# fakerlove1/HPFG

Measured on AMD Instinct MI355X. Metric: labeled+unlabeled images/sec/node, U-Net 224x224 ACDC-shaped (Mean-Teacher step), higher is better.
Workload: dtype bf16x3 (fp32 storage; products as split-bf16 MFMA hi*hi+hi*lo+lo*hi, fp32 accumulate); 1 GPU; mean_teacher_unet_224x224 (BASELINE configs[1]): U-Net 1ch->4cls, 8 labelled + 8 unlabelled per GPU, student fwd+bwd + train-mode teacher fwd + CE/Dice/MSE + SGD + EMA; size=224, hipgraph=True, sync_bn=False, parallelism=dp1, math=bf16x3

## Files before the change

### hpfg_amd/_lib.py

```python
from __future__ import annotations

import ctypes as C
import os
import threading

_HERE = os.path.dirname(os.path.abspath(__file__))
LIB_PATH = os.path.join(_HERE, "lib", "libhpfg_hip.so")

BN_MEAN, BN_RSTD, BN_SCALE, BN_SHIFT, BN_K1, BN_K2, BN_K3, BN_SPARE, BN_ROWS = range(9)
ACT_NONE, ACT_PLAIN, ACT_STRIDED, ACT_BNACT, ACT_BNACT_POOL, ACT_UP2X, ACT_DZ, ACT_SPLIT16, ACT_UPBWD = range(9)
OPT_CONV_THIN, OPT_FIRST_MFMA, OPT_FIRST_WGRAD, OPT_NARROW_DEEP, OPT_UPDATE_PACK = 0, 1, 2, 3, 4
LOSS_NSUM = 32
LOSS_MAX_CLASSES = 16
ACC_MAX_SHARDS = 8
VERSION = 142
RESIZE_TAPS = 36
SURFACE_SEGS = 32
MATH_F32, MATH_BF16X3 = 0, 1


class HipLibraryError(RuntimeError):
    pass


class Act(C.Structure):
    _fields_ = [("z", C.c_void_p), ("bn", C.c_void_p), ("aux", C.c_void_p), ("mode", C.c_int32), ("C", C.c_int32),
                ("Hs", C.c_int32), ("Ws", C.c_int32), ("pstride", C.c_int32), ("aux_pstride", C.c_int32),
                ("bn_stride", C.c_int32), ("bn_coff", C.c_int32), ("sn", C.c_int32), ("sc", C.c_int32), ("sy", C.c_int32),
                ("sx", C.c_int32), ("drop_p", C.c_float), ("drop_seed", C.c_uint32), ("drop_mask", C.c_void_p), ("seed_dev", C.c_void_p),
                ("bn_acc", C.c_void_p), ("bn_gamma", C.c_void_p), ("bn_beta", C.c_void_p), ("bn_count", C.c_float), ("bn_eps", C.c_float),
                ("bn_shards", C.c_int32), ("reserved1", C.c_int32)]


class ConvArgs(C.Structure):
    _fields_ = [("a0", Act), ("a1", Act), ("wpk", C.c_void_p), ("bias", C.c_void_p), ("out", C.c_void_p),
                ("stat_partials", C.c_void_p), ("out_pstride", C.c_int32), ("Cout", C.c_int32), ("CoutPad", C.c_int32),
                ("N", C.c_int32), ("H", C.c_int32), ("W", C.c_int32), ("taps", C.c_int32), ("math", C.c_int32),
                ("bwd_stats", C.c_int32), ("bwd_of", Act), ("out2", C.c_void_p), ("out_split", C.c_int32), ("out2_pstride", C.c_int32),
                ("stat_acc", C.c_void_p), ("stat_shards", C.c_int32), ("reserved2", C.c_int32), ("stage_out", C.c_void_p), ("side_sums", C.c_void_p)]


class WgradArgs(C.Structure):
    _fields_ = [("a0", Act), ("a1", Act), ("g", Act), ("slab", C.c_void_p), ("dw_oihw", C.c_void_p), ("Cin", C.c_int32),
                ("CinPad", C.c_int32), ("Cout", C.c_int32), ("CoutPad", C.c_int32), ("N", C.c_int32), ("H", C.c_int32),
                ("W", C.c_int32), ("taps", C.c_int32), ("S", C.c_int32), ("math", C.c_int32), ("defer_reduce", C.c_int32)]


class PeerX(C.Structure):
    _fields_ = [("mbox", C.c_void_p * 8), ("epoch", C.c_void_p), ("err", C.c_void_p), ("world", C.c_int32), ("rank", C.c_int32),
                ("slot", C.c_int32), ("cap", C.c_int32), ("slot_bytes", C.c_int64)]


class PeerBuf(C.Structure):
    _fields_ = [("win", C.c_void_p * 8), ("epoch", C.c_void_p), ("err", C.c_void_p), ("world", C.c_int32), ("rank", C.c_int32),
                ("slice", C.c_int64), ("n", C.c_int64), ("stride", C.c_int64)]


class FusedBwdArgs(C.Structure):
    _fields_ = [("d", ConvArgs), ("xa0", Act), ("xa1", Act), ("slab", C.c_void_p), ("Cin", C.c_int32), ("CinPad", C.c_int32),
                ("Cout", C.c_int32), ("CoutPad", C.c_int32)]


class AugSample(C.Structure):
    _fields_ = [("img_off", C.c_int64), ("lab_off", C.c_int64), ("h", C.c_int32), ("w", C.c_int32), ("mode", C.c_int32), ("k", C.c_int32),
                ("axis", C.c_int32), ("tab_off", C.c_int32), ("m00", C.c_double), ("m01", C.c_double), ("m10", C.c_double),
                ("m11", C.c_double), ("off_y", C.c_double), ("off_x", C.c_double)]


class BnAccDesc(C.Structure):
    _fields_ = [("acc", C.c_void_p), ("gamma", C.c_void_p), ("beta", C.c_void_p), ("running_mean", C.c_void_p), ("running_var", C.c_void_p),
                ("bn", C.c_void_p), ("C", C.c_int32), ("count", C.c_float), ("shards", C.c_int32), ("reserved", C.c_int32)]


class BnAccBwdDesc(C.Structure):
    _fields_ = [("acc", C.c_void_p), ("gamma", C.c_void_p), ("bn", C.c_void_p), ("dgamma", C.c_void_p), ("dbeta", C.c_void_p),
                ("C", C.c_int32), ("count", C.c_float), ("shards", C.c_int32), ("reserved", C.c_int32)]


class SlabDesc(C.Structure):
    _fields_ = [("slab", C.c_void_p), ("dw_oihw", C.c_void_p), ("S", C.c_int32), ("taps", C.c_int32), ("Cin", C.c_int32),
                ("CinPad", C.c_int32), ("Cout", C.c_int32), ("CoutPad", C.c_int32)]


class PackDesc(C.Structure):
    _fields_ = [("w_oihw", C.c_void_p), ("b", C.c_void_p), ("wpk_fwd", C.c_void_p), ("wpk_dgrad", C.c_void_p),
                ("bias_pad", C.c_void_p), ("wpk16_fwd", C.c_void_p), ("wpk16_dgrad", C.c_void_p), ("Cout", C.c_int32), ("Cin", C.c_int32),
                ("CoutPad", C.c_int32), ("CinPad", C.c_int32), ("taps", C.c_int32), ("kc", C.c_int32)]


class UpdatePackDesc(C.Structure):
    _fields_ = [("w_off", C.c_long), ("b_off", C.c_long), ("wpk16_fwd", C.c_void_p), ("wpk16_dgrad", C.c_void_p), ("bias_pad", C.c_void_p),
                ("t_wpk16_fwd", C.c_void_p), ("t_bias_pad", C.c_void_p), ("Cout", C.c_int32), ("Cin", C.c_int32), ("CoutPad", C.c_int32),
                ("CinPad", C.c_int32), ("taps", C.c_int32), ("kc", C.c_int32), ("kc_t", C.c_int32), ("reserved", C.c_int32)]
# ... 80 lines not shown
    "hpfg_ln_bwd_blocks": (_i, [_l]),
    "hpfg_ln_px_fwd": (_i, [_p, _p, _p, _p, _p, _p, _i, _i, _i, _i, _i, _f, _p]),
    "hpfg_ln_px_bwd": (_i, [_p, _p, _p, _p, _p, _p, _p, _p, _p, _i, _i, _i, _i, _i, _p]),
    "hpfg_ln_px_bwd_blocks": (_i, [_l]),
    "hpfg_attn_fwd": (_i, [_p, _p, _p, _i, _i, _i, _i, _f, _p]),
    "hpfg_attn_bwd": (_i, [_p, _p, _p, _p, _p, _p, _i, _i, _i, _i, _f, _p]),
    "hpfg_dwgelu_fwd": (_i, [_p, _p, _p, _p, _i, _i, _i, _i, _p]),
    "hpfg_dwgelu_bwd": (_i, [_p, _p, _p, _p, _p, _p, _p, _p, _p, _i, _i, _i, _i, _p]),
    "hpfg_dwgelu_bwd_blocks": (_i, [_i, _i, _i]),
    "hpfg_resize_bilinear_fwd": (_i, [_p, _p, _i, _i, _i, _i, _i, _i, _p]),
    "hpfg_resize_sum_fwd": (_i, [_p, C.POINTER(C.c_void_p), C.POINTER(C.c_int), C.POINTER(C.c_int), _i, _p, _i, _i, _i, _i, _p]),
    "hpfg_resize_bilinear_bwd": (_i, [_p, _p, _i, _i, _i, _i, _i, _i, _p]),
    "hpfg_residual_scale": (_i, [_p, _p, _p, _p, _i, _l, _p]),
    "hpfg_scale_rows": (_i, [_p, _p, _p, _i, _l, _p]),
    "hpfg_im2col_nhwc": (_i, [_p, _p, _i, _i, _i, _i, _i, _i, _p]),
    "hpfg_col2im_nhwc": (_i, [_p, _p, _i, _i, _i, _i, _i, _i, _p]),
    "hpfg_linear_wgrad": (_i, [_p, _p, _p, _p, _l, _i, _i, _p]),
    "hpfg_linear_wgrad_splits": (_i, [_l, _i, _i]),
    "hpfg_tok_col_stats": (_i, [_p, _l, _i, _p, _p, _p]),
    "hpfg_tok_stat_blocks": (_i, [_l]),
    "hpfg_bnrelu_apply": (_i, [_p, _p, _p, _p, _p, _p, _f, _l, _p, _l, _i, _p]),
    "hpfg_bnrelu_bwd": (_i, [_p, _p, _p, _p, _p, _p, _p, _f, _l, _p, _p, _p, _l, _i, _p]),
    "hpfg_noise_add": (_i, [_p, _p, _p, _l, _l, _f, _f, _f, _p]),
    "hpfg_uncertainty_mask": (_i, [C.POINTER(PredBlocks), _i, _i, _i, _i, _i, _p, _p, _p, _p]),
    "hpfg_mix_samples": (_i, [_p, _p, _p, _p, _i, _l, _p]),
    "hpfg_softmax_mix": (_i, [_p, _p, _p, _p, _i, _i, _i, _i, _p]),
    "hpfg_pool_scatter_add": (_i, [C.POINTER(Act), _p, _i, _p, _i, _i, _i, _i, _p]),
    "hpfg_upsample2x_bwd": (_i, [_p, _i, _p, _i, _i, _i, _i, _p]),
    "hpfg_upsample2x_bwd_sums": (_i, [_p, _i, _p, _i, _i, _i, _i, _p, _p]),
    "hpfg_upsample2x_bwd_blocks": (_i, [_i, _i, _i, _i]),
    "hpfg_loss_blocks": (_i, [_i, _i, _i]),
    "hpfg_loss_nsum": (_i, [_i]),
    "hpfg_seg_loss_partials": (_i, [C.POINTER(LossArgs), _p]),
    "hpfg_seg_loss_finalize": (_i, [C.POINTER(LossArgs), _p]),
    "hpfg_seg_loss_bwd": (_i, [C.POINTER(LossArgs), _p, _p]),
    "hpfg_argmax_labels": (_i, [_p, _i, _i, _i, _i, _p, _p, _p, _p]),
    "hpfg_cutmix_blend": (_i, [_p, _p, _p, _p, _l, _p]),
    "hpfg_sgd_step": (_i, [_p, _p, _p, _l, _p, _f, _f, _f, _p]),
    "hpfg_adamw_step": (_i, [_p, _p, _p, _p, _l, _p, _p, _d, _d, _f, _f, _f, _p]),
    "hpfg_ema_update": (_i, [_p, _p, _l, _p, _p]),
    "hpfg_sgd_ema_step": (_i, [_p, _p, _p, _l, _p, _f, _f, _f, _p, _l, _p, _p]),
    "hpfg_sgd_ema_pack_step": (_i, [_p, _p, _p, _l, _p, _f, _f, _f, _p, _l, _p, _p, C.POINTER(UpdatePackDesc), _i, _p, C.POINTER(C.c_long), _i, _p]),
    "hpfg_attn_mfma_fwd": (_i, [_p, _p, _p, _i, _i, _i, _i, _f, _p]),
    "hpfg_attn_mfma_bwd": (_i, [_p, _p, _p, _p, _p, _p, _i, _i, _i, _i, _f, _p]),
    "hpfg_attn_mfma_blocks": (_i, [_i]),
    "hpfg_attn_mfma_fwd_hd": (_i, [_p, _p, _p, _i, _i, _i, _i, _i, _f, _p]),
    "hpfg_attn_mfma_bwd_hd": (_i, [_p, _p, _p, _p, _p, _p, _i, _i, _i, _i, _i, _f, _p]),
    "hpfg_attn_mfma_scratch_floats": (_l, [_i, _i, _i, _i]),
    "hpfg_attn_keys_max": (_i, []),
    "hpfg_attn_keys_fwd": (_i, [_p, _p, _p, _p, _i, _i, _i, _i, _i, _f, _i, _p]),
    "hpfg_attn_keys_bwd": (_i, [_p, _p, _p, _p, _p, _p, _p, _p, _i, _i, _i, _i, _i, _f, _i, _p]),
    "hpfg_attn_keys_scratch_floats": (_l, [_i, _i, _i, _i, _i, _i]),
    "hpfg_attn_window_fwd": (_i, [_p, _p, _p, _i, _i, _i, _i, _i, _i, _i, _f, _i, _p]),
    "hpfg_attn_window_bwd": (_i, [_p, _p, _p, _p, _p, _p, _i, _i, _i, _i, _i, _i, _i, _f, _i, _p]),
    "hpfg_attn_window_scratch_floats": (_l, [_i, _i, _i, _i, _i, _i, _i]),
    "hpfg_attn_window_drop_fwd": (_i, [_p, _p, _p, _i, _i, _i, _i, _i, _i, _i, _f, _i, _f, _u32, _p, _p, _p]),
    "hpfg_attn_window_drop_bwd": (_i, [_p, _p, _p, _p, _p, _p, _i, _i, _i, _i, _i, _i, _i, _f, _i, _f, _u32, _p, _p, _p]),
    "hpfg_attn_window_drop_elems": (_l, [_i, _i, _i, _i, _i]),
    "hpfg_attn_window_drop_mask": (_i, [_p, _i, _i, _i, _i, _i, _f, _u32, _p, _p]),
    "hpfg_gelu_fwd": (_i, [_p, _p, _l, _p]),
    "hpfg_gelu_bwd": (_i, [_p, _p, _p, _l, _p]),
    "hpfg_token_dropout": (_i, [_p, _p, _l, _f, _u32, _p, _p, _p]),
    "hpfg_patch_merge_fwd": (_i, [_p, _p, _i, _i, _i, _i, _p]),
    "hpfg_patch_merge_bwd": (_i, [_p, _p, _i, _i, _i, _i, _p]),
    "hpfg_attn_fwd_hd": (_i, [_p, _p, _p, _i, _i, _i, _i, _i, _f, _p]),
    "hpfg_attn_bwd_hd": (_i, [_p, _p, _p, _p, _p, _p, _i, _i, _i, _i, _i, _f, _p]),
    "hpfg_gemm_f32": (_i, [_p, _l, _l, _p, _l, _l, _p, _l, _i, _i, _i, _p, _i, _i, _p]),
    "hpfg_gemm_f32_splitk": (_i, [_p, _l, _l, _p, _l, _l, _p, _l, _i, _i, _i, _p, _i, _i, _p, _p]),
    "hpfg_gemm_f32_splits": (_i, [_i, _i, _i]),
    "hpfg_gemm_bf16x3": (_i, [_p, _l, _l, _p, _l, _l, _p, _l, _i, _i, _i, _p, _i, _i, _p]),
    "hpfg_gemm_bf16x3_splits": (_i, [_i, _i, _i]),
    "hpfg_gemm_bf16x3_splitk": (_i, [_p, _l, _l, _p, _l, _l, _p, _l, _i, _i, _i, _p, _i, _i, _p, _p]),
    "hpfg_gemm_bf16x3_ok": (_i, [_p, _l, _l, _p, _l, _l, _i, _i, _i]),
    "hpfg_gemm_tn_bf16x3": (_i, [_p, _p, _p, _p, _l, _i, _i, _i, _p]),
    "hpfg_gemm_tn_splits": (_i, [_l, _i, _i]),
    "hpfg_col_sum2": (_i, [_p, _l, _i, _l, _p, _p, _p]),
    "hpfg_col_sum_splits": (_i, [_l]),
    "hpfg_col_sum": (_i, [_p, _l, _i, _l, _p, _p]),
    "hpfg_relu_bwd": (_i, [_p, _p, _l, _p]),
    "hpfg_neck_pool_fwd": (_i, [_p, _i, _i, _i, _i, _i, _i, _p, _p, _p]),
    "hpfg_neck_pool_bwd": (_i, [_p, _p, _i, _i, _i, _i, _i, _p, _p]),
    "hpfg_l2norm_fwd": (_i, [_p, _i, _i, _i, _i, _i, _p, _p, _p]),
    "hpfg_l2norm_bwd": (_i, [_p, _p, _p, _i, _i, _i, _i, _i, _p, _p, _p]),
    "hpfg_ntxent_rows": (_i, [_p, _i, _f, _p, _p, _p]),
}

_lock = threading.Lock()
_lib = None


def load() -> C.CDLL:
    global _lib
    if _lib is not None:
        return _lib
    with _lock:
        if _lib is not None:
            return _lib
        if not os.path.exists(LIB_PATH):
            raise HipLibraryError(
                f"{LIB_PATH} not found: build it with `python -c 'import __graft_entry__ as g; g.build()'` "
                f"or `make -C hpfg_amd/csrc`. There is no CPU fallback for the HIP path.")
        lib = C.CDLL(LIB_PATH)
        for name, (res, args) in PROTOTYPES.items():
            fn = getattr(lib, name)
            fn.restype = res
            fn.argtypes = args
        if lib.hpfg_version() != VERSION:
            raise HipLibraryError(f"libhpfg_hip.so version {lib.hpfg_version()} != binding version {VERSION}; rebuild")
        if os.environ.get("HPFG_FIRST_WGRAD", "1") == "0":
            lib.hpfg_set_option(OPT_FIRST_WGRAD, 0)
        if os.environ.get("HPFG_NARROW_DEEP") is not None:
            lib.hpfg_set_option(OPT_NARROW_DEEP, int(os.environ["HPFG_NARROW_DEEP"]))
        if os.environ.get("HPFG_UPDATE_PACK", "1") == "0":
            lib.hpfg_set_option(OPT_UPDATE_PACK, 0)
        _lib = lib
    return _lib


def check(rc: int, what: str):
    if rc != 0:
        msg = load().hpfg_last_error().decode("utf-8", "replace")
        raise HipLibraryError(f"{what} failed (rc={rc}): {msg}")


def ptr(t):
    return None if t is None else t.data_ptr()


def none_act() -> Act:
    return Act()
```

### hpfg_amd/csrc/common.h

```cpp
#pragma once
#include <hip/hip_runtime.h>
#include <stdint.h>
#include <stdio.h>
#include "../../include/hpfg_hip.h"

typedef float f32x4 __attribute__((ext_vector_type(4)));

#define HPFG_LEAKY 0.01f

extern "C" void hpfg_set_error(const char* fmt, ...);
int hpfg_opt(int which);
#define HPFG_ARG_CHECK(cond, ...)            \
  do {                                       \
    if (!(cond)) {                           \
      hpfg_set_error(__VA_ARGS__);           \
      return -1;                             \
    }                                        \
  } while (0)

static inline int hpfg_launch_status(const char* what) {
  hipError_t e = hipGetLastError();
  if (e != hipSuccess) {
    hpfg_set_error("%s: %s", what, hipGetErrorString(e));
    return (int)e;
// ... 266 lines not shown
      }
      break;
    }
    default:
      break;
  }
  return v;
}

__device__ static inline void dz_load_g_xhat(const HpfgAct& s, const ActCtx& cx, long pix, int c, f32x4& g_out, f32x4& xh_out) {
  f32x4 z = *reinterpret_cast<const f32x4*>(s.z + pix * s.pstride + c);
  f32x4 g = *reinterpret_cast<const f32x4*>(s.aux + pix * s.aux_pstride + c);
  const float* t = s.bn + s.bn_coff + c;
  f32x4 mu = *reinterpret_cast<const f32x4*>(t + HPFG_BN_MEAN * s.bn_stride);
  f32x4 rs = *reinterpret_cast<const f32x4*>(t + HPFG_BN_RSTD * s.bn_stride);
  f32x4 sc = *reinterpret_cast<const f32x4*>(t + HPFG_BN_SCALE * s.bn_stride);
  f32x4 sh = *reinterpret_cast<const f32x4*>(t + HPFG_BN_SHIFT * s.bn_stride);
  const uint32_t km = s.drop_p > 0.f ? keep4(s, cx, (uint32_t)(pix * s.C + c)) : 0xFu;
#pragma unroll
  for (int j = 0; j < 4; ++j) {
    float gg = (km >> j) & 1u ? g[j] * cx.inv_keep : 0.f;
    float yv = z[j] * sc[j] + sh[j];
    g_out[j] = yv > 0.f ? gg : HPFG_LEAKY * gg;
    xh_out[j] = (z[j] - mu[j]) * rs[j];
  }
}

__device__ static inline f32x4 cat_load4(const HpfgAct& a0, const ActCtx& c0, const HpfgAct& a1, const ActCtx& c1, int n, int y, int x, int c) {
  if (c < a0.C || a1.mode == HPFG_ACT_NONE) return act_load4(a0, c0, n, y, x, c);
  return act_load4(a1, c1, n, y, x, c - a0.C);
}


enum { HPFG_KIND_PLAIN = 0, HPFG_KIND_BNACT = 1, HPFG_KIND_POOL = 2, HPFG_KIND_CAT = 3, HPFG_KIND_DZ = 4, HPFG_KIND_SPLIT = 5, HPFG_KIND_UPB = 6 };

template <int MODE>
__device__ static inline f32x4 act_load4_mode(const HpfgAct& s, const ActCtx& cx, int n, int y, int x, int c) {
  HpfgAct t = s;
  t.mode = MODE;
  return act_load4(t, cx, n, y, x, c);
}

template <int KIND>
__device__ static inline f32x4 kind_load4(const HpfgAct& a0, const ActCtx& c0, const HpfgAct& a1, const ActCtx& c1, int n, int y, int x, int c) {
  if (KIND == HPFG_KIND_PLAIN) {
    if (a0.mode == HPFG_ACT_STRIDED) return act_load4_mode<HPFG_ACT_STRIDED>(a0, c0, n, y, x, c);
    return act_load4_mode<HPFG_ACT_PLAIN>(a0, c0, n, y, x, c);
  }
  if (KIND == HPFG_KIND_BNACT) return act_load4_mode<HPFG_ACT_BNACT>(a0, c0, n, y, x, c);
  if (KIND == HPFG_KIND_POOL) return act_load4_mode<HPFG_ACT_BNACT_POOL>(a0, c0, n, y, x, c);
  if (KIND == HPFG_KIND_DZ) return act_load4_mode<HPFG_ACT_DZ>(a0, c0, n, y, x, c);
  if (c < a0.C) return act_load4_mode<HPFG_ACT_BNACT>(a0, c0, n, y, x, c);
  return act_load4_mode<HPFG_ACT_UP2X>(a1, c1, n, y, x, c - a0.C);
}

__device__ inline void hpfg_up_taps(int lo, int L, int* idx, float* wgt, int& cnt) {
  const int O = 2 * L;
  const float r = O > 1 ? (float)(L - 1) / (float)(O - 1) : 0.f;
  cnt = 0;
  int b = 2 * lo - 2, e = 2 * lo + 4;
  if (b < 0) b = 0;
  if (e > O - 1) e = O - 1;
  for (int o = b; o <= e; ++o) {
    float f = r * (float)o;
    int i0 = (int)f;
    int i1 = i0 + (i0 < L - 1 ? 1 : 0);
    float w1 = f - (float)i0, w0 = 1.f - w1, w = 0.f;
    if (i0 == lo) w += w0;
    if (i1 == lo) w += w1;
    if ((i0 == lo || i1 == lo) && cnt < 8) {
      idx[cnt] = o;
      wgt[cnt] = w;
      ++cnt;
    }
  }
}
constexpr int HPFG_UPB_TAPS = 5;

__device__ __forceinline__ float hpfg_own_vgpr(float x) {
  asm volatile("" : "+v"(x));
  return x;
}
#if defined(HPFG_NO_PK_F32)
#elif defined(__HIP_DEVICE_COMPILE__)
#define HPFG_NO_PK_F32 __attribute__((target("no-packed-fp32-ops")))
#else
#define HPFG_NO_PK_F32
#endif

static inline int hpfg_kind_of(const HpfgAct& a0, const HpfgAct& a1) {
  if (a1.mode == HPFG_ACT_UP2X && a0.mode == HPFG_ACT_BNACT) return HPFG_KIND_CAT;
  if (a1.mode != HPFG_ACT_NONE) return -1;
  switch (a0.mode) {
    case HPFG_ACT_PLAIN: case HPFG_ACT_STRIDED: return HPFG_KIND_PLAIN;
    case HPFG_ACT_BNACT: return HPFG_KIND_BNACT;
    case HPFG_ACT_BNACT_POOL: return HPFG_KIND_POOL;
    case HPFG_ACT_DZ: return HPFG_KIND_DZ;
    case HPFG_ACT_SPLIT16: return HPFG_KIND_SPLIT;
    case HPFG_ACT_UPBWD: return HPFG_KIND_UPB;
    default: return -1;
  }
}
```

### hpfg_amd/csrc/conv.hip

```cpp
#include "conv_kernel.h"
#include "conv_bf16_kernel.h"

namespace {

struct HpfgFirstConvArgs {
  HpfgAct x;
  const float* w_oihw;
  const float* bias;
  float* out;
  float* stat_partials;
  long long* stat_acc;
  int stat_shards;
  long long* counters;
  int n_counters;
  int* seed_word;
  int seed_add;
};

__device__ __forceinline__ void first_bump(const HpfgFirstConvArgs& q) {
  if (blockIdx.x == 0) {
    for (int i = threadIdx.x; i < q.n_counters; i += 256) q.counters[i] += 1;
    if (threadIdx.x == 0 && q.seed_word && q.seed_add) *q.seed_word = (*q.seed_word + q.seed_add) & 0x7FFFFFFF;
  }
}
// ... 238 lines not shown
  for (const HpfgAct* s : {&a->a0, &a->a1}) {
    if (!s->bn_acc) continue;
    HPFG_ARG_CHECK((a->math & 0xff) == HPFG_MATH_BF16X3 && (s->mode == HPFG_ACT_BNACT || s->mode == HPFG_ACT_BNACT_POOL || s->mode == HPFG_ACT_DZ) &&
                       s->bn_gamma && (s->bn_beta || s->mode == HPFG_ACT_DZ) && s->bn_count >= 1.f && s->bn_count <= 16777216.f && s->C <= 256 && s->bn_shards >= 1 &&
                       s->bn_shards <= HPFG_ACC_MAX_SHARDS,
                   "conv_fwd: bn_acc needs a BNACT / BNACT_POOL / DZ source of the bf16x3 kernels with gamma (beta), a count of at most 2^24 (a float holds N*H*W exactly up to there) and at most 256 channels");
  }
  HPFG_ARG_CHECK((a->math & 0xff) != HPFG_MATH_BF16X3 || !(a->a0.mode == HPFG_ACT_BNACT || a->a0.mode == HPFG_ACT_BNACT_POOL || a->a0.mode == HPFG_ACT_DZ) ||
                     a->a0.C <= 256,
                 "conv_fwd(bf16x3): a BatchNorm'd source has at most 256 channels (got %d)", a->a0.C);
  const bool upb = a->a0.mode == HPFG_ACT_UPBWD;
  HPFG_ARG_CHECK(!upb || ((a->math & 0xff) == HPFG_MATH_BF16X3 && a->taps == 1 && a->a1.mode == HPFG_ACT_NONE && a->a0.C % 8 == 0 && a->a0.pstride % 4 == 0 &&
                          a->a0.Hs == a->H && a->a0.Ws == a->W && a->H <= 16383 && a->W <= 16383 && (long)a->N * 4 * a->H * a->W * a->a0.pstride < (1L << 31)),
                 "conv_fwd: an UPBWD source belongs to the 1x1 bf16x3 dgrad (channels a multiple of 8, pixel stride of 4, Hs x Ws == H x W)");
  HPFG_ARG_CHECK(!a->side_sums || upb, "conv_fwd: side_sums goes with an UPBWD source");
  HPFG_ARG_CHECK(!a->stage_out || upb || ((a->math & 0xff) == HPFG_MATH_BF16X3 && a->taps == 9 && hpfg_kind_of(a->a0, a->a1) > HPFG_KIND_PLAIN &&
                                    (a->a0.C + a->a1.C) % 8 == 0 && (a->H % 16 || a->W % 16)),
                 "conv_fwd: stage_out is a feature of the 3x3 bf16x3 kernels (non-PLAIN source, channels a multiple of 8, H or W not a multiple of 16)");
  hipStream_t st = (hipStream_t)stream;
  if (a->bwd_stats) {
    const int kind = hpfg_kind_of(a->a0, a->a1);
    HPFG_ARG_CHECK((a->math & 0xff) == HPFG_MATH_BF16X3 && (kind == HPFG_KIND_DZ || kind == HPFG_KIND_PLAIN || (kind == HPFG_KIND_UPB && a->bwd_stats == 1)),
                   "conv_fwd: bwd_stats is a dgrad feature of the bf16x3 kernels (DZ, PLAIN or UPBWD source)");
    HPFG_ARG_CHECK((a->stat_partials || a->stat_acc) && a->bwd_of.z && a->bwd_of.bn && !a->bias,
                   "conv_fwd: bwd_stats needs stat_partials or stat_acc, bwd_of.z / .bn and no bias");
    const int up = a->bwd_stats == 2 ? 2 : 1;
    HPFG_ARG_CHECK(a->bwd_stats == 1 || a->bwd_stats == 2, "conv_fwd: bwd_stats must be 0, 1 or 2");
    HPFG_ARG_CHECK(a->bwd_of.C == a->Cout && a->Cout == a->CoutPad && a->bwd_of.Hs == up * a->H && a->bwd_of.Ws == up * a->W && a->bwd_of.pstride % 4 == 0,
                   "conv_fwd: bwd_of must describe a layer with C == Cout == CoutPad (%d/%d/%d) at the output size (twice it for bwd_stats == 2)",
                   a->bwd_of.C, a->Cout, a->CoutPad);
    HPFG_ARG_CHECK(a->bwd_stats == 1 || (a->taps == 9 && (a->H % 16 || a->W % 16) && a->bwd_of.aux && a->bwd_of.aux_pstride % 4 == 0 && a->bwd_of.drop_p == 0.f && !a->out_split),
                   "conv_fwd: bwd_stats == 2 (max-pool backward in the epilogue) needs a 3x3 dgrad at a size that is not a multiple of 16, bwd_of.aux (the gradient so far) and no dropout behind bwd_of");
  }
  if ((a->math & 0xff) == HPFG_MATH_BF16X3) {
    {
      const int r = hpfg_conv_thin_try(*a, st, rows_only);
      if (r != HPFG_THIN_NONE) return r;
    }
    switch (hpfg_kind_of(a->a0, a->a1)) {
      case HPFG_KIND_PLAIN: return hpfg_conv16_launch_plain(*a, st, rows_only);
      case HPFG_KIND_BNACT: return hpfg_conv16_launch_bnact(*a, st, rows_only);
      case HPFG_KIND_POOL: return hpfg_conv16_launch_pool(*a, st, rows_only);
      case HPFG_KIND_CAT: return hpfg_conv16_launch_cat(*a, st, rows_only);
      case HPFG_KIND_DZ: return hpfg_conv16_launch_dz(*a, st, rows_only);
      case HPFG_KIND_UPB: return hpfg_conv16_launch_upb(*a, st, rows_only);
      default: break;
    }
    hpfg_set_error("conv_fwd(bf16x3): unsupported source combination (a0.mode=%d, a1.mode=%d)", a->a0.mode, a->a1.mode);
    return -1;
  }
  if (rows_only) {
    const int tl = tile_is_big(a->H, a->W) ? 16 : 8;
    *rows_only = a->N * ((a->H + tl - 1) / tl) * ((a->W + tl - 1) / tl);
    return 0;
  }
  switch (hpfg_kind_of(a->a0, a->a1)) {
    case HPFG_KIND_PLAIN: return hpfg_conv_launch_plain(*a, st);
    case HPFG_KIND_BNACT: return hpfg_conv_launch_bnact(*a, st);
    case HPFG_KIND_POOL: return hpfg_conv_launch_pool(*a, st);
    case HPFG_KIND_CAT: return hpfg_conv_launch_cat(*a, st);
    case HPFG_KIND_DZ: return hpfg_conv_launch_dz(*a, st);
    default: break;
  }
  hpfg_set_error("conv_fwd: unsupported source combination (a0.mode=%d, a1.mode=%d)", a->a0.mode, a->a1.mode);
  return -1;
}
// ... 45 lines not shown
```

### hpfg_amd/csrc/fused_bwd.hip

```cpp
#include "fused_bwd_kernel.h"

int hpfg_first_wgrad_grid(int N, int H, int W);
int hpfg_first_wgrad_launch(const HpfgAct& g, const HpfgAct& x, float* slab, int Cin, int N, int H, int W, hipStream_t st);

namespace {

using namespace hpfg_fused;

template <int CI, int CO, int AK, int GK, int NW, int WGS, int PFA, int PFPOS, int BMAX = 48, bool NODG = false>
int launch(const HpfgFusedBwdArgs& a, hipStream_t st, bool grid_only) {
  const int grid = fused_grid<CI, CO, AK, GK, NW, WGS, BMAX>(a);
  if (grid_only) return grid;
  const int tx = a.d.W / T, ty = a.d.H / T;
  if (a.d.stat_acc) HPFG_ACC_CHECK(grid, a.d.stat_shards, "fused_bwd");
  if constexpr (NODG) {
    hipLaunchKernelGGL((fused_bwd_kernel<CI, CO, AK, GK, false, NW, WGS, PFA, PFPOS, BMAX, true>), dim3(grid), dim3(64 * NW), 0, st, a, tx, ty);
  } else if (a.d.bwd_stats) {
    if constexpr (AK == HPFG_KIND_BNACT)
      hipLaunchKernelGGL((fused_bwd_kernel<CI, CO, AK, GK, true, NW, WGS, PFA, PFPOS, BMAX>), dim3(grid), dim3(64 * NW), 0, st, a, tx, ty);
    else
      return -3;
  } else {
    hipLaunchKernelGGL((fused_bwd_kernel<CI, CO, AK, GK, false, NW, WGS, PFA, PFPOS, BMAX>), dim3(grid), dim3(64 * NW), 0, st, a, tx, ty);
  }
  return hipGetLastError() == hipSuccess ? 0 : -1;
}

int dispatch(const HpfgFusedBwdArgs& a, hipStream_t st, bool grid_only) {
  const int ci = a.CinPad / 16, co = a.CoutPad / 16;
  const int ak = hpfg_kind_of(a.xa0, a.xa1), gk = hpfg_kind_of(a.d.a0, a.d.a1);
#define HPFG_FUSED_CASE(CI, CO, AK, GK, NW, WGS, PFA, PFPOS) \
  if (ci == CI && co == CO && ak == AK && gk == GK) return launch<CI, CO, AK, GK, NW, WGS, PFA, PFPOS>(a, st, grid_only);
  if (!a.d.out) {
    if (ci == 1 && co == 1 && ak == HPFG_KIND_PLAIN && gk == HPFG_KIND_DZ) {
      if (a.Cin == 1 && a.d.W >= 64 && a.d.W <= 512 && a.Cout == 16 && a.xa0.mode == HPFG_ACT_STRIDED && a.d.a0.pstride % 4 == 0 && a.d.a0.aux_pstride % 4 == 0 &&
          hpfg_opt(HPFG_OPT_FIRST_WGRAD) != 0) {
        if (grid_only) return hpfg_first_wgrad_grid(a.d.N, a.d.H, a.d.W);
        return hpfg_first_wgrad_launch(a.d.a0, a.xa0, a.slab, a.Cin, a.d.N, a.d.H, a.d.W, st);
      }
      return launch<1, 1, HPFG_KIND_PLAIN, HPFG_KIND_DZ, 4, 2, 1, 1, 48, true>(a, st, grid_only);
    }
    return grid_only ? 0 : -2;
  }
  HPFG_FUSED_CASE(1, 1, HPFG_KIND_BNACT, HPFG_KIND_DZ, 4, 2, 1, 1)
  HPFG_FUSED_CASE(1, 1, HPFG_KIND_BNACT, HPFG_KIND_PLAIN, 4, 2, 1, 1)
  HPFG_FUSED_CASE(1, 2, HPFG_KIND_POOL, HPFG_KIND_DZ, 8, 1, 1, 0)
  HPFG_FUSED_CASE(2, 2, HPFG_KIND_BNACT, HPFG_KIND_DZ, 8, 1, 2, 1)
  HPFG_FUSED_CASE(2, 1, HPFG_KIND_CAT, HPFG_KIND_DZ, 8, 1, 2, 1)
#undef HPFG_FUSED_CASE
  return grid_only ? 0 : -2;
}

int check(const HpfgFusedBwdArgs* a) {
  HPFG_ARG_CHECK(a, "fused_bwd: null args");
  const HpfgConvArgs& d = a->d;
  if (d.taps != 9 || d.H % T || d.W % T || (d.math & 0xff) != HPFG_MATH_BF16X3) return 1;
  if (a->CinPad % 16 || a->CoutPad % 16 || a->CinPad > 64 || a->CoutPad > 32) return 1;
  return 0;
}

}

extern "C" int hpfg_fused_bwd_grid(const HpfgFusedBwdArgs* a) {
  const int c = check(a);
  if (c) return c < 0 ? -1 : 0;
  return dispatch(*a, nullptr, true);
}

extern "C" int hpfg_fused_bwd(const HpfgFusedBwdArgs* a, void* stream) {
  const int c = check(a);
  if (c < 0) return -1;
  HPFG_ARG_CHECK(c == 0, "fused_bwd: 3x3 bf16x3 layers with H, W multiples of 16, CinPad <= 64 and CoutPad <= 32 only");
  const HpfgConvArgs& d = a->d;
  const bool wonly = !d.out;
  HPFG_ARG_CHECK(a->slab && d.a0.z && (wonly ? (!d.wpk && !d.bwd_stats && !d.out2) : d.wpk != nullptr), "fused_bwd: slab and the dZ source are required; wpk with out");
  HPFG_ARG_CHECK(d.Cout == a->Cin && d.CoutPad == a->CinPad && d.a0.C == a->Cout && a->xa0.C + a->xa1.C == a->Cin,
                 "fused_bwd: the dgrad side must describe the same layer (d.Cout == Cin, d.a0.C == Cout, input channels == Cin)");
  HPFG_ARG_CHECK((wonly || a->Cin % 8 == 0) && (a->Cout % 8 == 0 || d.a0.mode == HPFG_ACT_PLAIN || d.a0.mode == HPFG_ACT_STRIDED), "fused_bwd: Cin (and Cout behind a DZ source) must be multiples of 8");
#ifndef HPFG_TRACE
  HPFG_ARG_CHECK(!d.bias, "fused_bwd: the dgrad side takes no bias");
#endif
  HPFG_ARG_CHECK(d.a1.mode == 0 && !d.a1.z, "fused_bwd: the dgrad side takes no second source");
  HPFG_ARG_CHECK(wonly || (d.Cout == d.CoutPad && d.out_pstride % 4 == 0 && d.out2_pstride % 4 == 0), "fused_bwd: Cin must be a multiple of 16 and the dX pixel strides of 4");
  if (hpfg_kind_of(a->xa0, a->xa1) == HPFG_KIND_CAT)
    HPFG_ARG_CHECK(a->xa0.C == a->xa1.C && a->xa0.C % 16 == 0, "fused_bwd: a concatenated input must be two halves of a multiple of 16 channels");
  HPFG_ARG_CHECK(!d.out_split || (d.out2 && d.out_split % 16 == 0 && d.out_split < d.Cout && !d.bwd_stats),
                 "fused_bwd: out_split needs out2, a multiple of 16 below Cin, and no bwd_stats");
  if (d.bwd_stats) {
    HPFG_ARG_CHECK((d.stat_partials || d.stat_acc) && d.bwd_of.z && d.bwd_of.bn, "fused_bwd: bwd_stats needs stat_partials or stat_acc, and bwd_of.z / .bn");
    HPFG_ARG_CHECK(!d.stat_acc || (d.stat_shards >= 1 && d.stat_shards <= HPFG_ACC_MAX_SHARDS && (d.stat_shards & (d.stat_shards - 1)) == 0),
                   "fused_bwd: bad stat_shards %d", d.stat_shards);
    HPFG_ARG_CHECK(d.bwd_of.C == d.Cout && d.Cout == d.CoutPad && d.bwd_of.Hs == d.H && d.bwd_of.Ws == d.W && d.bwd_of.pstride % 4 == 0,
                   "fused_bwd: bwd_of must describe a layer with C == Cin == CinPad at the layer's size");
    HPFG_ARG_CHECK(a->xa0.mode == HPFG_ACT_BNACT && a->xa1.mode == 0 && d.bwd_of.z == a->xa0.z && d.bwd_of.bn == a->xa0.bn &&
                       d.bwd_of.bn_coff == a->xa0.bn_coff && d.bwd_of.pstride == a->xa0.pstride,
                   "fused_bwd: bwd_of must be the producer of this layer's (BNACT) input");
  } else {
    HPFG_ARG_CHECK(!d.stat_partials && !d.stat_acc, "fused_bwd: stat_partials / stat_acc without bwd_stats");
  }
  const int r = dispatch(*a, (hipStream_t)stream, false);
  HPFG_ARG_CHECK(r != -2, "fused_bwd: no instantiation for CinPad %d, CoutPad %d, input kind %d, dZ kind %d", a->CinPad, a->CoutPad,
                 hpfg_kind_of(a->xa0, a->xa1), hpfg_kind_of(a->d.a0, a->d.a1));
  HPFG_ARG_CHECK(r != -3, "fused_bwd: bwd_stats needs a BNACT input");
  HPFG_ARG_CHECK(r == 0, "fused_bwd: launch failed");
  return 0;
}
```

### hpfg_amd/csrc/fused_bwd_kernel.h

```cpp
#pragma once
#include <type_traits>
#include "tile16.h"

namespace hpfg_fused {

using namespace hpfg_tile16;
using hpfg_conv16::Cfg;

constexpr int DPL = PL, DCH = CH;
constexpr int APL = T * T * 32;
constexpr int ACH = 2 * APL;

template <int NW>
struct Split {
  static constexpr int NTH = 64 * NW;
  static constexpr int ND = halo_pieces<NTH>(), NA = T * T * 2 / NTH, MI = 16 / NW;
  static_assert(NW == 4 || NW == 8, "4 or 8 waves");
};

template <int CI, int CO, int AK, int GK, int NW, bool BWD, int BMAX = 48>
struct Geo : Halves<CI, AK> {
  using Halves<CI, AK>::NA0;
  using Halves<CI, AK>::NA1;
  static constexpr int TABD = GK == HPFG_KIND_DZ ? 5 * 16 * CO * 4 : 0;
  static constexpr int TABA = 2 * 16 * NA0 * 4;
  static constexpr int STAT = 2 * NW * 16 * CI * 4;
  static constexpr int KS = 5 * CO;
  static constexpr bool BREG = KS * CI * 8 <= BMAX;
  static constexpr int BFR = BREG ? 0 : KS * CI * 2 * 1024;
  static constexpr bool ZLDS = BWD && AK == HPFG_KIND_BNACT;
  static constexpr int ZPS = 64 * CI + 32;
  static constexpr int ZL = ZLDS ? T * T * ZPS : 0;
  static constexpr int OFF_STAT = CO * DCH + CI * ACH, OFF_TABD = OFF_STAT + STAT, OFF_TABA = OFF_TABD + TABD, OFF_B = OFF_TABA + TABA,
                       OFF_Z = OFF_B + BFR, OFF_U = OFF_Z + ZL;
  static constexpr int LDS = OFF_U + NA1 * UBYTES;
};

template <int CI, int CO, int AK, int GK, bool BWD, int NW, int WGS, int PFA, int PFPOS, int BMAX = 48, bool NODG = false>
__global__ __launch_bounds__(64 * NW, WGS) void fused_bwd_kernel(HpfgFusedBwdArgs p, int tiles_x, int tiles_y) {
  using C = Cfg<16, 16, 4, 1, CI, 9, 16>;
  using G = Geo<CI, CO, AK, GK, NW, BWD, BMAX>;
  static_assert(!BWD || AK == HPFG_KIND_BNACT, "the backward sums of the layer below need its raw output as this layer's input");
  using SP = Split<NW>;
  constexpr int AK0 = G::AK0, NA0 = G::NA0, NA1 = G::NA1, NTH = SP::NTH, ND = SP::ND, NA = SP::NA, MI = SP::MI;
  __shared__ __attribute__((aligned(16))) unsigned char lds[G::LDS];
  unsigned char* ldsD = lds;
  unsigned char* ldsA = lds + CO * DCH;
  float* ldsf = reinterpret_cast<float*>(lds + G::OFF_STAT);
  float* tabD = reinterpret_cast<float*>(lds + G::OFF_TABD);
  float* tabA = reinterpret_cast<float*>(lds + G::OFF_TABA);
  const bf16x8* ldsB = reinterpret_cast<const bf16x8*>(lds + G::OFF_B);
  unsigned char* ldsZ = lds + G::OFF_Z;
  float* ldsU = reinterpret_cast<float*>(lds + G::OFF_U);
  static_assert(NA1 == 0 || UP::SH * UP::SW * 2 <= NTH, "one source piece of the upsampled half per thread");
  const int tid = threadIdx.x, lane = tid & 63, wave = tid >> 6;
  const int H = p.d.H, W = p.d.W;
  const int ntiles = tiles_x * tiles_y, nwork = ntiles * p.d.N;
  const HpfgAct none = {};
  const HpfgAct& aD = p.d.a0;
  const HpfgAct aS = skip_source<G::CATK>(p.xa0);
  const ActCtx cxg = make_ctx(aD), cxa = make_ctx(aS);
#ifdef HPFG_TRACE
  const bool tr_on = (p.d.math & 0x2000) && tid == 0;
  unsigned long long* tr_buf = reinterpret_cast<unsigned long long*>(const_cast<float*>(p.d.bias)) + 256 * (long)blockIdx.x;
  int tr_i = 0;
#endif
  HPFG_TR_REAL(12)
  HPFG_TR(1)
  const int gsel = tid & 1;

  if (GK == HPFG_KIND_DZ) fill_tables_lds<GK, 16 * CO>(aD, tabD, 16 * CO, tid, NTH);
  fill_tables_lds<AK0, 16 * NA0, false>(aS, tabA, 16 * NA0, tid, NTH);

  constexpr int NIJ = CI * CO;
  constexpr int PPW = NIJ >= NW ? NIJ / NW : 1;
  constexpr int TSTR = NIJ >= NW ? 1 : NW / NIJ;
  constexpr int NT = (9 + TSTR - 1) / TSTR;
  static_assert(NIJ == 1 || NIJ == 2 || NIJ == 4 || NIJ == 8, "pairs must split evenly over the waves");
  f32x4 accw[PPW][NT];
#pragma unroll
  for (int a = 0; a < PPW; ++a)
#pragma unroll
    for (int t = 0; t < NT; ++t) accw[a][t] = f32x4{0.f, 0.f, 0.f, 0.f};
  const int wt0 = NIJ >= NW ? 0 : wave / NIJ;

  const int kg = lane >> 4;
  int aoff[MI], toff[5];
  frag_offsets<MI>(aoff, toff, wave, lane);
  const int q4 = (lane & 15) >> 2, pp = lane & 3;
  const int trA = (4 * kg + q4) * 32 + pp * 8, trD = trA;

  constexpr int KS = G::KS;
  constexpr int PB = G::BREG && !NODG ? KS : 0;
  const int ntn = p.d.CoutPad / 16;
  const bf16x8* wpk = reinterpret_cast<const bf16x8*>(p.d.wpk);
  bf16x8 pbh[PB > 0 ? PB : 1][CI], pbl[PB > 0 ? PB : 1][CI];
  resident_weights<C, PB, !G::BREG && !NODG>(pbh, pbl, wpk, ntn, reinterpret_cast<bf16x8*>(lds + G::OFF_B), KS * CI * 2 * 64, tid, NTH);

  f32x4 s1[CI], s2[CI];
#pragma unroll
  for (int j = 0; j < CI; ++j) {
    s1[j] = f32x4{0.f, 0.f, 0.f, 0.f};
    s2[j] = s1[j];
  }
  ActCtx bcx = {};
  if (BWD) bcx = make_ctx(p.d.bwd_of);

  const TileWalk tw = tile_walk(nwork, gridDim.x >= 8 ? 8 : 1);
  const int wend = tw.wend, GS = tw.step;

  RawPiece<GK> rawD[CO][ND];
  RawPiece<AK0> rawA0[NA0][NA];
  f32x4 rawU[NA1 > 0 ? NA1 : 1][2];

  auto issue = [&](auto early_tag, int n, int ty0, int tx0, bool live) {
    constexpr bool EARLY = decltype(early_tag)::value;
    if (EARLY) {
#pragma unroll
      for (int c = 0; c < CO; ++c) {
        const int c0 = c * 16 + gsel * 8;
        issue_halo<GK, NTH>(rawD[c], aD, cxg, n, ty0, tx0, H, W, tid, c0, c0 < aD.C, live);
      }
    }
#pragma unroll
    for (int c = 0; c < NA0; ++c) {
      if ((c < PFA) != EARLY) continue;
      const int c0 = c * 16 + gsel * 8;
      const bool chv = c0 < aS.C;
#pragma unroll
      for (int i = 0; i < NA; ++i) {
        const int pix = (tid + i * NTH) >> 1;
        issue_piece<AK0>(rawA0[c][i], aS, none, cxa, n, live ? ty0 + pix / T : 0, live ? tx0 + pix % T : 0, chv ? c0 : 0, live && chv);
      }
    }
    if (NA1 > 0) {
      const int sy_base = up_base(ty0, p.xa1.Hs), sx_base = up_base(tx0, p.xa1.Ws);
#pragma unroll
      for (int c = 0; c < NA1; ++c) {
        if ((NA0 + c < PFA) != EARLY) continue;
        const int cu = c * 16 + gsel * 8;
        up_patch_issue<UP::SW>(rawU[c], p.xa1, n, sy_base, sx_base, live ? tid >> 1 : 0, cu < p.xa1.C ? cu : 0);
      }
    }
  };

  int w = tw.w;
  if (w < wend) issue(std::true_type{}, w / ntiles, ((w % ntiles) / tiles_x) * T, ((w % ntiles) % tiles_x) * T, true);
  __syncthreads();
  HPFG_TR(2)

  for (; w < wend; w += GS) {
    const int n = w / ntiles, ty0 = ((w % ntiles) / tiles_x) * T, tx0 = ((w % ntiles) % tiles_x) * T;
    if (PFA < CI) issue(std::false_type{}, n, ty0, tx0, true);
    HPFG_TR(3)
#pragma unroll
    for (int c = 0; c < CO; ++c) {
      const int c0 = c * 16 + gsel * 8;
      Tab tg;
      load_tables_lds<GK, 16 * CO>(tg, tabD, aD, c0);
      stage_halo<GK, NTH>(ldsD + c * DCH, rawD[c], tg, aD, cxg, n, ty0, tx0, H, W, tid, c0, c0 < aD.C);
    }
#pragma unroll
    for (int c = 0; c < NA0; ++c) {
      const int c0 = c * 16 + gsel * 8;
      const bool chv = c0 < aS.C;
      Tab ta;
      load_tables_lds<AK0, 16 * NA0>(ta, tabA, aS, c0);
#pragma unroll
      for (int i = 0; i < NA; ++i) {
        const int pix = (tid + i * NTH) >> 1;
        f32x4 v0, v1;
        finish_piece<AK0>(v0, v1, rawA0[c][i], ta, aS, none, cxa, n, ty0 + pix / T, tx0 + pix % T, chv ? c0 : 0, chv);
        if (G::ZLDS) {
          *reinterpret_cast<f32x4*>(ldsZ + pix * G::ZPS + c0 * 4) = rawA0[c][i].v[0];
          *reinterpret_cast<f32x4*>(ldsZ + pix * G::ZPS + c0 * 4 + 16) = rawA0[c][i].v[1];
        }
        bf16x8 hi, lo;
        split8(v0, v1, hi, lo);
        unsigned char* o = ldsA + c * ACH + pix * 32 + gsel * 16;
        *reinterpret_cast<bf16x8*>(o) = hi;
        *reinterpret_cast<bf16x8*>(o + APL) = lo;
      }
    }
    if (NA1 > 0) {
      if (tid < UP::SH * UP::SW * 2) {
#pragma unroll
        for (int c = 0; c < NA1; ++c) up_patch_park<16>(ldsU + c * (UBYTES / 4), rawU[c], tid >> 1, gsel * 8);
      }
      __syncthreads();
      const int sy_base = up_base(ty0, p.xa1.Hs), sx_base = up_base(tx0, p.xa1.Ws);
#pragma unroll
      for (int i = 0; i < NA; ++i) {
        const int pix = (tid + i * NTH) >> 1;
// ... 210 lines not shown
```

### hpfg_amd/csrc/loss.hip

```cpp
#include <string.h>
#include "common.h"
#include "peer.h"

namespace {

constexpr int PIX_PER_BLOCK = 1024;
constexpr float SMOOTH = 1e-5f;
constexpr int OFF_I0 = 8;
constexpr int stride_of(int C) { return C <= 4 ? 4 : 16; }
constexpr int nsum_of(int C) { return OFF_I0 + 6 * stride_of(C); }
static_assert(nsum_of(4) == HPFG_LOSS_NSUM && nsum_of(5) == HPFG_LOSS_NSUM_WIDE && nsum_of(16) == HPFG_LOSS_NSUM_WIDE, "sums layout");

template <int C>
__device__ inline void load_px(const float* base, long pix, float* l) {
  if (C % 4 == 0) {
    const f32x4* b = reinterpret_cast<const f32x4*>(base + pix * C);
#pragma unroll
    for (int j = 0; j < C / 4; ++j) {
      f32x4 v = b[j];
      l[4 * j] = v[0]; l[4 * j + 1] = v[1]; l[4 * j + 2] = v[2]; l[4 * j + 3] = v[3];
    }
  } else {
#pragma unroll
    for (int c = 0; c < C; ++c) l[c] = base[pix * C + c];
  }
}

template <int C>
__device__ inline void store_px(float* base, long pix, const float* g) {
  if (C % 4 == 0) {
    f32x4* b = reinterpret_cast<f32x4*>(base + pix * C);
#pragma unroll
    for (int j = 0; j < C / 4; ++j) b[j] = f32x4{g[4 * j], g[4 * j + 1], g[4 * j + 2], g[4 * j + 3]};
  } else {
#pragma unroll
    for (int c = 0; c < C; ++c) base[pix * C + c] = g[c];
  }
}

template <int C>
__device__ inline void softmax_w(const float* l, float* p, float& m, float& se) {
  m = l[0];
#pragma unroll
  for (int c = 1; c < C; ++c) m = fmaxf(m, l[c]);
  se = 0.f;
#pragma unroll
  for (int c = 0; c < C; ++c) {
    p[c] = expf(l[c] - m);
    se += p[c];
  }
  const float inv = 1.f / se;
#pragma unroll
  for (int c = 0; c < C; ++c) p[c] *= inv;
}

__device__ inline float wave_sum(float v) {
#pragma unroll
  for (int o = 32; o >= 1; o >>= 1) v += __shfl_xor(v, o);
  return v;
}

template <int C>
__global__ __launch_bounds__(256) void loss_partials_kernel(HpfgLossArgs a, long npix_img) {
  constexpr int S = stride_of(C), NS = nsum_of(C);
  __shared__ float red[4][NS];
  const int tid = threadIdx.x, lane = tid & 63, wave = tid >> 6;
  for (int i = tid; i < 4 * NS; i += 256) (&red[0][0])[i] = 0.f;
  const long total = (long)a.N * npix_img;
  const long p0 = (long)blockIdx.x * PIX_PER_BLOCK;
  const long p1 = p0 + PIX_PER_BLOCK < total ? p0 + PIX_PER_BLOCK : total;
  const long pb = (long)a.n_lab * npix_img;
  __syncthreads();
#pragma nounroll
  for (int grp = 0; grp < 2; ++grp) {
    const long lo = grp == 0 ? p0 : (p0 > pb ? p0 : pb);
    const long hi = grp == 0 ? (p1 < pb ? p1 : pb) : p1;
    if (lo >= hi) continue;
    const uint8_t* lab = grp == 0 ? a.labels0 : a.labels1;
    const long lab_off = grp == 0 ? 0 : pb;
    const bool cons = grp == 1 && a.t_logits;
    float nll = 0.f, cnt = 0.f, mse = 0.f, msk = 0.f;
    float I[C], Z[C], Y[C];
#pragma unroll
    for (int c = 0; c < C; ++c) I[c] = Z[c] = Y[c] = 0.f;
    for (long pix = lo + tid; pix < hi; pix += 256) {
      float l[C], p[C], m, se;
      load_px<C>(a.logits, pix, l);
      softmax_w<C>(l, p, m, se);
// ... 40 lines not shown
    }
    float* r = red[wave];
    const int base = OFF_I0 + grp * 3 * S;
    nll = wave_sum(nll);
    cnt = wave_sum(cnt);
    if (lane == 0) {
      r[2 * grp] = nll;
      r[2 * grp + 1] = cnt;
    }
    if (cons) {
      mse = wave_sum(mse);
      msk = wave_sum(msk);
      if (lane == 0) {
        r[4] = mse;
        r[5] = msk;
      }
    }
    if (lab) {
#pragma unroll
      for (int c = 0; c < C; ++c) {
        const float vi = wave_sum(I[c]), vz = wave_sum(Z[c]), vy = wave_sum(Y[c]);
        if (lane == 0) {
          r[base + c] = vi;
          r[base + S + c] = vz;
          r[base + 2 * S + c] = vy;
        }
      }
    }
  }
  __syncthreads();
  for (int i = tid; i < NS; i += 256) a.partials[(long)blockIdx.x * NS + i] = red[0][i] + red[1][i] + red[2][i] + red[3][i];
}

__global__ __launch_bounds__(256) void loss_reduce_kernel(const float* __restrict__ partials, int nblk, int ns, float* __restrict__ sums, HpfgPeerX px) {
  __shared__ double sh[4];
  const int i = blockIdx.x;
  double v = 0.0;
  for (int b = threadIdx.x; b < nblk; b += 256) v += (double)partials[(long)b * ns + i];
#pragma unroll
  for (int o = 32; o >= 1; o >>= 1) v += __shfl_xor(v, o);
  if ((threadIdx.x & 63) == 0) sh[threadIdx.x >> 6] = v;
  __syncthreads();
  if (threadIdx.x == 0) {
    double t[1] = {sh[0] + sh[1] + sh[2] + sh[3]};
    if (px.world > 1) {
      const int idx[1] = {i};
      hpfg_peer_allreduce<1>(px, idx, t);
    }
    sums[i] = (float)t[0];
  }
}

__device__ inline float dice_of(const float* s, int base, int S, int C) {
  float d = 0.f;
  for (int c = 0; c < C; ++c) d += 1.f - (2.f * s[base + c] + SMOOTH) / (s[base + S + c] + s[base + 2 * S + c] + SMOOTH);
  return d / (float)C;
}

__global__ void loss_finalize_kernel(HpfgLossArgs a) {
  if (threadIdx.x != 0 || blockIdx.x != 0) return;
  const float* s = a.sums;
  const int C = a.C, S = stride_of(C);
  float ce0 = s[1] > 0.f ? s[0] / s[1] : 0.f;
  float ce1 = s[3] > 0.f ? s[2] / s[3] : 0.f;
  float d0 = a.labels0 && a.n_lab > 0 ? dice_of(s, OFF_I0, S, C) : 0.f;
  float d1 = a.labels1 && a.n_lab < a.N ? dice_of(s, OFF_I0 + 3 * S, S, C) : 0.f;
  float cnt = (float)((double)(a.N - a.n_lab) * a.H * a.W * C * a.world);
  float mse = (a.t_logits && cnt > 0.f) ? (a.cons_mask ? s[4] / (2.f * s[5] + 1e-16f) : s[4] / cnt) : 0.f;
  const float* k = a.coef;
  a.out[0] = k[0] * ce0 + k[1] * d0 + k[2] * ce1 + k[3] * d1 + k[4] * mse;
  a.out[1] = ce0;
  a.out[2] = d0;
  a.out[3] = ce1;
  a.out[4] = d1;
  a.out[5] = mse;
  a.out[6] = 0.f;
  a.out[7] = 0.f;
}

template <int C>
__global__ __launch_bounds__(256) void loss_bwd_kernel(HpfgLossArgs a, long npix_img, const float* __restrict__ gscale_dev) {
  constexpr int S = stride_of(C), CW = 16;
  __shared__ float cA[2][CW], cB[2][CW];
  const float gscale = gscale_dev ? *gscale_dev : 1.f;
  const float* s = a.sums;
  const float* k = a.coef;
  const long total = (long)a.N * npix_img;
  const long pb = (long)a.n_lab * npix_img;
  const float cnt_mse = (float)((double)(a.N - a.n_lab) * a.H * a.W * C * a.world);
  if (threadIdx.x < 2 * CW) {
    const int g = threadIdx.x / CW, c = threadIdx.x % CW;
    float ca = 0.f, cb = 0.f;
    if (c < C) {
      const int base = OFF_I0 + g * 3 * S;
      const float wd = k[2 * g + 1] / (float)C;
      const float den = s[base + S + c] + s[base + 2 * S + c] + SMOOTH;
      const float num = 2.f * s[base + c] + SMOOTH;
      ca = -2.f * wd / den;
      cb = 2.f * wd * num / (den * den);
    }
    cA[g][c] = ca;
    cB[g][c] = cb;
  }
  __syncthreads();
  const float wm = cnt_mse > 0.f ? k[4] * 2.f / (a.cons_mask ? 2.f * s[5] + 1e-16f : cnt_mse) : 0.f;
  for (long pix = blockIdx.x * 256L + threadIdx.x; pix < total; pix += (long)gridDim.x * 256) {
    const int grp = pix < pb ? 0 : 1;
    float l[C], p[C], dp[C], m, se;
    load_px<C>(a.logits, pix, l);
    if (a.input_is_prob) {
#pragma unroll
      for (int c = 0; c < C; ++c) p[c] = l[c];
    } else {
      softmax_w<C>(l, p, m, se);
    }
#pragma unroll
    for (int c = 0; c < C; ++c) dp[c] = 0.f;
    const uint8_t* lab = grp == 0 ? a.labels0 : a.labels1;
    int t = 255;
    if (lab) {
      t = grp == 0 ? lab[pix] : lab[pix - pb];
      const float* ga = cA[grp];
      const float* gb = cB[grp];
#pragma unroll
      for (int c = 0; c < C; ++c) {
        const float tc = (t == c) ? 1.f : 0.f;
        dp[c] += ga[c] * tc + gb[c] * p[c];
      }
    }
    if (grp == 1 && a.t_logits) {
      float q[C], tl[C], tm, ts;
      const long upix = pix - pb;
      load_px<C>(a.t_logits, a.t_unlab_only ? upix : pix, tl);
      if (a.teacher_is_prob) {
#pragma unroll
        for (int c = 0; c < C; ++c) q[c] = tl[c];
      } else {
        softmax_w<C>(tl, q, tm, ts);
      }
      const float w = a.cons_mask ? wm * a.cons_mask[upix] : wm;
#pragma unroll
      for (int c = 0; c < C; ++c) dp[c] += w * (p[c] - q[c]);
    }
    float dot = 0.f;
#pragma unroll
    for (int c = 0; c < C; ++c) dot += p[c] * dp[c];
    const float cn = s[2 * grp + 1];
    const float wc = k[2 * grp];
    const bool ce_on = lab && t != 255 && t < C && cn > 0.f;
    float g[C];
#pragma unroll
    for (int c = 0; c < C; ++c) {
      g[c] = a.input_is_prob ? dp[c] : p[c] * (dp[c] - dot);
      if (ce_on && !a.input_is_prob) g[c] += wc * (p[c] - (t == c ? 1.f : 0.f)) / cn;
      g[c] *= gscale;
    }
    store_px<C>(a.dlogits, pix, g);
  }
}

#define HPFG_LOSS_CASE(N_, ...) case N_: { constexpr int C = N_; __VA_ARGS__; } break;
#define HPFG_LOSS_DISPATCH(C_, ...) \
  switch (C_) {                      \
    HPFG_LOSS_CASE(2, __VA_ARGS__) HPFG_LOSS_CASE(3, __VA_ARGS__) HPFG_LOSS_CASE(4, __VA_ARGS__) HPFG_LOSS_CASE(5, __VA_ARGS__) HPFG_LOSS_CASE(6, __VA_ARGS__)      \
    HPFG_LOSS_CASE(7, __VA_ARGS__) HPFG_LOSS_CASE(8, __VA_ARGS__) HPFG_LOSS_CASE(9, __VA_ARGS__) HPFG_LOSS_CASE(10, __VA_ARGS__) HPFG_LOSS_CASE(11, __VA_ARGS__)    \
    HPFG_LOSS_CASE(12, __VA_ARGS__) HPFG_LOSS_CASE(13, __VA_ARGS__) HPFG_LOSS_CASE(14, __VA_ARGS__) HPFG_LOSS_CASE(15, __VA_ARGS__) HPFG_LOSS_CASE(16, __VA_ARGS__) \
    default: HPFG_ARG_CHECK(false, "seg_loss: C must be 2..16 (got %d)", C_); \
  }

}

extern "C" int hpfg_loss_blocks(int N, int H, int W) { return (int)(((long)N * H * W + PIX_PER_BLOCK - 1) / PIX_PER_BLOCK); }

extern "C" int hpfg_loss_nsum(int C) { return nsum_of(C); }

static int check_loss(const HpfgLossArgs* a) {
  HPFG_ARG_CHECK(a && a->logits && a->coef && a->sums, "seg_loss: null pointer");
  HPFG_ARG_CHECK(a->C >= 2 && a->C <= 16, "seg_loss: C must be 2..16 (got %d)", a->C);
  HPFG_ARG_CHECK(a->N > 0 && a->n_lab >= 0 && a->n_lab <= a->N && a->H > 0 && a->W > 0 && a->world >= 1, "seg_loss: bad sizes");
  HPFG_ARG_CHECK(a->n_lab == 0 || a->labels0, "seg_loss: labels0 missing");
  return 0;
}

static int loss_partials_impl(const HpfgLossArgs* a, const HpfgPeerX* px, void* stream) {
  if (int rc = check_loss(a)) return rc;
  HPFG_ARG_CHECK(a->partials, "seg_loss_partials: workspace missing");
  const int nblk = hpfg_loss_blocks(a->N, a->H, a->W), ns = nsum_of(a->C);
  const long npix = (long)a->H * a->W;
  HPFG_LOSS_DISPATCH(a->C, hipLaunchKernelGGL(loss_partials_kernel<C>, dim3(nblk), dim3(256), 0, (hipStream_t)stream, *a, npix));
  HpfgPeerX none;
  memset(&none, 0, sizeof(none));
  hipLaunchKernelGGL(loss_reduce_kernel, dim3(ns), dim3(256), 0, (hipStream_t)stream, a->partials, nblk, ns, a->sums, px ? *px : none);
  return hpfg_launch_status("loss_partials_kernel");
}

extern "C" int hpfg_seg_loss_partials(const HpfgLossArgs* a, void* stream) { return loss_partials_impl(a, nullptr, stream); }

extern "C" int hpfg_seg_loss_partials_x(const HpfgLossArgs* a, const HpfgPeerX* px, void* stream) {
  HPFG_ARG_CHECK(px, "seg_loss_partials_x: null exchange descriptor");
  if (int rc = check_loss(a)) return rc;
  if (px->world > 1) {
    HPFG_ARG_CHECK(px->world <= HPFG_PEER_MAX_RANKS && px->rank >= 0 && px->rank < px->world && px->epoch && px->slot >= 0 &&
                       hpfg_loss_nsum(a->C) <= px->cap && px->slot_bytes == hpfg_peer_slot_bytes(px->world, px->cap),
                   "seg_loss_partials_x: bad exchange descriptor");
    for (int r = 0; r < px->world; ++r) HPFG_ARG_CHECK(px->mbox[r], "seg_loss_partials_x: mailbox of rank %d not mapped", r);
  }
  return loss_partials_impl(a, px, stream);
}

extern "C" int hpfg_seg_loss_finalize(const HpfgLossArgs* a, void* stream) {
  if (int rc = check_loss(a)) return rc;
  HPFG_ARG_CHECK(a->out, "seg_loss_finalize: out missing");
  hipLaunchKernelGGL(loss_finalize_kernel, dim3(1), dim3(64), 0, (hipStream_t)stream, *a);
  return hpfg_launch_status("loss_finalize_kernel");
}

extern "C" int hpfg_seg_loss_bwd(const HpfgLossArgs* a, const float* grad_scale_dev, void* stream) {
  if (int rc = check_loss(a)) return rc;
  HPFG_ARG_CHECK(a->dlogits, "seg_loss_bwd: dlogits missing");
  const long npix = (long)a->H * a->W, total = a->N * npix;
  long b = (total + 255) / 256;
  if (b > 4096) b = 4096;
  HPFG_LOSS_DISPATCH(a->C, hipLaunchKernelGGL(loss_bwd_kernel<C>, dim3((int)b), dim3(256), 0, (hipStream_t)stream, *a, npix, grad_scale_dev));
  return hpfg_launch_status("loss_bwd_kernel");
}
```

### hpfg_amd/csrc/misc.hip

```cpp
#include <stdarg.h>
#include <string.h>
#include "stage.h"

static thread_local char g_err[512] = "";
extern "C" void hpfg_set_error(const char* fmt, ...) {
  va_list ap;
  va_start(ap, fmt);
  vsnprintf(g_err, sizeof(g_err), fmt, ap);
  va_end(ap);
}
extern "C" const char* hpfg_last_error(void) { return g_err; }
extern "C" int hpfg_version(void) { return HPFG_VERSION; }

static int g_opt[HPFG_OPT_COUNT] = {1, 1, 1, 128, 1};
int hpfg_opt(int which) { return which >= 0 && which < HPFG_OPT_COUNT ? g_opt[which] : 0; }
extern "C" int hpfg_get_option(int which) { return hpfg_opt(which); }
extern "C" int hpfg_set_option(int which, int value) {
  HPFG_ARG_CHECK(which >= 0 && which < HPFG_OPT_COUNT, "set_option: unknown option %d", which);
  const int old = g_opt[which];
  g_opt[which] = value;
  return old;
}

namespace {

__global__ __launch_bounds__(256) void pack_weights_kernel(const HpfgPackDesc* __restrict__ table, long long* __restrict__ counters, int n_counters,
                                                           int* __restrict__ seed_word, int seed_add, long long* __restrict__ zero, long n_zero) {
  if (blockIdx.x == 0 && blockIdx.y == 0) {
    for (int i = threadIdx.x; i < n_counters; i += 256) counters[i] += 1;
    if (threadIdx.x == 0 && seed_word && seed_add) *seed_word = (*seed_word + seed_add) & 0x7FFFFFFF;
  }
  for (long i = ((long)blockIdx.y * gridDim.x + blockIdx.x) * 256 + threadIdx.x; i < n_zero; i += (long)gridDim.x * gridDim.y * 256) zero[i] = 0;
  const HpfgPackDesc d = table[blockIdx.y];
  const long total = (long)d.taps * d.CinPad * d.CoutPad;
  const int nt_f = d.CoutPad / 16, nch_f = d.CinPad / 16;
  const int nt_d = d.CinPad / 16, nch_d = d.CoutPad / 16;
  for (long i = blockIdx.x * 256L + threadIdx.x; i < total; i += (long)gridDim.x * 256) {
    int ks = (int)(i & 3), lane = (int)((i >> 2) & 63);
    long r = i >> 8;
    if (d.wpk_fwd) {
      int nt = (int)(r % nt_f), ch = (int)((r / nt_f) % nch_f), tap = (int)(r / ((long)nt_f * nch_f));
      int co = nt * 16 + (lane & 15), ci = ch * 16 + ks * 4 + (lane >> 4);
      d.wpk_fwd[i] = (co < d.Cout && ci < d.Cin) ? d.w_oihw[((long)co * d.Cin + ci) * d.taps + tap] : 0.f;
    }
    if (d.wpk_dgrad) {
      int nt = (int)(r % nt_d), ch = (int)((r / nt_d) % nch_d), tap = (int)(r / ((long)nt_d * nch_d));
      int co = ch * 16 + ks * 4 + (lane >> 4), ci = nt * 16 + (lane & 15);
// ... 594 lines not shown
```

### hpfg_amd/csrc/stage.h

```cpp
#pragma once
#include "common.h"

namespace hpfg_stage {

typedef __bf16 bf16x8 __attribute__((ext_vector_type(8)));

typedef float f32x2 __attribute__((ext_vector_type(2)));
typedef __bf16 bf16x2 __attribute__((ext_vector_type(2)));

__device__ __forceinline__ void split8(const f32x4& a, const f32x4& b, bf16x8& hi, bf16x8& lo) {
  uint32_t hw[4], lw[4];
#pragma unroll
  for (int k = 0; k < 4; ++k) {
    const float x0 = k < 2 ? a[2 * k] : b[2 * k - 4], x1 = k < 2 ? a[2 * k + 1] : b[2 * k - 3];
    const bf16x2 h = __builtin_convertvector(f32x2{x0, x1}, bf16x2);
    const uint32_t w = __builtin_bit_cast(uint32_t, h);
    const f32x2 hf = {__builtin_bit_cast(float, w << 16), __builtin_bit_cast(float, w & 0xFFFF0000u)};
    const bf16x2 l = __builtin_convertvector(f32x2{x0, x1} - hf, bf16x2);
    hw[k] = w;
    lw[k] = __builtin_bit_cast(uint32_t, l);
  }
  typedef uint32_t u32x4 __attribute__((ext_vector_type(4)));
  hi = __builtin_bit_cast(bf16x8, (u32x4{hw[0], hw[1], hw[2], hw[3]}));
  lo = __builtin_bit_cast(bf16x8, (u32x4{lw[0], lw[1], lw[2], lw[3]}));
}

__device__ __forceinline__ f32x4 ld4(const float* base, int off) { return *reinterpret_cast<const f32x4*>(base + off); }
__device__ __forceinline__ int clampi(int v, int lo, int hi) { return min(max(v, lo), hi); }

typedef short s16x4 __attribute__((ext_vector_type(4)));
typedef short s16x8 __attribute__((ext_vector_type(8)));
__device__ __forceinline__ bf16x8 tr_read8(const unsigned char* row0, const unsigned char* row1) {
  const s16x4 a = __builtin_amdgcn_ds_read_tr16_b64_v4i16((s16x4 __attribute__((address_space(3)))*)(row0));
  const s16x4 b = __builtin_amdgcn_ds_read_tr16_b64_v4i16((s16x4 __attribute__((address_space(3)))*)(row1));
  return __builtin_bit_cast(bf16x8, (s16x8{a[0], a[1], a[2], a[3], b[0], b[1], b[2], b[3]}));
}

#ifdef HPFG_TRACE
#define HPFG_TR(ID)                                                                                        \
  if (tr_on && tr_i < 255) {                                                                               \
    tr_buf[tr_i++] = ((unsigned long long)(ID) << 56) | (__builtin_amdgcn_s_memtime() & 0xffffffffffffffull); \
  }
#define HPFG_TR_REAL(ID)                                                                                   \
  if (tr_on && tr_i < 255) {                                                                               \
    tr_buf[tr_i++] = ((unsigned long long)(ID) << 56) | (__builtin_amdgcn_s_memrealtime() & 0xffffffffffffffull); \
  }
#else
#define HPFG_TR(ID)
#define HPFG_TR_REAL(ID)
#endif

struct TileWalk {
  int w, wend, step;
};
__device__ __forceinline__ TileWalk tile_walk(int nwork, int nx) {
  const int xg = (int)blockIdx.x % nx, xj = (int)blockIdx.x / nx;
  const int per_x = (nwork + nx - 1) / nx;
  TileWalk t;
  t.wend = (xg + 1) * per_x < nwork ? (xg + 1) * per_x : nwork;
  t.step = ((int)gridDim.x - xg + nx - 1) / nx;
  t.w = xg * per_x + xj;
  return t;
}

template <int KIND>
struct RawCount { static constexpr int N = KIND == HPFG_KIND_POOL || KIND == HPFG_KIND_CAT ? 8 : (KIND == HPFG_KIND_DZ ? 4 : 2); };

template <int KIND>
struct RawPiece {
  f32x4 v[RawCount<KIND>::N];
  uint32_t dm[2];
};

struct Tab {
  f32x4 sc[2], sh[2], k1[2], k2[2], k3[2];
};

template <int KIND>
__device__ __forceinline__ void load_tables(Tab& t, const HpfgAct& a0, int c0, bool chvalid) {
  if (KIND == HPFG_KIND_PLAIN || KIND == HPFG_KIND_SPLIT || !chvalid) return;
  if (KIND == HPFG_KIND_CAT && c0 >= a0.C) return;
  const float* b = a0.bn + a0.bn_coff + c0;
  const int st = a0.bn_stride;
  t.sc[0] = ld4(b, HPFG_BN_SCALE * st);
  t.sc[1] = ld4(b, HPFG_BN_SCALE * st + 4);
  t.sh[0] = ld4(b, HPFG_BN_SHIFT * st);
  t.sh[1] = ld4(b, HPFG_BN_SHIFT * st + 4);
  if (KIND == HPFG_KIND_DZ) {
    t.k1[0] = ld4(b, HPFG_BN_K1 * st);
    t.k1[1] = ld4(b, HPFG_BN_K1 * st + 4);
    t.k2[0] = ld4(b, HPFG_BN_K2 * st);
    t.k2[1] = ld4(b, HPFG_BN_K2 * st + 4);
    t.k3[0] = ld4(b, HPFG_BN_K3 * st);
    t.k3[1] = ld4(b, HPFG_BN_K3 * st + 4);
  }
}

constexpr int HPFG_BN_CMAX = 256;
template <int KIND>
// ... 200 lines not shown
    up_coord(gx, u.Ws, i0, i1, wx1);
    const float wy0 = 1.f - wy1, wx0 = 1.f - wx1;
    v0 = bilerp(wy0, wy1, wx0, wx1, raw[0], raw[2], raw[4], raw[6]);
    v1 = bilerp(wy0, wy1, wx0, wx1, raw[1], raw[3], raw[5], raw[7]);
  } else {
    f32x4 ga = raw[2], gb = raw[3];
    if (a.drop_p > 0.f) {
      const uint32_t e = (uint32_t)(((n * a.Hs + gy) * a.Ws + gx) * a.C + c0);
      const uint32_t thr = drop_thresh(a, cx0);
      ga = ga * cx0.inv_keep;
      gb = gb * cx0.inv_keep;
      keep_select4(ga, a.drop_mask ? rp.dm[0] : hpfg_hash32(e >> 2, cx0.seed), thr);
      keep_select4(gb, a.drop_mask ? rp.dm[1] : hpfg_hash32((e + 4) >> 2, cx0.seed), thr);
    }
    const f32x4 ya = raw[0] * t.sc[0] + t.sh[0], yb = raw[1] * t.sc[1] + t.sh[1];
    const f32x4 la = ga * HPFG_LEAKY, lb = gb * HPFG_LEAKY;
#pragma unroll
    for (int j = 0; j < 4; ++j) {
      ga[j] = ya[j] > 0.f ? ga[j] : la[j];
      gb[j] = yb[j] > 0.f ? gb[j] : lb[j];
    }
    v0 = t.k1[0] * ga + (t.k2[0] * raw[0] + t.k3[0]);
    v1 = t.k1[1] * gb + (t.k2[1] * raw[1] + t.k3[1]);
  }
  if (need_ok) {
#pragma unroll
    for (int j = 0; j < 4; ++j) {
      v0[j] = ok ? v0[j] : 0.f;
      v1[j] = ok ? v1[j] : 0.f;
    }
  }
}

template <int KIND>
__device__ __forceinline__ void split_piece(const f32x4& v0, const f32x4& v1, bf16x8& hi, bf16x8& lo) {
  if (KIND == HPFG_KIND_SPLIT) {
    hi = __builtin_bit_cast(bf16x8, v0);
    lo = __builtin_bit_cast(bf16x8, v1);
  } else {
    split8(v0, v1, hi, lo);
  }
}

}
```

### hpfg_amd/csrc/tile16.h

```cpp
#pragma once
#include "conv_bf16_kernel.h"

namespace hpfg_tile16 {

using namespace hpfg_stage;

constexpr int T = 16, HP = 18, RS = 18;
constexpr int NSLOT = (HP * HP + 15) / 16 * 16;
constexpr int PL = NSLOT * 32;
constexpr int CH = 2 * PL;
using UP = UpPatch<T, T>;
constexpr int UBYTES = UP::SH * UP::SW * 16 * 4;

template <int CI, int AK>
struct Halves {
  static constexpr bool CATK = AK == HPFG_KIND_CAT;
  static constexpr int AK0 = CATK ? HPFG_KIND_BNACT : AK;
  static constexpr int NA0 = CATK ? CI / 2 : CI, NA1 = CATK ? CI / 2 : 0;
};
template <bool CATK>
__device__ __forceinline__ HpfgAct skip_source(const HpfgAct& a) {
  HpfgAct s = a;
  if (CATK) s.drop_p = 0.f;
  return s;
// ... 34 lines not shown
#pragma unroll
  for (int i = 0; i < halo_pieces<NTH>(); ++i) {
    const int idx = tid + i * NTH, pix = idx >> 1;
    const int gy = ty0 + pix / HP - 1, gx = tx0 + pix % HP - 1;
    const bool ok = live && idx < HP * HP * 2 && chv && gy >= 0 && gy < H && gx >= 0 && gx < W;
    issue_piece<KIND>(raw[i], a, none, cx, n, live ? clampi(gy, 0, H - 1) : 0, live ? clampi(gx, 0, W - 1) : 0, chv ? c0 : 0, ok);
  }
}
__device__ __forceinline__ void store_halo(unsigned char* chunk, int idx, const f32x4& v0, const f32x4& v1) {
  if (idx < HP * HP * 2) {
    const int pix = idx >> 1;
    bf16x8 hi, lo;
    split8(v0, v1, hi, lo);
    unsigned char* o = chunk + ((pix / HP) * RS + pix % HP) * 32 + (idx & 1) * 16;
    *reinterpret_cast<bf16x8*>(o) = hi;
    *reinterpret_cast<bf16x8*>(o + PL) = lo;
  }
}
template <int KIND, int NTH>
__device__ __forceinline__ void stage_halo(unsigned char* chunk, const RawPiece<KIND> (&raw)[halo_pieces<NTH>()], const Tab& t, const HpfgAct& a,
                                           const ActCtx& cx, int n, int ty0, int tx0, int H, int W, int tid, int c0, bool chv) {
  const HpfgAct none = {};
#pragma unroll
  for (int i = 0; i < halo_pieces<NTH>(); ++i) {
    const int idx = tid + i * NTH, pix = idx >> 1;
    const int gy = ty0 + pix / HP - 1, gx = tx0 + pix % HP - 1;
    const bool ok = idx < HP * HP * 2 && chv && gy >= 0 && gy < H && gx >= 0 && gx < W;
    f32x4 v0, v1;
    finish_piece<KIND>(v0, v1, raw[i], t, a, none, cx, n, clampi(gy, 0, H - 1), clampi(gx, 0, W - 1), chv ? c0 : 0, ok);
    store_halo(chunk, idx, v0, v1);
  }
}

}
```

### hpfg_amd/csrc/wgrad.hip

```cpp
#include <cstdlib>
#include "wgrad_kernel.h"
#include "wgrad_bf16_kernel.h"

namespace {

__global__ __launch_bounds__(256) void slab_reduce_kernel(const float* __restrict__ slab, float* __restrict__ dw, int S, int taps, int Cin,
                                                          int CinPad, int Cout, int CoutPad) {
  __shared__ float red[16][17];
  const long per = (long)taps * CinPad * CoutPad;
  const int il = threadIdx.x & 15, sl = threadIdx.x >> 4;
  const long i = (long)blockIdx.x * 16 + il;
  float t0 = 0.f, t1 = 0.f;
  if (i < per) {
    int s = sl;
    for (; s + 16 < S; s += 32) {
      t0 += slab[s * per + i];
      t1 += slab[(s + 16) * per + i];
    }
    if (s < S) t0 += slab[s * per + i];
  }
  red[sl][il] = t0 + t1;
  __syncthreads();
  if (sl == 0 && i < per) {
    float t = 0.f;
// ... 98 lines not shown
  for (int o = 32; o >= 1; o >>= 1) a += __shfl_xor(a, o);
  if (threadIdx.x == 0) out[c] = (float)a;
}

}

extern "C" int hpfg_wgrad_splits(int N, int H, int W, int CinPad, int CoutPad, int taps) {
  (void)taps;
  using namespace hpfg_wg;
  int ni, nj;
  hpfg_wg16::pick_shape(CinPad, CoutPad, &ni, &nj);
  long pairs = (long)(CinPad / (16 * ni)) * (CoutPad / (16 * nj));
  long nwork = (long)N * ((H + TH - 1) / TH) * ((W + TW - 1) / TW);
  const long resident = 512;
  long target = resident / pairs;
  if (target < 1) target = 1;
  if (target > nwork) target = nwork;
  long per_block = (nwork + target - 1) / target;
  return (int)((nwork + per_block - 1) / per_block);
}

extern "C" long hpfg_wgrad_slab_floats(int N, int H, int W, int CinPad, int CoutPad, int taps) {
  return (long)hpfg_wgrad_splits(N, H, W, CinPad, CoutPad, taps) * taps * CinPad * CoutPad;
}

extern "C" int hpfg_wgrad(const HpfgWgradArgs* a, void* stream) {
  HPFG_ARG_CHECK(a && a->slab && a->dw_oihw, "wgrad: null pointer");
  HPFG_ARG_CHECK(a->taps == 9 || a->taps == 1, "wgrad: taps must be 1 or 9");
  HPFG_ARG_CHECK(a->CinPad % 16 == 0 && a->CoutPad % 16 == 0 && a->Cin <= a->CinPad && a->Cout <= a->CoutPad, "wgrad: bad channel padding");
  HPFG_ARG_CHECK(a->S >= 1, "wgrad: S < 1");
  HPFG_ARG_CHECK(a->a1.mode == HPFG_ACT_NONE || a->a0.C % 16 == 0, "wgrad: concat needs a0.C %% 16 == 0");
  hipStream_t st = (hipStream_t)stream;
  const int akind = hpfg_kind_of(a->a0, a->a1);
  HPFG_ARG_CHECK(akind >= 0 && akind != HPFG_KIND_DZ, "wgrad: unsupported input source (a0.mode=%d, a1.mode=%d)", a->a0.mode, a->a1.mode);
  int rc = 1;
  const bool b16 = (a->math & 0xff) == HPFG_MATH_BF16X3 && a->taps == 9;
  if ((a->math & 0xff) == HPFG_MATH_BF16X3 && a->taps == 1 && (a->g.mode == HPFG_ACT_PLAIN || a->g.mode == HPFG_ACT_STRIDED) && a->g.C % 4 == 0)
    rc = hpfg_wgrad16_launch_1x1(*a, akind, st);
  if (a->g.mode == HPFG_ACT_SPLIT16 || akind == HPFG_KIND_SPLIT) {
    HPFG_ARG_CHECK(b16, "wgrad: SPLIT16 sources are a feature of the 3x3 bf16x3 kernel");
    rc = hpfg_wgrad16_launch_split(*a, akind, st);
  } else if (rc != 1) {
  } else if (b16 && a->g.mode == HPFG_ACT_DZ) rc = hpfg_wgrad16_launch_dz(*a, akind, st);
  else if (b16 && (a->g.mode == HPFG_ACT_PLAIN || a->g.mode == HPFG_ACT_STRIDED)) rc = hpfg_wgrad16_launch_plain(*a, akind, st);
  else if (a->g.mode == HPFG_ACT_DZ) rc = hpfg_wgrad_launch_dz(*a, akind, st);
  else if (a->g.mode == HPFG_ACT_PLAIN || a->g.mode == HPFG_ACT_STRIDED) rc = hpfg_wgrad_launch_plain(*a, akind, st);
  else {
    hpfg_set_error("wgrad: unsupported gradient source mode %d", a->g.mode);
    return -1;
  }
  if (rc || a->defer_reduce) return rc;
  long per = (long)a->taps * a->CinPad * a->CoutPad;
  hipLaunchKernelGGL(slab_reduce_kernel, dim3((unsigned)((per + 15) / 16)), dim3(256), 0, st, a->slab, a->dw_oihw, a->S, a->taps, a->Cin, a->CinPad,
                     a->Cout, a->CoutPad);
  return hpfg_launch_status("slab_reduce_kernel");
}

extern "C" int hpfg_slab_reduce_multi(const HpfgSlabDesc* table_dev, const HpfgSlabDesc* table_host, int nlayers, void* stream) {
  HPFG_ARG_CHECK(table_dev && table_host && nlayers > 0 && nlayers < 65536, "slab_reduce_multi: bad args");
  long mx = 0;
  for (int i = 0; i < nlayers; ++i) {
    long per = (long)table_host[i].taps * table_host[i].CinPad * table_host[i].CoutPad;
    if (per > mx) mx = per;
  }
  long gx = (mx + 63) / 64;
  if (gx > 2048) gx = 2048;
  hipLaunchKernelGGL(slab_reduce_multi_kernel, dim3((unsigned)gx, nlayers), dim3(256), 0, (hipStream_t)stream, table_dev);
// ... 26 lines not shown
```

### hpfg_amd/engine.py

```python
from __future__ import annotations

import ctypes as C
import itertools
import os
from dataclasses import dataclass
from typing import Dict, List, Optional

import torch

from . import _lib as L

SEED_BUMP = -1

WIDTHS = (16, 32, 64, 128, 256)
ENC_DROPOUT = (0.05, 0.1, 0.2, 0.3, 0.5)
BN_EPS, BN_MOMENTUM = 1e-5, 0.1


ACC, LOCAL, ALLREDUCE, PEER, EVAL = "acc", "local", "allreduce", "peer", "eval"


def bn_route(train: bool, math: int, bn_acc_on: bool, peer: bool, world: int, force_sync: bool) -> str:
    if not train:
        return EVAL
# ... 153 lines not shown
        self._accb_table: Optional[DescTable] = None
        self.seed_dev = torch.zeros(1, dtype=torch.int32, device=device)
        self.bump_counters: Optional[torch.Tensor] = None
        self.base_seed = 0x1234567
        self.dropout_on = False
        self._stage_inputs = False
        self.bwd_ready = False
        self.x: Optional[torch.Tensor] = None
        self.world = 1
        self.gtmp, self.direct = None, False
        self._bwd_alloc_key: Optional[tuple] = None
        self.dA, self.dA_ps = {}, {}
        self.dcat, self.dup, self.dU, self.dP = {}, {}, {}, {}
        self.slab_of, self.csum_part, self.csum_rows = {}, {}, {}
        self.slabs: Optional[DescTable] = None
        self.bias_layers = [s for s in self.order if not s.bn]
        self._n_enc_desc = sum(1 for s in self.order if s.name.startswith("encoder."))
        self._n_thin_enc_desc = sum(1 for s in self.order if s.name.startswith("encoder.in_conv") or s.name.startswith("encoder.down1"))
        self.fuse_bwd_stats = 1
        self._fused_rows: Dict[str, int] = {}
        self.fused_bwd = os.environ.get("HPFG_FUSED_BWD", "1") == "1"
        self.pool_fuse = True
        self._pool_done: set = set()
        self.dz_side = True
        self.act_side = True
        self.upb_fuse = os.environ.get("HPFG_UPB_FUSE", "1") == "1"
        self.upb_max_c1 = int(os.environ.get("HPFG_UPB_MAX_C1", "128"))
        self.dzbuf: Dict[str, torch.Tensor] = {}
        self.actbuf: Dict[str, torch.Tensor] = {}
        self._act_live: set = set()
        self.defer_wgrad = False
        self._deferred: Optional[list] = None
        self._csum_pending: Optional[torch.Tensor] = None
        self.fused_grid: Dict[str, int] = {}
        self._side, self._side_used = None, False
        self.force_sync = False
        self.math = L.MATH_F32
        self.ext_masks: Dict[str, torch.Tensor] = {}
        self.allreduce = None
        self.peer, self.peer_base, self.xepoch = None, 0, None
        self.marks: Optional[MarkLog] = None

    def _stream(self):
        return torch.cuda.current_stream(self.dev).cuda_stream

    def _call(self, fn, *args, tag: Optional[str] = None, stream: Optional[int] = None):
        st = self._stream() if stream is None else stream

        def launch():
            L.check(fn(*args, st), f"{fn.__name__}[{tag}]" if tag else fn.__name__)
        if tag is None or self.marks is None:
            return launch()
        self.marks.bracket(tag, st, launch)

    @property
    def _b16(self) -> bool:
        return self.math == L.MATH_BF16X3

    def _fork_side(self) -> torch.cuda.Stream:
        if self._side is None:
            self._side = torch.cuda.Stream(device=self.dev)
        self._side.wait_stream(torch.cuda.current_stream(self.dev))
        return self._side

    def _join_side(self):
        if self._side_used:
            torch.cuda.current_stream(self.dev).wait_stream(self._side)
            self._side_used = False

    def layer_seed(self, s: ConvSpec) -> int:
        return (self.base_seed * 0x9E3779B1 + 0x85EBCA6B * (s.idx + 1)) & 0xFFFFFFFF

    def _act_bn(self, name: str, mode=L.ACT_BNACT) -> L.Act:
        s = self.specs[name]
        a = L.Act()
        a.z, a.bn, a.mode, a.C = L.ptr(self.z[name]), L.ptr(self.bn[name]), mode, s.cout
        a.Hs, a.Ws, a.pstride, a.bn_stride, a.bn_coff = s.h, s.w, s.cout, s.cout, 0
        if self.fwd_route == ACC and mode in (L.ACT_BNACT, L.ACT_BNACT_POOL):
            a.bn_acc, a.bn_gamma, a.bn_beta = L.ptr(self.acc_of[name]), L.ptr(self.params[f"{s.bn}.weight"]), L.ptr(self.params[f"{s.bn}.bias"])
            a.bn_count, a.bn_eps, a.bn_shards = float(self.N * s.h * s.w), BN_EPS, self.acc_shards[name]
        if mode == L.ACT_BNACT:
            self._act_dropout(a, s)
        return a

    def _act_dropout(self, a: L.Act, s: ConvSpec):
        if s.drop_p > 0 and self.dropout_on:
            a.drop_p, a.drop_seed, a.seed_dev = s.drop_p, self.layer_seed(s), L.ptr(self.seed_dev)
            a.drop_mask = L.ptr(self.ext_masks.get(s.name)) if self.ext_masks else None

    def _act_plain(self, t: torch.Tensor, C_: int, h: int, w: int, pstride: Optional[int] = None, mode=L.ACT_PLAIN) -> L.Act:
# ... 85 lines not shown
        self._call(self.lib.hpfg_bn_acc_bwd_finalize, dev, host, n, tag="bn_bfin_all")

    def _finalize_all(self, track: bool):
        if track not in self._acc_tables:
            descs = (L.BnAccDesc * len(self.bn_layers))()
            for d, s in zip(descs, self.bn_layers):
                d.acc, d.gamma, d.beta = L.ptr(self.acc_of[s.name]), L.ptr(self.params[f"{s.bn}.weight"]), L.ptr(self.params[f"{s.bn}.bias"])
                d.running_mean = L.ptr(self.buffers[f"{s.bn}.running_mean"]) if track else None
                d.running_var = L.ptr(self.buffers[f"{s.bn}.running_var"]) if track else None
                d.bn, d.C, d.count, d.shards = L.ptr(self.bn[s.name]), s.cout, float(self.N * s.h * s.w), self.acc_shards[s.name]
            self._acc_tables[track] = DescTable(descs, self.dev)
        dev, host, n = self._acc_tables[track].sub(0, len(self.bn_layers))
        self._call(self.lib.hpfg_bn_acc_finalize, dev, host, n, BN_MOMENTUM, BN_EPS, tag="bn_fin_all")

    def _finalize_bn(self, s: ConvSpec, nblk: int, track: bool):
        rm, rv = (L.ptr(self.buffers[f"{s.bn}.running_{k}"]) if track else None for k in ("mean", "var"))
        tail = (float(self.N * s.h * s.w * self.world), L.ptr(self.params[f"{s.bn}.weight"]), L.ptr(self.params[f"{s.bn}.bias"]), rm, rv,
                BN_MOMENTUM, BN_EPS, L.ptr(self.bn[s.name]), s.cout)
        if self.fwd_route == PEER:
            px = self.peer.peer_desc(self.peer_base + 2 * self._bn_idx[s.name], self.xepoch)
            self._call(self.lib.hpfg_bn_fwd_finalize_x, L.ptr(self.partials), nblk, C.byref(px), *tail, tag="bn_fin:" + s.name)
        elif self.fwd_route == ALLREDUCE:
            sums = self.sums[: 2 * s.cout_pad]
            self._call(self.lib.hpfg_reduce_partials, L.ptr(self.partials), nblk, s.cout_pad, L.ptr(sums))
            self.allreduce(sums)
            self._call(self.lib.hpfg_bn_fwd_finalize, None, 0, L.ptr(sums), *tail)
        else:
            self._call(self.lib.hpfg_bn_fwd_finalize, L.ptr(self.partials), nblk, None, *tail, tag="bn_fin:" + s.name)

    def forward(self, x: torch.Tensor, train: bool = True, dropout: Optional[bool] = None, track_running: bool = True,
                seed_step: Optional[int] = None, needs_grad: bool = True) -> torch.Tensor:
        pack_args = self._fwd_begin(x, train, dropout, seed_step, needs_grad)
        logits = torch.empty(self.N, self.H, self.W, self.ncls, dtype=torch.float32, device=self.dev)
        for i, s in enumerate(self.order):
            if i == 0 and pack_args is not None:
                main = torch.cuda.current_stream(self.dev)
                with torch.cuda.stream(self._fork_side()):
                    self.pack(**pack_args)
                self._fwd_layer(s, logits, track_running)
                main.wait_stream(self._side)
                continue
            self._fwd_layer(s, logits, track_running)
            if self.after_layer is not None and i == self.after_layer[0]:
                self.after_layer[1]()
        if self.fwd_route == ACC:
            self._finalize_all(track_running)
            self._acc_dirty = False
        self.bwd_ready = bool(train and needs_grad)
        return logits

    def _fwd_begin(self, x: torch.Tensor, train: bool, dropout: Optional[bool], seed_step: Optional[int], needs_grad: bool) -> Optional[dict]:
        assert x.is_cuda and x.dtype == torch.float32 and tuple(x.shape) == (self.N, self.in_ch, self.H, self.W), (x.shape, x.dtype, x.device)
        self.x = x
        self._act_live = set()
        self._stage_inputs = bool(train and needs_grad and self.act_side and self._b16)
        self.dropout_on = train if dropout is None else dropout
        if seed_step is not None and seed_step != SEED_BUMP:
            self.seed_dev.fill_(int(seed_step) & 0x7FFFFFFF)
        counters, self.bump_counters = self.bump_counters, None
        self.fwd_route = bn_route(train, self.math, self.bn_acc_on, self.peer is not None, self.world, self.force_sync)
        if self.fwd_route == ACC:
            if self._acc_dirty:
                self.acc_all.zero_()
            self._acc_dirty = True
        pack_args = dict(with_dgrad=bool(train and needs_grad), counters=counters, seed_add=1 if seed_step == SEED_BUMP else 0)
        self._first_bump = None
        self.last_fwd_packed = not (self._b16 and self.frag_ok and self.frag_token is not None and (self.frag_dgrad or not pack_args["with_dgrad"]))
        self.frag_ok = False
        if not self.last_fwd_packed:
            if counters is not None or pack_args["seed_add"]:
                self._first_bump = (counters, pack_args["seed_add"])
            pack_args = None
        elif not (self.pack_overlap and train):
            self.pack(**pack_args)
            pack_args = None
        if self.marks is not None:
            self.marks.calib(self._stream())
        if self.fwd_route == PEER:
            self.peer.bump(self.xepoch, self._stream())
        return pack_args

    def _fwd_layer(self, s: ConvSpec, logits: torch.Tensor, track_running: bool):
        out = logits if s.name == "decoder.out_conv" else self.z[s.name]
        want_stats = bool(s.bn) and self.fwd_route != EVAL
        acc = want_stats and self.fwd_route == ACC
        if s.idx == 0:
# ... 163 lines not shown
        return self.N * ((su.h + t - 1) // t) * ((su.w + t - 1) // t)

    def _side_buf(self, pool: Dict[str, torch.Tensor], s: ConvSpec, c: int) -> torch.Tensor:
        if s.name not in pool:
            pool[s.name] = torch.empty(self.N, s.h, s.w, c, dtype=torch.float32, device=self.dev)
        return pool[s.name]

    @staticmethod
    def _side_layer(s: ConvSpec) -> bool:
        return s.taps == 9 and bool(s.h % 16 or s.w % 16)

    def _sums_from_epilogue(self, ca: L.ConvArgs, s: ConvSpec, kind: int, layer: str, dA: torch.Tensor, dA_ps: int, rows: Optional[int] = None):
        ca.bwd_stats, ca.bwd_of, ca.stat_partials = kind, self._act_dz(layer, dA, dA_ps), L.ptr(self.partials)
        if rows is None:
            rows = self.lib.hpfg_conv_stat_rows(C.byref(ca))
        if rows <= 0 or rows * 2 * s.cin > self.partials.numel():
            raise RuntimeError(f"backward of {s.name}: {rows} rows of backward sums of {layer} do not fit the partials workspace")
        if self.bwd_route == ACC:
            ca.stat_partials, ca.stat_acc, ca.stat_shards = None, L.ptr(self.accb_of[layer]), self.acc_shards[layer]
        self._fused_rows[layer] = rows
        if kind == 2:
            self._pool_done.add(layer)

    def _dx_args(self, ca: L.ConvArgs, s: ConvSpec, g: L.Act, out: Optional[torch.Tensor], out2: Optional[torch.Tensor]) -> L.ConvArgs:
        ca.a0, ca.math, ca.out = g, self.math, L.ptr(out)
        if out is not None:
            ca.wpk = L.ptr(self.wpk16_d[s.name]) if self._b16 else L.ptr(self.wpk_d[s.name])
        ca.out_pstride, ca.Cout, ca.CoutPad = s.cin, s.cin, s.cin_pad
        if out2 is not None:
            ca.out2, ca.out_split, ca.out_pstride, ca.out2_pstride = L.ptr(out2), s.cin // 2, s.cin // 2, s.cin // 2
        ca.N, ca.H, ca.W, ca.taps = self.N, s.h, s.w, s.taps
        return ca

    def _fused_bwd(self, s: ConvSpec, g: L.Act, out: torch.Tensor, stats_for: Optional[str], out2: Optional[torch.Tensor]):
        fa = L.FusedBwdArgs()
        fa.xa0, fa.xa1 = self.input_acts(s.name)
        fa.slab = L.ptr(self.slab_of[s.name])
        fa.Cin, fa.CinPad, fa.Cout, fa.CoutPad = s.cin, s.cin_pad, s.cout, s.cout_pad
        ca = self._dx_args(fa.d, s, g, out, out2)
        rows, grid = self.fused_grid[s.name], self.lib.hpfg_fused_bwd_grid(C.byref(fa))
        if grid != rows:
            raise RuntimeError(f"fused_bwd[{s.name}]: {grid} workgroups, {rows} weight-gradient slabs allocated")
        if stats_for is not None and self.fuse_bwd_stats and s.cin == s.cin_pad and out2 is None:
            self._sums_from_epilogue(ca, s, 1, stats_for, out, s.cin, rows)
        self._call(self.lib.hpfg_fused_bwd, C.byref(fa), tag="fused_bwd:" + s.name)

    def _wgrad(self, s: ConvSpec, g: L.Act, stream: Optional[int] = None):
        wa = L.WgradArgs()
        if s.name in self._act_live:
            wa.a0, wa.a1 = self._act_split(self.actbuf[s.name], s.cin, s.h, s.w), L.Act()
        else:
            wa.a0, wa.a1 = self.input_acts(s.name)
        wa.g = g
        wa.slab, wa.dw_oihw, wa.defer_reduce = L.ptr(self.slab_of[s.name]), L.ptr(self.grads[f"{s.name}.weight"]), 1
        wa.Cin, wa.CinPad, wa.Cout, wa.CoutPad = s.cin, s.cin_pad, s.cout, s.cout_pad
        wa.N, wa.H, wa.W, wa.taps = self.N, s.h, s.w, s.taps
        wa.S = self.lib.hpfg_wgrad_splits(self.N, s.h, s.w, s.cin_pad, s.cout_pad, s.taps)
        wa.math = self.math
        self._call(self.lib.hpfg_wgrad, C.byref(wa), tag="wgrad:" + s.name, stream=stream)

    def _dgrad(self, s: ConvSpec, g: L.Act, out: torch.Tensor, stats_for: Optional[str] = None, out2: Optional[torch.Tensor] = None,
               stage_out: Optional[torch.Tensor] = None, pool_of: Optional[str] = None, side_sums: Optional[torch.Tensor] = None):
        ca = self._dx_args(L.ConvArgs(), s, g, out, out2)
        if stage_out is not None:
            ca.stage_out = L.ptr(stage_out)
        if side_sums is not None:
            ca.side_sums = L.ptr(side_sums)
            rows = self.lib.hpfg_conv_stat_rows(C.byref(ca))
            if rows != self.csum_rows[s.name]:
                raise RuntimeError(f"dgrad[{s.name}]: {rows} workgroups, {self.csum_rows[s.name]} rows of bias-gradient sums allocated")
        spills = s.taps == 9 and s.cin_pad % 32 == 0 and s.h % 16 == 0 and s.w % 16 == 0
        fusable = self._b16 and self.fuse_bwd_stats and s.cin == s.cin_pad
        if stats_for is not None and fusable and (not spills or self.fuse_bwd_stats == 2):
            self._sums_from_epilogue(ca, s, 1, stats_for, out, s.cin)
        elif pool_of is not None and fusable and self._side_layer(s) and out2 is None:
            self._sums_from_epilogue(ca, s, 2, pool_of, self.dA[pool_of], self.dA_ps[pool_of])
        self._call(self.lib.hpfg_conv_fwd, C.byref(ca), tag="dgrad:" + s.name)

    def _slab_reduce(self, lo: int, hi: int, stream=None):
        if hi <= lo:
            return
        self._call(self.lib.hpfg_slab_reduce_multi, *self.slabs.sub(lo, hi), tag="slab_reduce", stream=stream)

    def _csum(self, dlogits: torch.Tensor, stream: Optional[int] = None):
        s = self.specs["decoder.out_conv"]
        self._call(self.lib.hpfg_channel_sum_partials, L.ptr(dlogits), self.ncls, self.N * s.h * s.w, self.ncls, L.ptr(self.csum_part[s.name]), tag="csum:" + s.name, stream=stream)

    def _flush_deferred(self, lo: int, hi: int):
        if self._deferred is None:
            return
        side = self._fork_side().cuda_stream
        if self._csum_pending is not None:
            self._csum(self._csum_pending, side)
            self._csum_pending = None
        batches = [(self._deferred, lo, hi)]
        if hi == self._n_enc_desc and lo + 2 < hi and len(self._deferred) == hi - lo:
            batches = [(self._deferred[:-2], lo + 2, hi), (self._deferred[-2:], lo, lo + 2)]
        for layers, a, b in batches:
            for s_, g_ in layers:
                self._wgrad(s_, g_, side)
            self._slab_reduce(a, b, side)
        self._side_used = True

    def _bwd_head(self, dlogits: torch.Tensor):
        s = self.specs["decoder.out_conv"]
        g = self._act_plain(dlogits, self.ncls, s.h, s.w)
        if self.marks is not None:
            self.marks.calib(self._stream())
        if self._deferred is None:
            self._csum(dlogits)
        else:
            self._csum_pending = dlogits
        self._wgrad_dgrad(s, g, self.dA["decoder.up4.conv.conv_conv.4"], "decoder.up4.conv.conv_conv.4")

    def _bwd_decoder_block(self, k: int, sole_consumer: bool):
        sp = self.specs
        p = f"decoder.up{k}.conv.conv_conv"
        s2, s1, su = sp[f"{p}.4"], sp[f"{p}.0"], sp[f"decoder.up{k}.conv1x1"]
        g2 = self._bn_backward(s2)
        self._wgrad_dgrad(s2, g2, self.dA[s1.name], s1.name)
        g1 = self._bn_backward(s1)
        c2 = su.cout
        self._wgrad_dgrad(s1, g1, self.dcat[k], out2=self.dup.get(k))
        if k in self.dup:
            dup, dup_ps = self.dup[k], c2
        else:
            dup, dup_ps = self.dcat[k].view(-1)[c2:], 2 * c2
        prev = enc_prefix(4) + ".4" if k == 1 else f"decoder.up{k - 1}.conv.conv_conv.4"
        stats_prev = prev if sole_consumer else None
        gu = self._act_plain(self.dU[k], c2, su.h, su.w)
        if self._upb_on(su):
            gsrc = L.Act()
            gsrc.z, gsrc.mode, gsrc.C, gsrc.Hs, gsrc.Ws, gsrc.pstride = L.ptr(dup), L.ACT_UPBWD, c2, su.h, su.w, dup_ps
            self._dgrad(su, gsrc, self.dA[prev], stats_prev, stage_out=self.dU[k], side_sums=self.csum_part[su.name])
            if self._deferred is not None:
                self._deferred.append((su, gu))
            else:
                self._wgrad(su, gu)
        else:
            self._call(self.lib.hpfg_upsample2x_bwd_sums, L.ptr(dup), dup_ps, L.ptr(self.dU[k]), self.N, su.h, su.w, c2, L.ptr(self.csum_part[su.name]), tag="upbwd:" + su.name)
            self._wgrad_dgrad(su, gu, self.dA[prev], stats_prev)

    def _bwd_encoder_level(self, lvl: int):
        p = enc_prefix(lvl)
        s2, s1 = self.specs[f"{p}.4"], self.specs[f"{p}.0"]
        g2 = self._bn_backward(s2, self.dP[lvl + 1] if (lvl < 4 and s2.name not in self._pool_done) else None)
        self._wgrad_dgrad(s2, g2, self.dA[s1.name], s1.name)
        g1 = self._bn_backward(s1)
        if lvl > 0:
            self._wgrad_dgrad(s1, g1, self.dP[lvl], pool_of=(enc_prefix(lvl - 1) + ".4") if self.pool_fuse else None)
        elif s1.name in self.fused_grid:
            self._fused_bwd(s1, g1, None, None, None)
        else:
            self._wgrad(s1, g1)

    def backward(self, dlogits: torch.Tensor, dfeat4: Optional[torch.Tensor] = None, bucket_cb=None):
        assert self.bwd_ready, "backward() needs a preceding train-mode forward()"
        assert dlogits.is_contiguous() and tuple(dlogits.shape) == (self.N, self.H, self.W, self.ncls)
        self._alloc_bwd()
        self.bwd_route = bn_route(True, self.math, self.bn_acc_on, self.peer is not None, self.world, self.force_sync)
        if self.bwd_route == ACC:
            if self._accb_dirty:
                self.accb_all.zero_()
            self._accb_dirty = True
        defer = bool(self.defer_wgrad and bucket_cb is None)
        self._deferred = [] if defer else None
        self._pool_done, self._csum_pending = set(), None
        self._bwd_head(dlogits)
        for k in range(4, 0, -1):
            self._bwd_decoder_block(k, sole_consumer=k > 1 or dfeat4 is None)
        if dfeat4 is not None:
            self.dA[enc_prefix(4) + ".4"].add_(dfeat4)
        self._flush_deferred(self._n_enc_desc, len(self.slabs.host))
        self._deferred = [] if defer else None
        if bucket_cb is not None:
            self._join_side()
            self._slab_reduce(self._n_enc_desc, len(self.slabs.host))
            self._finalize_bwd_all(self._n_enc_bn, len(self.bn_layers))
            bucket_cb(0)
        for lvl in range(4, -1, -1):
            self._bwd_encoder_level(lvl)
            if lvl == 2:
                self._flush_deferred(self._n_thin_enc_desc, self._n_enc_desc)
                self._deferred = None
        if defer:
            self._slab_reduce(0, self._n_thin_enc_desc)
        self._join_side()
        self._finalize_bwd_all(0, self._n_enc_bn if bucket_cb is not None else len(self.bn_layers))
        self._accb_dirty = False
        if bucket_cb is not None:
            self._slab_reduce(0, self._n_enc_desc)
            bucket_cb(1)
        elif not defer:
            self._slab_reduce(0, len(self.slabs.host))
        self.bwd_ready = False
```

### hpfg_amd/model/unet.py

```python
from __future__ import annotations

from collections import OrderedDict
from typing import Dict, List, Optional, Tuple

import torch
import torch.nn as nn

import os
import weakref

from .. import _lib as L
from .. import engine as E
from .. import heads

WIDTHS = E.WIDTHS

_INSTANCES = [0]


def reset_dropout_streams(count: int = 0) -> None:
    _INSTANCES[0] = int(count)


def _fresh_dropout_seed() -> int:
# ... 149 lines not shown
            ls = [(n, b) for n, b in self.named_buffers() if b.dtype == torch.long]
            fl = torch.stack([b.detach().reshape(()) for _, b in ls]).to(dev) if ls else torch.zeros(0, dtype=torch.long, device=dev)
            for i, (n, b) in enumerate(ls):
                b.data = fl[i]
        self._flat, self._flat_grad, self._flat_buf, self._flat_long = flat, flat_grad, fb, fl
        self._engines, self._last_engine = {}, None
        self._anchor = torch.zeros(1, device=dev, requires_grad=True)
        self._backbone_numel = sum(p.numel() for n, p in ps if n.startswith("encoder.") or n.startswith("decoder."))
        self._encoder_numel = sum(p.numel() for n, p in ps if n.startswith("encoder."))

    def _is_flat(self) -> bool:
        ps = list(self.parameters())
        if self._flat is None or not ps:
            return False
        first, last = ps[0], ps[-1]
        return (first.data_ptr() == self._flat.data_ptr() and
                last.data_ptr() == self._flat.data_ptr() + (self._flat.numel() - last.numel()) * 4)

    def _ensure_flat(self):
        if not self._is_flat():
            self._flatten()

    def _apply(self, fn, *a, **k):
        out = super()._apply(fn, *a, **k)
        self._flatten()
        return out

    def __deepcopy__(self, memo):
        cls = self.__class__
        new = cls.__new__(cls)
        nn.Module.__init__(new)
        import copy
        for k, v in self.__dict__.items():
            if k in ("_flat", "_flat_grad", "_flat_buf", "_flat_long", "_engines", "_last_engine", "_anchor", "dp"):
                continue
            new.__dict__[k] = copy.deepcopy(v, memo)
        new.dp = self.dp
        new.dropout_seed = _fresh_dropout_seed()
        new._flat = new._flat_grad = new._flat_buf = new._flat_long = None
        new._engines, new._anchor = {}, None
        new._flatten()
        return new

    def load_state_dict(self, *a, **k):
        out = super().load_state_dict(*a, **k)
        self._ensure_flat()
        self.mark_fragments_stale()
        return out

    def _weights_token(self) -> tuple:
        return (self.math, self._flat.data_ptr(), self._flat._version, sum(p._version for p in self.parameters()))

    def mark_fragments_stale(self):
        for pool in self.__dict__.get("_engines", {}).values():
            for e in pool:
                e.frag_token = None

    @property
    def flat_params(self) -> torch.Tensor:
        self._ensure_flat()
        return self._flat

    @property
    def flat_grads(self) -> torch.Tensor:
        self._ensure_flat()
        return self._flat_grad

    def grad_bucket(self, i: int) -> torch.Tensor:
        return self._flat_grad[self._encoder_numel:] if i == 0 else self._flat_grad[:self._encoder_numel]

    def backbone_numel(self) -> int:
        return self._backbone_numel

    def attach_grad_views(self):
        for n, p in self.named_parameters():
            if p.requires_grad:
                off, k = self._offsets[n]
                g = self._flat_grad[off:off + k].view(p.shape)
                if p.grad is None or p.grad.data_ptr() != g.data_ptr():
                    p.grad = g

    def zero_flat_grad(self):
        if getattr(self, "direct_grads", False):
            return
        self._flat_grad.zero_()

    def _next_seed(self):
        if getattr(self, "_graph_seed_mode", False):
            self._graph_fwds = getattr(self, "_graph_fwds", 0) + 1
            return E.SEED_BUMP
        self._seed_counter += 1
        return self._seed_counter

    def bump_graph_seed(self):
        self._seed_counter += getattr(self, "_fwds_per_replay", 0)

    def _acquire_engine(self, x: torch.Tensor) -> E.UNetEngine:
        if not x.is_cuda:
            raise RuntimeError("hpfg_amd.UNet runs on the HIP library only: move the input to the GPU (no CPU fallback)")
        self._ensure_flat()
        if x.device != self._flat.device:
            raise RuntimeError(f"input on {x.device} but parameters on {self._flat.device}")
        key = (tuple(x.shape), x.device.index)
        pool = self._engines.setdefault(key, [])
        direct = bool(getattr(self, "direct_grads", False))
        eng = next((e for e in pool if not e.bwd_ready and e.direct == direct), None)
        if eng is None and len(pool) >= 4:
            eng = next((e for e in pool if e.direct == direct), None)
        if eng is None:
            named = dict(self.named_parameters())
            params = {n: p.data for n, p in named.items()}
            bufs = {n: b.data for n, b in self.named_buffers()}
            gtmp = self._flat_grad if direct else torch.zeros_like(self._flat)
            grads = {n: gtmp[o:o + k].view(named[n].shape) for n, (o, k) in self._offsets.items()}
            eng = E.UNetEngine(params, bufs, grads, self.in_channels, self.num_classes, x.shape[0], x.shape[2], x.shape[3], x.device)
            eng.gtmp = gtmp
            eng.direct = direct
            pool.append(eng)
# ... 84 lines not shown
```

### hpfg_amd/train.py

```python
from __future__ import annotations

import contextlib
import ctypes as C
import math
import os
from typing import Dict, Optional

import numpy as np
import torch

from . import _lib as L
from .utils import (BoxMaskGenerator, build_lr_scheduler, build_optimizer, ema_alpha, linear_rampup, seg_loss, sigmoid_rampup,
                    update_ema_variables, update_ema_variables_backbone)
from .utils.loss import _nhwc
from .utils.optim import FusedSGD

S_LR1, S_LR2, S_ALPHA, S_THRESH, S_COEF_A, S_COEF_B = 0, 1, 2, 3, 8, 16


class StepScalars:

    SLOTS = 8

    def __init__(self, dev):
        self.host = torch.zeros(32, dtype=torch.float32)
        self.ring = torch.zeros(self.SLOTS, 32, dtype=torch.float32).pin_memory()
        self.events = [None] * self.SLOTS
        self.slot = 0
        self.dev = torch.zeros(32, dtype=torch.float32, device=dev)
        self.on_push = None

    def push(self):
        if self.on_push is not None:
            self.on_push()
        k = self.slot
        self.slot = (k + 1) % self.SLOTS
        if self.events[k] is not None:
            self.events[k].synchronize()
        self.ring[k].copy_(self.host)
        self.dev.copy_(self.ring[k], non_blocking=True)
        ev = self.events[k] or torch.cuda.Event()
        ev.record(torch.cuda.current_stream(self.dev.device))
        self.events[k] = ev

    def view(self, off, n=1):
# ... 111 lines not shown
        with torch.cuda.stream(stream):
            yield

    def _join(self, stream, *outs):
        cur = torch.cuda.current_stream(self.dev)
        cur.wait_stream(stream)
        for o in outs:
            for t_ in (o if isinstance(o, (tuple, list)) else (o,)):
                for u in (t_ if isinstance(t_, (tuple, list)) else (t_,)):
                    if torch.is_tensor(u):
                        u.record_stream(cur)

    def _teacher_forward(self, x, forked: bool = False):
        with (torch.cuda.stream(self.side) if forked else self._fork(self.side)), torch.no_grad():
            self._mark(2)
            out = self.ema_model(x)
            self._mark(3)
        return out

    def _backward(self, loss, stream):
        for o in self.optimizers:
            o.zero_grad()
        loss.backward()
        self._join(stream)

    def _attach(self, model, alone: bool = False):
        model.dp = self.dp
        model._alone = bool(alone)
        if alone:
            model.defer_wgrad = True
        if any(p.requires_grad for p in model.parameters()):
            model.direct_grads = True

    def _loss_backward(self, res):
        if getattr(self, "_g1", None) is None or self._g1.device != res.device:
            self._g1 = torch.zeros(res.numel(), dtype=res.dtype, device=res.device)
            self._g1[0] = 1.0
        res.backward(self._g1)

    def _reduce_grads(self, *models):
        if self.dp is not None and (self.dp.world_size > 1 or self.dp.force_sync):
            p2p = getattr(self.dp, "p2p_grads", False)
            red = self.dp.peer_allreduce_sum if p2p else self.dp.allreduce_sum
            for m in models:
                if getattr(m, "_buckets_launched", False):
                    m._buckets_launched = False
                    self.dp.join_buckets()
                elif hasattr(m, "flat_grads") and not hasattr(m, "_hpfg_generic_flat"):
                    red(m.flat_grads)
                elif getattr(m, "_hpfg_flat_optimizer", None) is not None:
                    opt = m._hpfg_flat_optimizer
                    assert opt.external_gather, "a flat-buffer optimizer under data parallel must be registered with _StepBase._own_gather"
                    red(opt.gather_flat_grads())
                else:
                    gs = [p.grad for p in m.parameters() if p.grad is not None]
                    flat = torch.cat([g.reshape(-1) for g in gs])
                    red(flat)
                    o = 0
                    for g in gs:
                        g.copy_(flat[o:o + g.numel()].view_as(g))
                        o += g.numel()

    def _own_gather(self, *optimizers):
        active = self.dp is not None and (self.dp.world_size > 1 or self.dp.force_sync)
        for o in optimizers:
            if hasattr(o, "external_gather"):
                o.external_gather = bool(active)

    def _set_grad_scale(self, *optimizers):
        if self.dp is not None and not getattr(self.dp, "sync_bn", True):
            for o in optimizers:
                o.grad_scale = 1.0 / self.dp.world_size

    @staticmethod
    def _lr(opt):
        lr = opt.param_groups[0]["lr"]
        return 0.0 if torch.is_tensor(lr) else float(lr)


class SupervisedStep(_StepBase):
    def __init__(self, model, args, dp=None):
        super().__init__(args, dp, [model])
        self.sc.host[S_COEF_A:S_COEF_A + 2] = torch.tensor([0.5, 0.5])

    def host_scalars(self, cur_itrs):
        self.sc.host[S_LR1] = self._lr(self.optimizer)

    def device_fwd_bwd(self, img, label):
        out = self.model(img)
        res = seg_loss(out, label, coef=self.sc.view(S_COEF_A, 8), dp=self.dp)
        self.optimizer.zero_grad()
        self._loss_backward(res)
        return {"loss": res[0].detach(), "logits": out.detach(), "parts": res.detach()}

    def step(self, img, label, cur_itrs):
        return self.eager_step((img, label), cur_itrs)


class _TeacherStudentStep(_StepBase):

    def __init__(self, model, ema_model, args, dp=None):
        super().__init__(args, dp, [model], ema_model)

    def host_scalars(self, cur_itrs, cons_w=None):
        w = self._cons_w(cur_itrs, cons_w)
        h = self.sc.host
        h[S_LR1] = self._lr(self.optimizer)
        h[S_ALPHA] = ema_alpha(cur_itrs, self.args.ema_decay)
        h[S_COEF_A:S_COEF_A + 5] = torch.tensor([0.5, 0.5, 0.0, 0.0, w])
        return w

    def device_update(self):
        fs, ft = getattr(self.model, "flat_params", None), getattr(self.ema_model, "flat_params", None)
        if isinstance(self.optimizer, FusedSGD) and fs is not None and ft is not None and fs.numel() == ft.numel() and fs.is_cuda:
            self.optimizer.step(push_lr=False, ema=(ft, fs.numel(), self.sc.view(S_ALPHA), self.ema_model))
        else:
            self.optimizer.step(push_lr=False)
            update_ema_variables(self.model, self.ema_model, self.args.ema_decay, 0, alpha_dev=self.sc.view(S_ALPHA))


class MeanTeacherStep(_TeacherStudentStep):
    def __init__(self, model, ema_model, args, dp=None):
        super().__init__(model, ema_model, args, dp)
        self.teacher_after = 7

    def device_fwd_bwd(self, label_img, target_label, unlabel_img):
        nl = label_img.shape[0]
        x = cat_batch(label_img, unlabel_img)
        self._mark(0)
        ev = torch.cuda.Event()
        ev.record(torch.cuda.current_stream(self.dev))
        self._mark(1)
        box = []

        def teacher():
            with torch.cuda.stream(self.side), torch.no_grad():
                self.side.wait_event(ev)
                self._mark(2)
                box.append(self.ema_model(x))
                self._mark(3)

        self.model._after_layer = (self.teacher_after, teacher)
        try:
            out = self.model(x)
        finally:
            self.model._after_layer = None
        if not box:
            teacher()
        t_out = box[0]
        self._mark(4)
        self._join(self.side, t_out)
        self._mark(5)
        res = seg_loss(out, target_label, nl, coef=self.sc.view(S_COEF_A, 8), teacher_logits=t_out, dp=self.dp)
        self.optimizer.zero_grad()
        self._loss_backward(res)
        self._mark(6)
        return {"loss": res[0].detach(), "parts": res.detach(), "logits": out.detach(), "t_logits": t_out}

    def device_update(self):
        super().device_update()
        self._mark(7)

    def step(self, label_img, target_label, unlabel_img, cur_itrs, cons_w=None):
        return self.eager_step((label_img, target_label, unlabel_img), cur_itrs, cons_w=cons_w)


def mix_samples(a: torch.Tensor, b: torch.Tensor, f: torch.Tensor) -> torch.Tensor:
    a, b, f = a.contiguous(), b.contiguous(), f.reshape(-1).float().contiguous()
    out = torch.empty_like(a)
    L.check(L.load().hpfg_mix_samples(L.ptr(a), L.ptr(b), L.ptr(f), L.ptr(out), a.shape[0], a[0].numel(),
                                      torch.cuda.current_stream(a.device).cuda_stream), "mix_samples")
    return out


def softmax_mix(t0: torch.Tensor, t1: torch.Tensor, f: torch.Tensor) -> torch.Tensor:
    x0, x1 = _nhwc(t0.detach()), _nhwc(t1.detach())
    n, H, W, Cc = x0.shape
    out = torch.empty(n, H, W, Cc, dtype=torch.float32, device=x0.device)
    L.check(L.load().hpfg_softmax_mix(L.ptr(x0), L.ptr(x1), L.ptr(f.reshape(-1).float().contiguous()), L.ptr(out), n, H, W, Cc,
                                      torch.cuda.current_stream(x0.device).cuda_stream), "softmax_mix")
    return out.permute(0, 3, 1, 2)


class ICTStep(_TeacherStudentStep):

    def draw_mix_factors(self, unlabel_bs: int, rng=None) -> torch.Tensor:
        rng = np.random if rng is None else rng
        a = float(getattr(self.args, "ict_alpha", 0.2))
# ... 709 lines not shown
```

### hpfg_amd/utils/__init__.py

```python
from .loss import DiceLoss, Med_Sup_Loss, Dense_Loss, seg_loss
from .optim import FusedAdamW, FusedSGD, build_lr_scheduler, build_optimizer, flatten_parameters
from .scheduler import CosineWarmupLR_Scheduler, Medical_LR, PolyLR
from .utils import (AttrDict, BoxMaskGenerator, ema_alpha, get_current_consistency_weight, linear_rampup, loadyaml, mk_path,
                    sigmoid_rampup, update_ema_variables, update_ema_variables_backbone)
from .logger import _get_logger
```

### hpfg_amd/utils/loss.py

```python
from __future__ import annotations

import ctypes as C
from typing import Optional, Sequence

import torch
import torch.nn as nn

from .. import _lib as L


def _nhwc(t: torch.Tensor) -> torch.Tensor:
    v = t.permute(0, 2, 3, 1)
    return v if v.is_contiguous() else v.contiguous()


def _labels_u8(t: Optional[torch.Tensor]) -> Optional[torch.Tensor]:
    if t is None:
        return None
    if t.dim() == 4:
        t = t[:, 0]
    if t.dtype != torch.uint8:
        t = t.to(torch.uint8)
    return t.contiguous()


class _SegLossFn(torch.autograd.Function):
    @staticmethod
    def forward(ctx, logits, coef, labels0, labels1, t_logits, n_lab, is_prob, dp, t_is_prob=False, cons_mask=None):
        lib = L.load()
        if not logits.is_cuda:
            raise RuntimeError("hpfg_amd losses run on the HIP library only (no CPU fallback)")
        if logits.shape[1] > L.LOSS_MAX_CLASSES:
            raise ValueError(f"seg_loss supports at most {L.LOSS_MAX_CLASSES} classes (got {logits.shape[1]})")
        x = _nhwc(logits.float())
        N, H, W, Cc = x.shape
        dev = x.device
        a = L.LossArgs()
        nblk = lib.hpfg_loss_blocks(N, H, W)
        nsum = lib.hpfg_loss_nsum(Cc)
        partials = torch.empty(nblk * nsum, dtype=torch.float32, device=dev)
        sums = torch.empty(nsum, dtype=torch.float32, device=dev)
        out = torch.empty(8, dtype=torch.float32, device=dev)
        t = _nhwc(t_logits.float()) if t_logits is not None else None
        a.logits, a.t_logits, a.labels0, a.labels1 = L.ptr(x), L.ptr(t), L.ptr(labels0), L.ptr(labels1)
        a.coef, a.partials, a.sums, a.out, a.dlogits = L.ptr(coef), L.ptr(partials), L.ptr(sums), L.ptr(out), None
        a.N, a.n_lab, a.H, a.W, a.C = N, n_lab, H, W, Cc
        if dp is not None and not getattr(dp, "sync_bn", True):
            dp = None
        a.world = dp.world_size if dp is not None else 1
        a.input_is_prob = 1 if is_prob else 0
        a.teacher_is_prob = 1 if t_is_prob else 0
        if t is not None:
            if t.shape[0] == N - n_lab and n_lab > 0:
                a.t_unlab_only = 1
            elif t.shape[0] != N:
                raise ValueError(f"consistency target has {t.shape[0]} images; expected {N} (whole batch) or {N - n_lab} (unlabelled part)")
        cm = None
        if cons_mask is not None:
            cm = cons_mask.float().reshape(-1).contiguous()
            if t is None or cm.numel() != (N - n_lab) * H * W:
                raise ValueError("cons_mask needs a consistency target and one weight per unlabelled pixel")
            a.cons_mask = L.ptr(cm)
        st = torch.cuda.current_stream(dev).cuda_stream
        if dp is not None and getattr(dp, "p2p", False) and (dp.world_size > 1 or dp.force_sync):
            slot, epoch = dp.next_loss_slot()
            dp.bump(epoch, st)
            px = dp.peer_desc(slot, epoch)
            L.check(lib.hpfg_seg_loss_partials_x(C.byref(a), C.byref(px), st), "seg_loss_partials_x")
        else:
            L.check(lib.hpfg_seg_loss_partials(C.byref(a), st), "seg_loss_partials")
            if dp is not None and (dp.world_size > 1 or dp.force_sync):
                dp.allreduce_sum(sums)
        L.check(lib.hpfg_seg_loss_finalize(C.byref(a), st), "seg_loss_finalize")
        ctx.args, ctx.keep = a, (x, t, labels0, labels1, coef, sums, cm)
        ctx.shape = (N, H, W, Cc)
        return out

    @staticmethod
    def backward(ctx, gout):
        lib = L.load()
        a = ctx.args
        N, H, W, Cc = ctx.shape
        x = ctx.keep[0]
        dl = torch.empty(N, H, W, Cc, dtype=torch.float32, device=x.device)
        a.dlogits = L.ptr(dl)
        gs = gout[0:1].contiguous()
        L.check(lib.hpfg_seg_loss_bwd(C.byref(a), L.ptr(gs), torch.cuda.current_stream(x.device).cuda_stream), "seg_loss_bwd")
        return dl.permute(0, 3, 1, 2), None, None, None, None, None, None, None, None, None


def seg_loss(logits: torch.Tensor, labels: Optional[torch.Tensor], n_lab: Optional[int] = None, *,
             coef: torch.Tensor, pseudo: Optional[torch.Tensor] = None, teacher_logits: Optional[torch.Tensor] = None,
             is_prob: bool = False, dp=None, teacher_prob: Optional[torch.Tensor] = None,
             cons_mask: Optional[torch.Tensor] = None) -> torch.Tensor:
    N = logits.shape[0]
    n_lab = N if n_lab is None else int(n_lab)
    if teacher_prob is not None:
        assert teacher_logits is None
        return _SegLossFn.apply(logits, coef, _labels_u8(labels), _labels_u8(pseudo), teacher_prob, n_lab, is_prob, dp, True, cons_mask)
    return _SegLossFn.apply(logits, coef, _labels_u8(labels), _labels_u8(pseudo), teacher_logits, n_lab, is_prob, dp, False, cons_mask)


def _coef(dev, vals: Sequence[float]) -> torch.Tensor:
    v = list(vals) + [0.0] * (8 - len(vals))
    return torch.tensor(v, dtype=torch.float32, device=dev)


class DiceLoss(nn.Module):

    def __init__(self, n_classes: int):
        super().__init__()
        self.n_classes = n_classes
        self._coef = {}

    def forward(self, inputs, target, weight=None, softmax=False):
        if weight is not None and any(w != 1 for w in weight):
            raise NotImplementedError("class weights are not used on the hot path")
        assert inputs.shape[1] == self.n_classes, "predict & target shape do not match"
        k = inputs.device
        if k not in self._coef:
            self._coef[k] = _coef(k, [0.0, 1.0])
        return seg_loss(inputs, target, coef=self._coef[k], is_prob=not softmax)[0]


class Med_Sup_Loss(nn.Module):
    def __init__(self, num_classes: int, ce: float = 0.5, dice: float = 0.5):
        super().__init__()
        self.num_classes, self.ce, self.dice = num_classes, ce, dice
        self._coef = {}

    def forward(self, outputs, target_label):
        k = outputs.device
        if k not in self._coef:
# ... 18 lines not shown
```

### include/hpfg_hip.h

```cpp
#ifndef HPFG_HIP_H
#define HPFG_HIP_H

#include <stdint.h>

#ifdef __cplusplus
extern "C" {
#endif

#define HPFG_VERSION 142
enum { HPFG_MATH_F32 = 0, HPFG_MATH_BF16X3 = 1 };

enum { HPFG_BN_MEAN = 0, HPFG_BN_RSTD = 1, HPFG_BN_SCALE = 2, HPFG_BN_SHIFT = 3,
       HPFG_BN_K1 = 4, HPFG_BN_K2 = 5, HPFG_BN_K3 = 6, HPFG_BN_SPARE = 7, HPFG_BN_ROWS = 8 };

enum {
  HPFG_ACT_NONE = 0,
  HPFG_ACT_PLAIN = 1,
  HPFG_ACT_STRIDED = 2,
  HPFG_ACT_BNACT = 3,
  HPFG_ACT_BNACT_POOL = 4,
  HPFG_ACT_UP2X = 5,
  HPFG_ACT_DZ = 6,
  HPFG_ACT_SPLIT16 = 7,
  HPFG_ACT_UPBWD = 8
};

typedef struct HpfgAct {
  const float* z;
  const float* bn;
  const float* aux;
  int32_t mode;
  int32_t C;
  int32_t Hs, Ws;
  int32_t pstride;
  int32_t aux_pstride;
  int32_t bn_stride;
  int32_t bn_coff;
  int32_t sn, sc, sy, sx;
  float drop_p;
  uint32_t drop_seed;
  const uint8_t* drop_mask;
  const uint32_t* seed_dev;
  const long long* bn_acc;
  const float* bn_gamma;
  const float* bn_beta;
  float bn_count;
  float bn_eps;
  int32_t bn_shards;
  int32_t reserved1;
} HpfgAct;

typedef struct HpfgConvArgs {
  HpfgAct a0, a1;
  const float* wpk;
  const float* bias;
  float* out;
  float* stat_partials;
  int32_t out_pstride, Cout, CoutPad;
  int32_t N, H, W;
  int32_t taps;
  int32_t math;
  int32_t bwd_stats;
  HpfgAct bwd_of;
  float* out2;
  int32_t out_split;
  int32_t out2_pstride;
  long long* stat_acc;
  int32_t stat_shards;
  int32_t reserved2;
  float* stage_out;
  float* side_sums;
} HpfgConvArgs;
#define HPFG_ACC_MAX_SHARDS 8
#define HPFG_ACC_WORDS(C, shards) ((shards) * 2 * 2 * (C))

typedef struct HpfgWgradArgs {
  HpfgAct a0, a1;
  HpfgAct g;
  float* slab;
  float* dw_oihw;
  int32_t Cin, CinPad, Cout, CoutPad;
  int32_t N, H, W, taps;
  int32_t S;
  int32_t math;
  int32_t defer_reduce;
} HpfgWgradArgs;

typedef struct HpfgFusedBwdArgs {
  HpfgConvArgs d;
  HpfgAct xa0, xa1;
  float* slab;
  int32_t Cin, CinPad, Cout, CoutPad;
} HpfgFusedBwdArgs;

typedef struct HpfgSlabDesc {
  const float* slab;
  float* dw_oihw;
  int32_t S, taps, Cin, CinPad, Cout, CoutPad;
} HpfgSlabDesc;

typedef struct HpfgPackDesc {
  const float* w_oihw;
  const float* b;
  float* wpk_fwd;
  float* wpk_dgrad;
  float* bias_pad;
  void* wpk16_fwd;
  void* wpk16_dgrad;
  int32_t Cout, Cin, CoutPad, CinPad, taps;
  int32_t kc;
} HpfgPackDesc;

int hpfg_version(void);
const char* hpfg_last_error(void);
enum { HPFG_OPT_CONV_THIN = 0, HPFG_OPT_FIRST_MFMA = 1, HPFG_OPT_FIRST_WGRAD = 2, HPFG_OPT_NARROW_DEEP = 3, HPFG_OPT_UPDATE_PACK = 4, HPFG_OPT_COUNT = 5 };
int hpfg_get_option(int which);
int hpfg_set_option(int which, int value);

int hpfg_conv3x3_first_fwd(const HpfgAct* x, const float* w_oihw, const float* bias, float* out, float* stat_partials,
                           int N, int H, int W, int Cin, int Cout, void* stream);
int hpfg_conv_first_rows(int N, int H, int W);
int hpfg_conv3x3_first_fwd_acc(const HpfgAct* x, const float* w_oihw, const float* bias, float* out, float* stat_partials, long long* stat_acc,
                               int stat_shards, int N, int H, int W, int Cin, int Cout, void* stream);
int hpfg_conv_fwd(const HpfgConvArgs* args, void* stream);
int hpfg_conv_stat_blocks(int N, int H, int W);
int hpfg_conv_stat_rows(const HpfgConvArgs* args);
int hpfg_bn_fwd_finalize(const float* partials, int nblk, const double* sums, double count, const float* gamma, const float* beta,
                         float* running_mean, float* running_var, float momentum, float eps, float* bn, int C, void* stream);
typedef struct HpfgBnAccDesc {
  const long long* acc;
  const float* gamma;
  const float* beta;
  float* running_mean;
  float* running_var;
  float* bn;
  int32_t C;
  float count;
  int32_t shards;
  int32_t reserved;
} HpfgBnAccDesc;
int hpfg_bn_acc_finalize(const HpfgBnAccDesc* table_dev, const HpfgBnAccDesc* table_host, int nlayers, float momentum, float eps, void* stream);
typedef struct HpfgBnAccBwdDesc {
  long long* acc;
  const float* gamma;
  float* bn;
  float* dgamma;
  float* dbeta;
  int32_t C;
// ... 70 lines not shown
  int32_t world, rank;
  int64_t slice;
  int64_t n;
  int64_t stride;
} HpfgPeerBuf;
long hpfg_peer_buf_slice(int world, long n);
long hpfg_peer_buf_bytes(int world, long n);
int hpfg_peer_allreduce_f32(const HpfgPeerBuf* pb, float* buf, void* stream);

typedef struct HpfgLossArgs {
  const float* logits;
  const float* t_logits;
  const uint8_t* labels0;
  const uint8_t* labels1;
  const float* coef;
  float* partials;
  float* sums;
  float* out;
  float* dlogits;
  int32_t N, n_lab, H, W, C;
  int32_t world;
  int32_t input_is_prob;
  int32_t teacher_is_prob;
  int32_t t_unlab_only;
  int32_t reserved0;
  const float* cons_mask;
} HpfgLossArgs;
#define HPFG_LOSS_NSUM 32
#define HPFG_LOSS_NSUM_WIDE 104
int hpfg_loss_blocks(int N, int H, int W);
int hpfg_loss_nsum(int C);
int hpfg_seg_loss_partials(const HpfgLossArgs* a, void* stream);
int hpfg_seg_loss_partials_x(const HpfgLossArgs* a, const HpfgPeerX* px, void* stream);
int hpfg_seg_loss_finalize(const HpfgLossArgs* a, void* stream);
int hpfg_seg_loss_bwd(const HpfgLossArgs* a, const float* grad_scale_dev , void* stream);
int hpfg_argmax_labels(const float* logits, int N, int H, int W, int C, const uint8_t* mix_labels, const float* mix_mask,
                       uint8_t* out, void* stream);
int hpfg_confusion_counts(const uint8_t* pred, const uint8_t* gt, long n, int C, unsigned long long* counts, void* stream);
#define HPFG_RESIZE_TAPS 36
int hpfg_resize_cubic(const float* src, int S, int h, int w, float* dst, int H, int W, const float* taps_y, const float* taps_x, void* scratch,
                      long scratch_bytes, void* stream);
long hpfg_resize_cubic_scratch_bytes(int S, int h, int w, int H, int W);
#define HPFG_SURFACE_SEGS 32
int hpfg_surface_counts(const uint8_t* pred, const uint8_t* gt, int S, int h, int w, int C, int ndim, unsigned int* counts, void* stream);
int hpfg_surface_distances(const uint8_t* pred, const uint8_t* gt, int S, int h, int w, int C, int ndim, const unsigned int* counts_host,
                           void* workspace, long workspace_bytes, void* stream);
long hpfg_surface_workspace_bytes(int C, long n_points);
int hpfg_surface_sums(const void* workspace, long workspace_bytes, int C, const unsigned int* counts_host, long long* sums, void* stream);
typedef struct HpfgAugSample {
  int64_t img_off, lab_off;
  int32_t h, w;
  int32_t mode;
  int32_t k, axis;
  int32_t tab_off;
  double m00, m01, m10, m11, off_y, off_x;
} HpfgAugSample;
int hpfg_augment_batch(const float* img_pool, const uint8_t* lab_pool, const HpfgAugSample* samples_dev, const int* tabs_dev, int B, int H, int W,
                       float* out_img, uint8_t* out_lab, void* stream);
int hpfg_box_masks(const int* rects, int n, int n_boxes, int H, int W, int invert, float* out, void* stream);
int hpfg_mix_samples(const float* a, const float* b, const float* f, float* out, int n, long per_sample, void* stream);
int hpfg_softmax_mix(const float* t0, const float* t1, const float* f, float* out_prob, int n, int H, int W, int C, void* stream);
int hpfg_timestamp(unsigned long long* slot, void* stream);
int hpfg_noise_add(const float* x, const float* noise, float* out, long n_src, long n_out, float scale, float lo, float hi, void* stream);
typedef struct HpfgPredBlocks {
  const float* p[8];
  int32_t n_blocks, per_block;
// ... 130 lines not shown
```

Before: 8002 images/s.

## Fuse seg-loss gradient into final-layer fused backward halo load

Adds an ACT_LOSSG source mode so the final conv's fused backward kernel computes the CE/Dice/MSE logit gradient on the fly while staging its halo, instead of running a separate loss_bwd pass. The loss partials are split into student and consistency parts so the teacher-dependent part and the finalize can run later, in the backward tail. The aim is to remove a full-resolution kernel launch and a round trip of dlogits through memory. The cost is extra per-pixel softmax work inside the conv kernel, per-class template instantiations, more complex Python autograd plumbing, and a risk of ordering bugs around when the sums are finalized.

```diff
diff --git a/hpfg_amd/_lib.py b/hpfg_amd/_lib.py
--- a/hpfg_amd/_lib.py
+++ b/hpfg_amd/_lib.py
@@ -8,12 +8,13 @@
 LIB_PATH = os.path.join(_HERE, "lib", "libhpfg_hip.so")
 
 BN_MEAN, BN_RSTD, BN_SCALE, BN_SHIFT, BN_K1, BN_K2, BN_K3, BN_SPARE, BN_ROWS = range(9)
-ACT_NONE, ACT_PLAIN, ACT_STRIDED, ACT_BNACT, ACT_BNACT_POOL, ACT_UP2X, ACT_DZ, ACT_SPLIT16, ACT_UPBWD = range(9)
-OPT_CONV_THIN, OPT_FIRST_MFMA, OPT_FIRST_WGRAD, OPT_NARROW_DEEP, OPT_UPDATE_PACK = 0, 1, 2, 3, 4
+ACT_NONE, ACT_PLAIN, ACT_STRIDED, ACT_BNACT, ACT_BNACT_POOL, ACT_UP2X, ACT_DZ, ACT_SPLIT16, ACT_UPBWD, ACT_LOSSG = range(10)
+OPT_CONV_THIN, OPT_FIRST_MFMA, OPT_FIRST_WGRAD, OPT_NARROW_DEEP, OPT_UPDATE_PACK, OPT_LOSS_ON_LOAD = 0, 1, 2, 3, 4, 5
 LOSS_NSUM = 32
 LOSS_MAX_CLASSES = 16
+LOSSG_MAX_CLASSES = 8
 ACC_MAX_SHARDS = 8
-VERSION = 142
+VERSION = 143
 RESIZE_TAPS = 36
 SURFACE_SEGS = 32
 MATH_F32, MATH_BF16X3 = 0, 1
@@ -56,9 +57,15 @@
                 ("slice", C.c_int64), ("n", C.c_int64), ("stride", C.c_int64)]
 
 
+class LossGrad(C.Structure):
+    _fields_ = [("t_logits", C.c_void_p), ("labels0", C.c_void_p), ("labels1", C.c_void_p), ("sums", C.c_void_p), ("coef", C.c_void_p),
+                ("grad_scale", C.c_void_p), ("dlogits", C.c_void_p), ("n_lab", C.c_int32), ("t_unlab_only", C.c_int32), ("world", C.c_int32),
+                ("reserved3", C.c_int32)]
+
+
 class FusedBwdArgs(C.Structure):
     _fields_ = [("d", ConvArgs), ("xa0", Act), ("xa1", Act), ("slab", C.c_void_p), ("Cin", C.c_int32), ("CinPad", C.c_int32),
-                ("Cout", C.c_int32), ("CoutPad", C.c_int32)]
+                ("Cout", C.c_int32), ("CoutPad", C.c_int32), ("lg", LossGrad)]
 
 
 class AugSample(C.Structure):
@@ -205,6 +212,7 @@
     "hpfg_loss_blocks": (_i, [_i, _i, _i]),
     "hpfg_loss_nsum": (_i, [_i]),
     "hpfg_seg_loss_partials": (_i, [C.POINTER(LossArgs), _p]),
+    "hpfg_seg_loss_partials_part": (_i, [C.POINTER(LossArgs), _i, _p]),
     "hpfg_seg_loss_finalize": (_i, [C.POINTER(LossArgs), _p]),
     "hpfg_seg_loss_bwd": (_i, [C.POINTER(LossArgs), _p, _p]),
     "hpfg_argmax_labels": (_i, [_p, _i, _i, _i, _i, _p, _p, _p, _p]),
@@ -260,6 +268,12 @@
 
 _lock = threading.Lock()
 _lib = None
+LAUNCH_LOG = None
+
+
+def log_launch(tag: str, stream):
+    if LAUNCH_LOG is not None:
+        LAUNCH_LOG.append((tag, int(stream)))
 
 
 def load() -> C.CDLL:
@@ -286,6 +300,8 @@
             lib.hpfg_set_option(OPT_NARROW_DEEP, int(os.environ["HPFG_NARROW_DEEP"]))
         if os.environ.get("HPFG_UPDATE_PACK", "1") == "0":
             lib.hpfg_set_option(OPT_UPDATE_PACK, 0)
+        if os.environ.get("HPFG_LOSS_ON_LOAD", "1") == "0":
+            lib.hpfg_set_option(OPT_LOSS_ON_LOAD, 0)
         _lib = lib
     return _lib
 
diff --git a/hpfg_amd/csrc/common.h b/hpfg_amd/csrc/common.h
--- a/hpfg_amd/csrc/common.h
+++ b/hpfg_amd/csrc/common.h
@@ -322,7 +322,7 @@
 }
 
 
-enum { HPFG_KIND_PLAIN = 0, HPFG_KIND_BNACT = 1, HPFG_KIND_POOL = 2, HPFG_KIND_CAT = 3, HPFG_KIND_DZ = 4, HPFG_KIND_SPLIT = 5, HPFG_KIND_UPB = 6 };
+enum { HPFG_KIND_PLAIN = 0, HPFG_KIND_BNACT = 1, HPFG_KIND_POOL = 2, HPFG_KIND_CAT = 3, HPFG_KIND_DZ = 4, HPFG_KIND_SPLIT = 5, HPFG_KIND_UPB = 6, HPFG_KIND_LOSSG = 7 };
 
 template <int MODE>
 __device__ static inline f32x4 act_load4_mode(const HpfgAct& s, const ActCtx& cx, int n, int y, int x, int c) {
@@ -388,6 +388,7 @@
     case HPFG_ACT_DZ: return HPFG_KIND_DZ;
     case HPFG_ACT_SPLIT16: return HPFG_KIND_SPLIT;
     case HPFG_ACT_UPBWD: return HPFG_KIND_UPB;
+    case HPFG_ACT_LOSSG: return HPFG_KIND_LOSSG;
     default: return -1;
   }
 }
diff --git a/hpfg_amd/csrc/conv.hip b/hpfg_amd/csrc/conv.hip
--- a/hpfg_amd/csrc/conv.hip
+++ b/hpfg_amd/csrc/conv.hip
@@ -294,6 +294,7 @@
     HPFG_ARG_CHECK(a->bwd_stats == 1 || (a->taps == 9 && (a->H % 16 || a->W % 16) && a->bwd_of.aux && a->bwd_of.aux_pstride % 4 == 0 && a->bwd_of.drop_p == 0.f && !a->out_split),
                    "conv_fwd: bwd_stats == 2 (max-pool backward in the epilogue) needs a 3x3 dgrad at a size that is not a multiple of 16, bwd_of.aux (the gradient so far) and no dropout behind bwd_of");
   }
+  HPFG_ARG_CHECK(a->a0.mode != HPFG_ACT_LOSSG && a->a1.mode != HPFG_ACT_LOSSG, "conv_fwd: an HPFG_ACT_LOSSG source is read by hpfg_fused_bwd only");
   if ((a->math & 0xff) == HPFG_MATH_BF16X3) {
     {
       const int r = hpfg_conv_thin_try(*a, st, rows_only);
diff --git a/hpfg_amd/csrc/fused_bwd.hip b/hpfg_amd/csrc/fused_bwd.hip
--- a/hpfg_amd/csrc/fused_bwd.hip
+++ b/hpfg_amd/csrc/fused_bwd.hip
@@ -2,6 +2,7 @@
 
 int hpfg_first_wgrad_grid(int N, int H, int W);
 int hpfg_first_wgrad_launch(const HpfgAct& g, const HpfgAct& x, float* slab, int Cin, int N, int H, int W, hipStream_t st);
+int hpfg_fused_bwd_lossg(const HpfgFusedBwdArgs& a, hipStream_t st, bool grid_only);
 
 namespace {
 
@@ -44,6 +45,7 @@
   }
   HPFG_FUSED_CASE(1, 1, HPFG_KIND_BNACT, HPFG_KIND_DZ, 4, 2, 1, 1)
   HPFG_FUSED_CASE(1, 1, HPFG_KIND_BNACT, HPFG_KIND_PLAIN, 4, 2, 1, 1)
+  if (ci == 1 && co == 1 && ak == HPFG_KIND_BNACT && gk == HPFG_KIND_LOSSG) return hpfg_fused_bwd_lossg(a, st, grid_only);
   HPFG_FUSED_CASE(1, 2, HPFG_KIND_POOL, HPFG_KIND_DZ, 8, 1, 1, 0)
   HPFG_FUSED_CASE(2, 2, HPFG_KIND_BNACT, HPFG_KIND_DZ, 8, 1, 2, 1)
   HPFG_FUSED_CASE(2, 1, HPFG_KIND_CAT, HPFG_KIND_DZ, 8, 1, 2, 1)
@@ -76,7 +78,15 @@
   HPFG_ARG_CHECK(a->slab && d.a0.z && (wonly ? (!d.wpk && !d.bwd_stats && !d.out2) : d.wpk != nullptr), "fused_bwd: slab and the dZ source are required; wpk with out");
   HPFG_ARG_CHECK(d.Cout == a->Cin && d.CoutPad == a->CinPad && d.a0.C == a->Cout && a->xa0.C + a->xa1.C == a->Cin,
                  "fused_bwd: the dgrad side must describe the same layer (d.Cout == Cin, d.a0.C == Cout, input channels == Cin)");
-  HPFG_ARG_CHECK((wonly || a->Cin % 8 == 0) && (a->Cout % 8 == 0 || d.a0.mode == HPFG_ACT_PLAIN || d.a0.mode == HPFG_ACT_STRIDED), "fused_bwd: Cin (and Cout behind a DZ source) must be multiples of 8");
+  HPFG_ARG_CHECK((wonly || a->Cin % 8 == 0) && (a->Cout % 8 == 0 || d.a0.mode == HPFG_ACT_PLAIN || d.a0.mode == HPFG_ACT_STRIDED || d.a0.mode == HPFG_ACT_LOSSG),
+                 "fused_bwd: Cin (and Cout behind a DZ source) must be multiples of 8");
+  if (d.a0.mode == HPFG_ACT_LOSSG) {
+    const HpfgLossGrad& g = a->lg;
+    HPFG_ARG_CHECK(!wonly && d.a0.C >= 2 && d.a0.C <= 8 && d.a0.pstride == d.a0.C && d.a0.Hs == d.H && d.a0.Ws == d.W,
+                   "fused_bwd: a LOSSG source is the logits [N][H][W][C] of 2 .. 8 classes (got C %d, pstride %d)", d.a0.C, d.a0.pstride);
+    HPFG_ARG_CHECK(g.sums && g.coef && g.dlogits && g.world >= 1 && g.n_lab >= 0 && g.n_lab <= d.N && (g.n_lab == 0 || g.labels0),
+                   "fused_bwd: a LOSSG source needs lg.sums, lg.coef, lg.dlogits, 0 <= n_lab <= N and labels0 with n_lab > 0");
+  }
 #ifndef HPFG_TRACE
   HPFG_ARG_CHECK(!d.bias, "fused_bwd: the dgrad side takes no bias");
 #endif
diff --git a/hpfg_amd/csrc/fused_bwd_kernel.h b/hpfg_amd/csrc/fused_bwd_kernel.h
--- a/hpfg_amd/csrc/fused_bwd_kernel.h
+++ b/hpfg_amd/csrc/fused_bwd_kernel.h
@@ -22,7 +22,7 @@
 struct Geo : Halves<CI, AK> {
   using Halves<CI, AK>::NA0;
   using Halves<CI, AK>::NA1;
-  static constexpr int TABD = GK == HPFG_KIND_DZ ? 5 * 16 * CO * 4 : 0;
+  static constexpr int TABD = GK == HPFG_KIND_DZ ? 5 * 16 * CO * 4 : (GK == HPFG_KIND_LOSSG ? LOSSG_TAB * 4 : 0);
   static constexpr int TABA = 2 * 16 * NA0 * 4;
   static constexpr int STAT = 2 * NW * 16 * CI * 4;
   static constexpr int KS = 5 * CO;
@@ -36,11 +36,12 @@
   static constexpr int LDS = OFF_U + NA1 * UBYTES;
 };
 
-template <int CI, int CO, int AK, int GK, bool BWD, int NW, int WGS, int PFA, int PFPOS, int BMAX = 48, bool NODG = false>
+template <int CI, int CO, int AK, int GK, bool BWD, int NW, int WGS, int PFA, int PFPOS, int BMAX = 48, bool NODG = false, int NCLS = 0>
 __global__ __launch_bounds__(64 * NW, WGS) void fused_bwd_kernel(HpfgFusedBwdArgs p, int tiles_x, int tiles_y) {
   using C = Cfg<16, 16, 4, 1, CI, 9, 16>;
   using G = Geo<CI, CO, AK, GK, NW, BWD, BMAX>;
   static_assert(!BWD || AK == HPFG_KIND_BNACT, "the backward sums of the layer below need its raw output as this layer's input");
+  static_assert((GK == HPFG_KIND_LOSSG) == (NCLS > 0) && (NCLS == 0 || (CO == 1 && NW == 4)), "a LOSSG source: one chunk of NCLS <= 8 classes");
   using SP = Split<NW>;
   constexpr int AK0 = G::AK0, NA0 = G::NA0, NA1 = G::NA1, NTH = SP::NTH, ND = SP::ND, NA = SP::NA, MI = SP::MI;
   __shared__ __attribute__((aligned(16))) unsigned char lds[G::LDS];
@@ -60,6 +61,7 @@
   const HpfgAct& aD = p.d.a0;
   const HpfgAct aS = skip_source<G::CATK>(p.xa0);
   const ActCtx cxg = make_ctx(aD), cxa = make_ctx(aS);
+  const LossgSrc lq = lossg_src(aD, p.lg);
 #ifdef HPFG_TRACE
   const bool tr_on = (p.d.math & 0x2000) && tid == 0;
   unsigned long long* tr_buf = reinterpret_cast<unsigned long long*>(const_cast<float*>(p.d.bias)) + 256 * (long)blockIdx.x;
@@ -70,6 +72,7 @@
   const int gsel = tid & 1;
 
   if (GK == HPFG_KIND_DZ) fill_tables_lds<GK, 16 * CO>(aD, tabD, 16 * CO, tid, NTH);
+  if constexpr (GK == HPFG_KIND_LOSSG) fill_lossg_table<NCLS>(tabD, p.lg, p.d.N, H, W, tid);
   fill_tables_lds<AK0, 16 * NA0, false>(aS, tabA, 16 * NA0, tid, NTH);
 
   constexpr int NIJ = CI * CO;
@@ -115,7 +118,9 @@
 
   auto issue = [&](auto early_tag, int n, int ty0, int tx0, bool live) {
     constexpr bool EARLY = decltype(early_tag)::value;
-    if (EARLY) {
+    if constexpr (GK == HPFG_KIND_LOSSG) {
+      if (EARLY) issue_halo_lossg<NCLS, NTH>(rawD[0], lq, n, ty0, tx0, H, W, tid, live);
+    } else if (EARLY) {
 #pragma unroll
       for (int c = 0; c < CO; ++c) {
         const int c0 = c * 16 + gsel * 8;
@@ -153,12 +158,16 @@
     const int n = w / ntiles, ty0 = ((w % ntiles) / tiles_x) * T, tx0 = ((w % ntiles) % tiles_x) * T;
     if (PFA < CI) issue(std::false_type{}, n, ty0, tx0, true);
     HPFG_TR(3)
-#pragma unroll
-    for (int c = 0; c < CO; ++c) {
-      const int c0 = c * 16 + gsel * 8;
-      Tab tg;
-      load_tables_lds<GK, 16 * CO>(tg, tabD, aD, c0);
-      stage_halo<GK, NTH>(ldsD + c * DCH, rawD[c], tg, aD, cxg, n, ty0, tx0, H, W, tid, c0, c0 < aD.C);
+    if constexpr (GK == HPFG_KIND_LOSSG) {
+      stage_halo_lossg<NCLS, NTH>(ldsD, rawD[0], tabD, lq, n, ty0, tx0, H, W, tid);
+    } else {
+#pragma unroll
+      for (int c = 0; c < CO; ++c) {
+        const int c0 = c * 16 + gsel * 8;
+        Tab tg;
+        load_tables_lds<GK, 16 * CO>(tg, tabD, aD, c0);
+        stage_halo<GK, NTH>(ldsD + c * DCH, rawD[c], tg, aD, cxg, n, ty0, tx0, H, W, tid, c0, c0 < aD.C);
+      }
     }
 #pragma unroll
     for (int c = 0; c < NA0; ++c) {
diff --git a/hpfg_amd/csrc/fused_bwd_lossg.hip b/hpfg_amd/csrc/fused_bwd_lossg.hip
--- /dev/null
+++ b/hpfg_amd/csrc/fused_bwd_lossg.hip
@@ -0,0 +1,34 @@
+#include "fused_bwd_kernel.h"
+
+namespace {
+
+using namespace hpfg_fused;
+
+template <int NC>
+int launch(const HpfgFusedBwdArgs& a, hipStream_t st, bool grid_only) {
+  constexpr int AK = HPFG_KIND_BNACT, GK = HPFG_KIND_LOSSG, NW = 4, WGS = 2, PFA = 1, PFPOS = 1, BMAX = 32;
+  const int grid = fused_grid<1, 1, AK, GK, NW, WGS, BMAX>(a);
+  if (grid_only) return grid;
+  const int tx = a.d.W / T, ty = a.d.H / T;
+  if (a.d.stat_acc) HPFG_ACC_CHECK(grid, a.d.stat_shards, "fused_bwd");
+  if (a.d.bwd_stats)
+    hipLaunchKernelGGL((fused_bwd_kernel<1, 1, AK, GK, true, NW, WGS, PFA, PFPOS, BMAX, false, NC>), dim3(grid), dim3(64 * NW), 0, st, a, tx, ty);
+  else
+    hipLaunchKernelGGL((fused_bwd_kernel<1, 1, AK, GK, false, NW, WGS, PFA, PFPOS, BMAX, false, NC>), dim3(grid), dim3(64 * NW), 0, st, a, tx, ty);
+  return hipGetLastError() == hipSuccess ? 0 : -1;
+}
+
+}
+
+int hpfg_fused_bwd_lossg(const HpfgFusedBwdArgs& a, hipStream_t st, bool grid_only) {
+  switch (a.d.a0.C) {
+    case 2: return launch<2>(a, st, grid_only);
+    case 3: return launch<3>(a, st, grid_only);
+    case 4: return launch<4>(a, st, grid_only);
+    case 5: return launch<5>(a, st, grid_only);
+    case 6: return launch<6>(a, st, grid_only);
+    case 7: return launch<7>(a, st, grid_only);
+    case 8: return launch<8>(a, st, grid_only);
+    default: return grid_only ? 0 : -2;
+  }
+}
diff --git a/hpfg_amd/csrc/loss.hip b/hpfg_amd/csrc/loss.hip
--- a/hpfg_amd/csrc/loss.hip
+++ b/hpfg_amd/csrc/loss.hip
@@ -1,59 +1,13 @@
 #include <string.h>
 #include "common.h"
+#include "loss_px.h"
 #include "peer.h"
 
 namespace {
 
+using namespace hpfg_loss;
+
 constexpr int PIX_PER_BLOCK = 1024;
-constexpr float SMOOTH = 1e-5f;
-constexpr int OFF_I0 = 8;
-constexpr int stride_of(int C) { return C <= 4 ? 4 : 16; }
-constexpr int nsum_of(int C) { return OFF_I0 + 6 * stride_of(C); }
-static_assert(nsum_of(4) == HPFG_LOSS_NSUM && nsum_of(5) == HPFG_LOSS_NSUM_WIDE && nsum_of(16) == HPFG_LOSS_NSUM_WIDE, "sums layout");
-
-template <int C>
-__device__ inline void load_px(const float* base, long pix, float* l) {
-  if (C % 4 == 0) {
-    const f32x4* b = reinterpret_cast<const f32x4*>(base + pix * C);
-#pragma unroll
-    for (int j = 0; j < C / 4; ++j) {
-      f32x4 v = b[j];
-      l[4 * j] = v[0]; l[4 * j + 1] = v[1]; l[4 * j + 2] = v[2]; l[4 * j + 3] = v[3];
-    }
-  } else {
-#pragma unroll
-    for (int c = 0; c < C; ++c) l[c] = base[pix * C + c];
-  }
-}
-
-template <int C>
-__device__ inline void store_px(float* base, long pix, const float* g) {
-  if (C % 4 == 0) {
-    f32x4* b = reinterpret_cast<f32x4*>(base + pix * C);
-#pragma unroll
-    for (int j = 0; j < C / 4; ++j) b[j] = f32x4{g[4 * j], g[4 * j + 1], g[4 * j + 2], g[4 * j + 3]};
-  } else {
-#pragma unroll
-    for (int c = 0; c < C; ++c) base[pix * C + c] = g[c];
-  }
-}
-
-template <int C>
-__device__ inline void softmax_w(const float* l, float* p, float& m, float& se) {
-  m = l[0];
-#pragma unroll
-  for (int c = 1; c < C; ++c) m = fmaxf(m, l[c]);
-  se = 0.f;
-#pragma unroll
-  for (int c = 0; c < C; ++c) {
-    p[c] = expf(l[c] - m);
-    se += p[c];
-  }
-  const float inv = 1.f / se;
-#pragma unroll
-  for (int c = 0; c < C; ++c) p[c] *= inv;
-}
-
 __device__ inline float wave_sum(float v) {
 #pragma unroll
   for (int o = 32; o >= 1; o >>= 1) v += __shfl_xor(v, o);
@@ -160,9 +114,9 @@
   for (int i = tid; i < NS; i += 256) a.partials[(long)blockIdx.x * NS + i] = red[0][i] + red[1][i] + red[2][i] + red[3][i];
 }
 
-__global__ __launch_bounds__(256) void loss_reduce_kernel(const float* __restrict__ partials, int nblk, int ns, float* __restrict__ sums, HpfgPeerX px) {
+__global__ __launch_bounds__(256) void loss_reduce_kernel(const float* __restrict__ partials, int nblk, int ns, int first, float* __restrict__ sums, HpfgPeerX px) {
   __shared__ double sh[4];
-  const int i = blockIdx.x;
+  const int i = first + blockIdx.x;
   double v = 0.0;
   for (int b = threadIdx.x; b < nblk; b += 256) v += (double)partials[(long)b * ns + i];
 #pragma unroll
@@ -208,81 +162,36 @@
 
 template <int C>
 __global__ __launch_bounds__(256) void loss_bwd_kernel(HpfgLossArgs a, long npix_img, const float* __restrict__ gscale_dev) {
-  constexpr int S = stride_of(C), CW = 16;
   __shared__ float cA[2][CW], cB[2][CW];
   const float gscale = gscale_dev ? *gscale_dev : 1.f;
   const float* s = a.sums;
   const float* k = a.coef;
   const long total = (long)a.N * npix_img;
   const long pb = (long)a.n_lab * npix_img;
-  const float cnt_mse = (float)((double)(a.N - a.n_lab) * a.H * a.W * C * a.world);
+  const float cnt_mse = mse_count(a.N, a.n_lab, a.H, a.W, C, a.world);
   if (threadIdx.x < 2 * CW) {
     const int g = threadIdx.x / CW, c = threadIdx.x % CW;
-    float ca = 0.f, cb = 0.f;
-    if (c < C) {
-      const int base = OFF_I0 + g * 3 * S;
-      const float wd = k[2 * g + 1] / (float)C;
-      const float den = s[base + S + c] + s[base + 2 * S + c] + SMOOTH;
-      const float num = 2.f * s[base + c] + SMOOTH;
-      ca = -2.f * wd / den;
-      cb = 2.f * wd * num / (den * den);
-    }
-    cA[g][c] = ca;
-    cB[g][c] = cb;
-  }
-  __syncthreads();
-  const float wm = cnt_mse > 0.f ? k[4] * 2.f / (a.cons_mask ? 2.f * s[5] + 1e-16f : cnt_mse) : 0.f;
+    grad_coef<C>(s, k, g, c, cA[g][c], cB[g][c]);
+  }
+  __syncthreads();
+  const float wm = grad_wm(s, k, cnt_mse, a.cons_mask != nullptr);
   for (long pix = blockIdx.x * 256L + threadIdx.x; pix < total; pix += (long)gridDim.x * 256) {
     const int grp = pix < pb ? 0 : 1;
-    float l[C], p[C], dp[C], m, se;
+    float l[C], tl[C], g[C];
     load_px<C>(a.logits, pix, l);
-    if (a.input_is_prob) {
-#pragma unroll
-      for (int c = 0; c < C; ++c) p[c] = l[c];
-    } else {
-      softmax_w<C>(l, p, m, se);
-    }
-#pragma unroll
-    for (int c = 0; c < C; ++c) dp[c] = 0.f;
     const uint8_t* lab = grp == 0 ? a.labels0 : a.labels1;
     int t = 255;
-    if (lab) {
-      t = grp == 0 ? lab[pix] : lab[pix - pb];
-      const float* ga = cA[grp];
-      const float* gb = cB[grp];
-#pragma unroll
-      for (int c = 0; c < C; ++c) {
-        const float tc = (t == c) ? 1.f : 0.f;
-        dp[c] += ga[c] * tc + gb[c] * p[c];
-      }
-    }
-    if (grp == 1 && a.t_logits) {
-      float q[C], tl[C], tm, ts;
+    if (lab) t = grp == 0 ? lab[pix] : lab[pix - pb];
+    const bool cons = grp == 1 && a.t_logits;
+    float w = wm;
+#pragma unroll
+    for (int c = 0; c < C; ++c) tl[c] = 0.f;
+    if (cons) {
       const long upix = pix - pb;
       load_px<C>(a.t_logits, a.t_unlab_only ? upix : pix, tl);
-      if (a.teacher_is_prob) {
-#pragma unroll
-        for (int c = 0; c < C; ++c) q[c] = tl[c];
-      } else {
-        softmax_w<C>(tl, q, tm, ts);
-      }
-      const float w = a.cons_mask ? wm * a.cons_mask[upix] : wm;
-#pragma unroll
-      for (int c = 0; c < C; ++c) dp[c] += w * (p[c] - q[c]);
-    }
-    float dot = 0.f;
-#pragma unroll
-    for (int c = 0; c < C; ++c) dot += p[c] * dp[c];
-    const float cn = s[2 * grp + 1];
-    const float wc = k[2 * grp];
-    const bool ce_on = lab && t != 255 && t < C && cn > 0.f;
-    float g[C];
-#pragma unroll
-    for (int c = 0; c < C; ++c) {
-      g[c] = a.input_is_prob ? dp[c] : p[c] * (dp[c] - dot);
-      if (ce_on && !a.input_is_prob) g[c] += wc * (p[c] - (t == c ? 1.f : 0.f)) / cn;
-      g[c] *= gscale;
-    }
+      if (a.cons_mask) w = wm * a.cons_mask[upix];
+    }
+    grad_px<C>(g, l, tl, t, lab != nullptr, cons, cA[grp], cB[grp], w, s[2 * grp + 1], k[2 * grp], gscale, a.input_is_prob != 0, a.teacher_is_prob != 0);
     store_px<C>(a.dlogits, pix, g);
   }
 }
@@ -310,19 +219,35 @@
   return 0;
 }
 
-static int loss_partials_impl(const HpfgLossArgs* a, const HpfgPeerX* px, void* stream) {
-  if (int rc = check_loss(a)) return rc;
+static int loss_partials_impl(const HpfgLossArgs* a, const HpfgPeerX* px, int first, int count, void* stream) {
   HPFG_ARG_CHECK(a->partials, "seg_loss_partials: workspace missing");
   const int nblk = hpfg_loss_blocks(a->N, a->H, a->W), ns = nsum_of(a->C);
   const long npix = (long)a->H * a->W;
   HPFG_LOSS_DISPATCH(a->C, hipLaunchKernelGGL(loss_partials_kernel<C>, dim3(nblk), dim3(256), 0, (hipStream_t)stream, *a, npix));
   HpfgPeerX none;
   memset(&none, 0, sizeof(none));
-  hipLaunchKernelGGL(loss_reduce_kernel, dim3(ns), dim3(256), 0, (hipStream_t)stream, a->partials, nblk, ns, a->sums, px ? *px : none);
+  hipLaunchKernelGGL(loss_reduce_kernel, dim3(count < 0 ? ns : count), dim3(256), 0, (hipStream_t)stream, a->partials, nblk, ns, first, a->sums, px ? *px : none);
   return hpfg_launch_status("loss_partials_kernel");
 }
 
-extern "C" int hpfg_seg_loss_partials(const HpfgLossArgs* a, void* stream) { return loss_partials_impl(a, nullptr, stream); }
+extern "C" int hpfg_seg_loss_partials(const HpfgLossArgs* a, void* stream) {
+  if (int rc = check_loss(a)) return rc;
+  return loss_partials_impl(a, nullptr, 0, -1, stream);
+}
+
+extern "C" int hpfg_seg_loss_partials_part(const HpfgLossArgs* a, int part, void* stream) {
+  HPFG_ARG_CHECK(a && a->logits && a->coef && a->sums, "seg_loss_partials_part: null pointer");
+  HPFG_ARG_CHECK(part == 0 || part == 1, "seg_loss_partials_part: part must be 0 (student sums) or 1 (consistency sums)");
+  if (part == 0) {
+    if (int rc = check_loss(a)) return rc;
+    HPFG_ARG_CHECK(!a->t_logits && !a->cons_mask, "seg_loss_partials_part: the student part takes no consistency target");
+    return loss_partials_impl(a, nullptr, 0, -1, stream);
+  }
+  HPFG_ARG_CHECK(a->C >= 2 && a->C <= 16, "seg_loss: C must be 2..16 (got %d)", a->C);
+  HPFG_ARG_CHECK(a->N > 0 && a->n_lab >= 0 && a->n_lab <= a->N && a->H > 0 && a->W > 0 && a->world >= 1, "seg_loss: bad sizes");
+  HPFG_ARG_CHECK(a->t_logits && !a->labels0 && !a->labels1, "seg_loss_partials_part: the consistency part takes t_logits and no labels");
+  return loss_partials_impl(a, nullptr, 4, 2, stream);
+}
 
 extern "C" int hpfg_seg_loss_partials_x(const HpfgLossArgs* a, const HpfgPeerX* px, void* stream) {
   HPFG_ARG_CHECK(px, "seg_loss_partials_x: null exchange descriptor");
@@ -333,7 +258,7 @@
                    "seg_loss_partials_x: bad exchange descriptor");
     for (int r = 0; r < px->world; ++r) HPFG_ARG_CHECK(px->mbox[r], "seg_loss_partials_x: mailbox of rank %d not mapped", r);
   }
-  return loss_partials_impl(a, px, stream);
+  return loss_partials_impl(a, px, 0, -1, stream);
 }
 
 extern "C" int hpfg_seg_loss_finalize(const HpfgLossArgs* a, void* stream) {
diff --git a/hpfg_amd/csrc/loss_px.h b/hpfg_amd/csrc/loss_px.h
--- /dev/null
+++ b/hpfg_amd/csrc/loss_px.h
@@ -0,0 +1,126 @@
+#pragma once
+#include "common.h"
+
+namespace hpfg_loss {
+
+constexpr float SMOOTH = 1e-5f;
+constexpr int OFF_I0 = 8;
+constexpr int CW = 16;
+constexpr int stride_of(int C) { return C <= 4 ? 4 : 16; }
+constexpr int nsum_of(int C) { return OFF_I0 + 6 * stride_of(C); }
+static_assert(nsum_of(4) == HPFG_LOSS_NSUM && nsum_of(5) == HPFG_LOSS_NSUM_WIDE && nsum_of(16) == HPFG_LOSS_NSUM_WIDE, "sums layout");
+
+template <int C>
+__device__ inline void load_px(const float* base, long pix, float* l) {
+  if (C % 4 == 0) {
+    const f32x4* b = reinterpret_cast<const f32x4*>(base + pix * C);
+#pragma unroll
+    for (int j = 0; j < C / 4; ++j) {
+      f32x4 v = b[j];
+      l[4 * j] = v[0]; l[4 * j + 1] = v[1]; l[4 * j + 2] = v[2]; l[4 * j + 3] = v[3];
+    }
+  } else {
+#pragma unroll
+    for (int c = 0; c < C; ++c) l[c] = base[pix * C + c];
+  }
+}
+
+template <int C>
+__device__ inline void store_px(float* base, long pix, const float* g) {
+  if (C % 4 == 0) {
+    f32x4* b = reinterpret_cast<f32x4*>(base + pix * C);
+#pragma unroll
+    for (int j = 0; j < C / 4; ++j) b[j] = f32x4{g[4 * j], g[4 * j + 1], g[4 * j + 2], g[4 * j + 3]};
+  } else {
+#pragma unroll
+    for (int c = 0; c < C; ++c) base[pix * C + c] = g[c];
+  }
+}
+
+template <int C>
+__device__ inline void softmax_w(const float* l, float* p, float& m, float& se) {
+  m = l[0];
+#pragma unroll
+  for (int c = 1; c < C; ++c) m = fmaxf(m, l[c]);
+  se = 0.f;
+#pragma unroll
+  for (int c = 0; c < C; ++c) {
+    p[c] = expf(l[c] - m);
+    se += p[c];
+  }
+  const float inv = 1.f / se;
+#pragma unroll
+  for (int c = 0; c < C; ++c) p[c] *= inv;
+}
+
+template <int C>
+__device__ __forceinline__ void grad_coef(const float* s, const float* k, int g, int c, float& ca, float& cb) {
+#pragma clang fp contract(off)
+  constexpr int S = stride_of(C);
+  ca = 0.f;
+  cb = 0.f;
+  if (c < C) {
+    const int base = OFF_I0 + g * 3 * S;
+    const float wd = k[2 * g + 1] / (float)C;
+    const float den = s[base + S + c] + s[base + 2 * S + c] + SMOOTH;
+    const float num = fmaf(2.f, s[base + c], SMOOTH);
+    ca = -2.f * wd / den;
+    cb = 2.f * wd * num / (den * den);
+  }
+}
+
+__device__ __forceinline__ float mse_count(int N, int n_lab, int H, int W, int C, int world) {
+  return (float)((double)(N - n_lab) * H * W * C * world);
+}
+__device__ __forceinline__ float grad_wm(const float* s, const float* k, float cnt_mse, bool masked) {
+#pragma clang fp contract(off)
+  return cnt_mse > 0.f ? k[4] * 2.f / (masked ? fmaf(2.f, s[5], 1e-16f) : cnt_mse) : 0.f;
+}
+
+template <int C>
+__device__ __forceinline__ void grad_px(float* g, const float* l, const float* tl, int t, bool has_lab, bool cons, const float* ga, const float* gb,
+                                        float w, float cn, float wc, float gscale, bool input_is_prob, bool teacher_is_prob) {
+#pragma clang fp contract(off)
+  constexpr int KF = C > 8 ? C - 8 : 0;
+  float p[C], dp[C], m, se;
+  if (input_is_prob) {
+#pragma unroll
+    for (int c = 0; c < C; ++c) p[c] = l[c];
+  } else {
+    softmax_w<C>(l, p, m, se);
+  }
+#pragma unroll
+  for (int c = 0; c < C; ++c) dp[c] = 0.f;
+  if (has_lab) {
+#pragma unroll
+    for (int c = 0; c < C; ++c) {
+      const float tc = (t == c) ? 1.f : 0.f;
+      dp[c] += ga[c] * tc + gb[c] * p[c];
+    }
+  } else {
+    t = 255;
+  }
+  if (cons) {
+    float q[C], tm, ts;
+    if (teacher_is_prob) {
+#pragma unroll
+      for (int c = 0; c < C; ++c) q[c] = tl[c];
+    } else {
+      softmax_w<C>(tl, q, tm, ts);
+    }
+#pragma unroll
+    for (int c = 0; c < C; ++c) dp[c] = fmaf(w, p[c] - q[c], dp[c]);
+  }
+  float dot = 0.f;
+#pragma unroll
+  for (int c = 0; c < C; ++c) dot = c < KF ? fmaf(p[c], dp[c], dot) : dot + p[c] * dp[c];
+  const bool ce_on = has_lab && t != 255 && t < C && cn > 0.f;
+#pragma unroll
+  for (int c = 0; c < C; ++c) {
+    g[c] = input_is_prob ? dp[c] : p[c] * (dp[c] - dot);
+    if (ce_on && !input_is_prob) g[c] += wc * (p[c] - (t == c ? 1.f : 0.f)) / cn;
+    g[c] *= gscale;
+  }
+}
+
+}
diff --git a/hpfg_amd/csrc/misc.hip b/hpfg_amd/csrc/misc.hip
--- a/hpfg_amd/csrc/misc.hip
+++ b/hpfg_amd/csrc/misc.hip
@@ -12,7 +12,7 @@
 extern "C" const char* hpfg_last_error(void) { return g_err; }
 extern "C" int hpfg_version(void) { return HPFG_VERSION; }
 
-static int g_opt[HPFG_OPT_COUNT] = {1, 1, 1, 128, 1};
+static int g_opt[HPFG_OPT_COUNT] = {1, 1, 1, 128, 1, 1};
 int hpfg_opt(int which) { return which >= 0 && which < HPFG_OPT_COUNT ? g_opt[which] : 0; }
 extern "C" int hpfg_get_option(int which) { return hpfg_opt(which); }
 extern "C" int hpfg_set_option(int which, int value) {
diff --git a/hpfg_amd/csrc/stage.h b/hpfg_amd/csrc/stage.h
--- a/hpfg_amd/csrc/stage.h
+++ b/hpfg_amd/csrc/stage.h
@@ -1,5 +1,6 @@
 #pragma once
 #include "common.h"
+#include "loss_px.h"
 
 namespace hpfg_stage {
 
@@ -64,7 +65,7 @@
 }
 
 template <int KIND>
-struct RawCount { static constexpr int N = KIND == HPFG_KIND_POOL || KIND == HPFG_KIND_CAT ? 8 : (KIND == HPFG_KIND_DZ ? 4 : 2); };
+struct RawCount { static constexpr int N = KIND == HPFG_KIND_POOL || KIND == HPFG_KIND_CAT ? 8 : (KIND == HPFG_KIND_DZ || KIND == HPFG_KIND_LOSSG ? 4 : 2); };
 
 template <int KIND>
 struct RawPiece {
@@ -331,6 +332,87 @@
   }
 }
 
+struct LossgSrc {
+  const float* logits;
+  const float* t_logits;
+  const uint8_t* labels0;
+  const uint8_t* labels1;
+  float* dlogits;
+  int n_lab, t_unlab_only, H, W;
+};
+__device__ __forceinline__ LossgSrc lossg_src(const HpfgAct& a, const HpfgLossGrad& g) {
+  return LossgSrc{a.z, g.t_logits, g.labels0, g.labels1, g.dlogits, g.n_lab, g.t_unlab_only, a.Hs, a.Ws};
+}
+constexpr int LOSSG_CB = 2 * hpfg_loss::CW, LOSSG_SC = 4 * hpfg_loss::CW, LOSSG_TAB = LOSSG_SC + 8;
+template <int NC>
+__device__ __forceinline__ void fill_lossg_table(float* t, const HpfgLossGrad& g, int N, int H, int W, int tid) {
+  using namespace hpfg_loss;
+  if (tid < 2 * CW) {
+    const int grp = tid / CW, c = tid % CW;
+    grad_coef<NC>(g.sums, g.coef, grp, c, t[grp * CW + c], t[LOSSG_CB + grp * CW + c]);
+  } else if (tid == 2 * CW) {
+    t[LOSSG_SC + 0] = grad_wm(g.sums, g.coef, mse_count(N, g.n_lab, H, W, NC, g.world), false);
+    t[LOSSG_SC + 1] = g.sums[1];
+    t[LOSSG_SC + 2] = g.sums[3];
+    t[LOSSG_SC + 3] = g.coef[0];
+    t[LOSSG_SC + 4] = g.coef[2];
+    t[LOSSG_SC + 5] = g.grad_scale ? *g.grad_scale : 1.f;
+  }
+}
+template <int NC>
+__device__ __forceinline__ void lossg_pack(const float* l, f32x4& a, f32x4& b) {
+#pragma unroll
+  for (int c = 0; c < NC; ++c) {
+    if (c < 4) a[c] = l[c];
+    else b[c - 4] = l[c];
+  }
+}
+template <int NC>
+__device__ __forceinline__ void lossg_unpack(float* l, const f32x4& a, const f32x4& b) {
+#pragma unroll
+  for (int c = 0; c < NC; ++c) l[c] = c < 4 ? a[c] : b[c - 4];
+}
+template <int NC>
+__device__ __forceinline__ void issue_piece_lossg(RawPiece<HPFG_KIND_LOSSG>& rp, const LossgSrc& q, int n, int gy, int gx, bool ok) {
+  static_assert(NC >= 2 && NC <= 8, "a LOSSG piece is the classes of one pixel in one 8-channel group");
+#pragma unroll
+  for (int i = 0; i < 4; ++i) rp.v[i] = f32x4{0.f, 0.f, 0.f, 0.f};
+  rp.dm[0] = 255u;
+  rp.dm[1] = 0u;
+  if (ok) {
+    const long pix = ((long)n * q.H + gy) * q.W + gx, pb = (long)q.n_lab * q.H * q.W;
+    const bool g1 = n >= q.n_lab;
+    float l[NC];
+    hpfg_loss::load_px<NC>(q.logits, pix, l);
+    lossg_pack<NC>(l, rp.v[0], rp.v[1]);
+    const uint8_t* lab = g1 ? q.labels1 : q.labels0;
+    if (lab) rp.dm[0] = lab[g1 ? pix - pb : pix];
+    if (g1 && q.t_logits) {
+      float tl[NC];
+      hpfg_loss::load_px<NC>(q.t_logits, q.t_unlab_only ? pix - pb : pix, tl);
+      lossg_pack<NC>(tl, rp.v[2], rp.v[3]);
+    }
+  }
+}
+template <int NC>
+__device__ __forceinline__ void finish_piece_lossg(f32x4& v0, f32x4& v1, const RawPiece<HPFG_KIND_LOSSG>& rp, const float* tab, const LossgSrc& q, int n,
+                                                   int gy, int gx, bool ok, bool store) {
+  v0 = f32x4{0.f, 0.f, 0.f, 0.f};
+  v1 = v0;
+  if (ok) {
+    const int grp = n < q.n_lab ? 0 : 1;
+    float l[NC], tl[NC], g[NC];
+    lossg_unpack<NC>(l, rp.v[0], rp.v[1]);
+    lossg_unpack<NC>(tl, rp.v[2], rp.v[3]);
+    const bool has_lab = (grp ? q.labels1 : q.labels0) != nullptr;
+    hpfg_loss::grad_px<NC>(g, l, tl, (int)rp.dm[0], has_lab, grp == 1 && q.t_logits != nullptr, tab + grp * hpfg_loss::CW,
+                           tab + LOSSG_CB + grp * hpfg_loss::CW, tab[LOSSG_SC], tab[LOSSG_SC + 1 + grp], tab[LOSSG_SC + 3 + grp], tab[LOSSG_SC + 5],
+                           false, false);
+    lossg_pack<NC>(g, v0, v1);
+    if (store) hpfg_loss::store_px<NC>(q.dlogits, ((long)n * q.H + gy) * q.W + gx, g);
+  }
+}
+
 template <int KIND>
 __device__ __forceinline__ void split_piece(const f32x4& v0, const f32x4& v1, bf16x8& hi, bf16x8& lo) {
   if (KIND == HPFG_KIND_SPLIT) {
diff --git a/hpfg_amd/csrc/tile16.h b/hpfg_amd/csrc/tile16.h
--- a/hpfg_amd/csrc/tile16.h
+++ b/hpfg_amd/csrc/tile16.h
@@ -90,4 +90,40 @@
   }
 }
 
+template <int NTH>
+constexpr int halo_pixels() { return (HP * HP + NTH - 1) / NTH; }
+template <int NC, int NTH>
+__device__ __forceinline__ void issue_halo_lossg(RawPiece<HPFG_KIND_LOSSG> (&raw)[halo_pieces<NTH>()], const LossgSrc& q, int n, int ty0, int tx0, int H,
+                                                 int W, int tid, bool live) {
+  static_assert(halo_pixels<NTH>() <= halo_pieces<NTH>(), "the pixel pieces fit the kernel's piece array");
+#pragma unroll
+  for (int i = 0; i < halo_pixels<NTH>(); ++i) {
+    const int pix = tid + i * NTH;
+    const int gy = ty0 + pix / HP - 1, gx = tx0 + pix % HP - 1;
+    issue_piece_lossg<NC>(raw[i], q, n, gy, gx, live && pix < HP * HP && gy >= 0 && gy < H && gx >= 0 && gx < W);
+  }
 }
+template <int NC, int NTH>
+__device__ __forceinline__ void stage_halo_lossg(unsigned char* chunk, const RawPiece<HPFG_KIND_LOSSG> (&raw)[halo_pieces<NTH>()], const float* tab,
+                                                 const LossgSrc& q, int n, int ty0, int tx0, int H, int W, int tid) {
+#pragma unroll
+  for (int i = 0; i < halo_pixels<NTH>(); ++i) {
+    const int pix = tid + i * NTH, py = pix / HP, px = pix % HP;
+    const int gy = ty0 + py - 1, gx = tx0 + px - 1;
+    const bool ok = pix < HP * HP && gy >= 0 && gy < H && gx >= 0 && gx < W;
+    f32x4 v0, v1;
+    finish_piece_lossg<NC>(v0, v1, raw[i], tab, q, n, gy, gx, ok, py >= 1 && py <= T && px >= 1 && px <= T);
+    if (pix < HP * HP) {
+      bf16x8 hi, lo;
+      split8(v0, v1, hi, lo);
+      const bf16x8 zero = __builtin_bit_cast(bf16x8, f32x4{0.f, 0.f, 0.f, 0.f});
+      unsigned char* o = chunk + (py * RS + px) * 32;
+      *reinterpret_cast<bf16x8*>(o) = hi;
+      *reinterpret_cast<bf16x8*>(o + 16) = zero;
+      *reinterpret_cast<bf16x8*>(o + PL) = lo;
+      *reinterpret_cast<bf16x8*>(o + PL + 16) = zero;
+    }
+  }
+}
+
+}
diff --git a/hpfg_amd/csrc/wgrad.hip b/hpfg_amd/csrc/wgrad.hip
--- a/hpfg_amd/csrc/wgrad.hip
+++ b/hpfg_amd/csrc/wgrad.hip
@@ -154,7 +154,7 @@
   HPFG_ARG_CHECK(a->a1.mode == HPFG_ACT_NONE || a->a0.C % 16 == 0, "wgrad: concat needs a0.C %% 16 == 0");
   hipStream_t st = (hipStream_t)stream;
   const int akind = hpfg_kind_of(a->a0, a->a1);
-  HPFG_ARG_CHECK(akind >= 0 && akind != HPFG_KIND_DZ, "wgrad: unsupported input source (a0.mode=%d, a1.mode=%d)", a->a0.mode, a->a1.mode);
+  HPFG_ARG_CHECK(akind >= 0 && akind != HPFG_KIND_DZ && akind != HPFG_KIND_LOSSG && a->g.mode != HPFG_ACT_LOSSG, "wgrad: unsupported input source (a0.mode=%d, a1.mode=%d)", a->a0.mode, a->a1.mode);
   int rc = 1;
   const bool b16 = (a->math & 0xff) == HPFG_MATH_BF16X3 && a->taps == 9;
   if ((a->math & 0xff) == HPFG_MATH_BF16X3 && a->taps == 1 && (a->g.mode == HPFG_ACT_PLAIN || a->g.mode == HPFG_ACT_STRIDED) && a->g.C % 4 == 0)
diff --git a/hpfg_amd/engine.py b/hpfg_amd/engine.py
--- a/hpfg_amd/engine.py
+++ b/hpfg_amd/engine.py
@@ -209,6 +209,7 @@
         self.defer_wgrad = False
         self._deferred: Optional[list] = None
         self._csum_pending: Optional[torch.Tensor] = None
+        self.loss_grad, self._loss_tail, self._logits_ptr = None, None, 0
         self.fused_grid: Dict[str, int] = {}
         self._side, self._side_used = None, False
         self.force_sync = False
@@ -226,6 +227,8 @@
 
         def launch():
             L.check(fn(*args, st), f"{fn.__name__}[{tag}]" if tag else fn.__name__)
+        if tag is not None:
+            L.log_launch(tag, st)
         if tag is None or self.marks is None:
             return launch()
         self.marks.bracket(tag, st, launch)
@@ -233,6 +236,13 @@
     @property
     def _b16(self) -> bool:
         return self.math == L.MATH_BF16X3
+
+    def loss_on_load_ok(self, logits_nhwc: torch.Tensor) -> bool:
+        if not (self.bwd_ready and self._b16 and self.ncls <= L.LOSSG_MAX_CLASSES and logits_nhwc.data_ptr() == self._logits_ptr and
+                tuple(logits_nhwc.shape) == (self.N, self.H, self.W, self.ncls)):
+            return False
+        self._alloc_bwd()
+        return "decoder.out_conv" in self.fused_grid
 
     def _fork_side(self) -> torch.cuda.Stream:
         if self._side is None:
@@ -384,6 +394,7 @@
                 seed_step: Optional[int] = None, needs_grad: bool = True) -> torch.Tensor:
         pack_args = self._fwd_begin(x, train, dropout, seed_step, needs_grad)
         logits = torch.empty(self.N, self.H, self.W, self.ncls, dtype=torch.float32, device=self.dev)
+        self._logits_ptr = logits.data_ptr()
         for i, s in enumerate(self.order):
             if i == 0 and pack_args is not None:
                 main = torch.cuda.current_stream(self.dev)
@@ -404,6 +415,7 @@
     def _fwd_begin(self, x: torch.Tensor, train: bool, dropout: Optional[bool], seed_step: Optional[int], needs_grad: bool) -> Optional[dict]:
         assert x.is_cuda and x.dtype == torch.float32 and tuple(x.shape) == (self.N, self.in_ch, self.H, self.W), (x.shape, x.dtype, x.device)
         self.x = x
+        self.loss_grad = None
         self._act_live = set()
         self._stage_inputs = bool(train and needs_grad and self.act_side and self._b16)
         self.dropout_on = train if dropout is None else dropout
@@ -633,12 +645,14 @@
         ca.N, ca.H, ca.W, ca.taps = self.N, s.h, s.w, s.taps
         return ca
 
-    def _fused_bwd(self, s: ConvSpec, g: L.Act, out: torch.Tensor, stats_for: Optional[str], out2: Optional[torch.Tensor]):
+    def _fused_bwd(self, s: ConvSpec, g: L.Act, out: torch.Tensor, stats_for: Optional[str], out2: Optional[torch.Tensor], loss_grad=None):
         fa = L.FusedBwdArgs()
         fa.xa0, fa.xa1 = self.input_acts(s.name)
         fa.slab = L.ptr(self.slab_of[s.name])
         fa.Cin, fa.CinPad, fa.Cout, fa.CoutPad = s.cin, s.cin_pad, s.cout, s.cout_pad
         ca = self._dx_args(fa.d, s, g, out, out2)
+        if loss_grad is not None:
+            loss_grad.fill(fa)
         rows, grid = self.fused_grid[s.name], self.lib.hpfg_fused_bwd_grid(C.byref(fa))
         if grid != rows:
             raise RuntimeError(f"fused_bwd[{s.name}]: {grid} workgroups, {rows} weight-gradient slabs allocated")
@@ -691,6 +705,9 @@
         if self._deferred is None:
             return
         side = self._fork_side().cuda_stream
+        if self._loss_tail is not None:
+            self._loss_tail.tail(side)
+            self._loss_tail = None
         if self._csum_pending is not None:
             self._csum(self._csum_pending, side)
             self._csum_pending = None
@@ -708,11 +725,27 @@
         g = self._act_plain(dlogits, self.ncls, s.h, s.w)
         if self.marks is not None:
             self.marks.calib(self._stream())
+        lg, self.loss_grad = self.loss_grad, None
+        if lg is not None and (lg.dlogits is None or lg.dlogits.data_ptr() != dlogits.data_ptr()):
+            raise RuntimeError("backward of decoder.out_conv: the loss gradient was left to be formed on load, but dlogits is not the tensor "
+                               "the loss handed over -- the logits have a second consumer; call seg_loss without on_load")
+        if lg is not None and s.name not in self.fused_grid:
+            lg.fallback(self._stream())
+            lg, tail = None, lg
+        else:
+            tail = lg
+        if lg is not None:
+            self._fused_bwd(s, g, self.dA["decoder.up4.conv.conv_conv.4"], "decoder.up4.conv.conv_conv.4", None, loss_grad=lg)
+            lg.consumed = True
         if self._deferred is None:
+            if tail is not None:
+                tail.tail(self._stream())
             self._csum(dlogits)
         else:
             self._csum_pending = dlogits
-        self._wgrad_dgrad(s, g, self.dA["decoder.up4.conv.conv_conv.4"], "decoder.up4.conv.conv_conv.4")
+            self._loss_tail = tail
+        if lg is None:
+            self._wgrad_dgrad(s, g, self.dA["decoder.up4.conv.conv_conv.4"], "decoder.up4.conv.conv_conv.4")
 
     def _bwd_decoder_block(self, k: int, sole_consumer: bool):
         sp = self.specs
@@ -766,7 +799,7 @@
             self._accb_dirty = True
         defer = bool(self.defer_wgrad and bucket_cb is None)
         self._deferred = [] if defer else None
-        self._pool_done, self._csum_pending = set(), None
+        self._pool_done, self._csum_pending, self._loss_tail = set(), None, None
         self._bwd_head(dlogits)
         for k in range(4, 0, -1):
             self._bwd_decoder_block(k, sole_consumer=k > 1 or dfeat4 is None)
diff --git a/hpfg_amd/model/unet.py b/hpfg_amd/model/unet.py
--- a/hpfg_amd/model/unet.py
+++ b/hpfg_amd/model/unet.py
@@ -205,7 +205,7 @@
         nn.Module.__init__(new)
         import copy
         for k, v in self.__dict__.items():
-            if k in ("_flat", "_flat_grad", "_flat_buf", "_flat_long", "_engines", "_last_engine", "_anchor", "dp"):
+            if k in ("_flat", "_flat_grad", "_flat_buf", "_flat_long", "_engines", "_last_engine", "_anchor", "dp", "_loss_grad"):
                 continue
             new.__dict__[k] = copy.deepcopy(v, memo)
         new.dp = self.dp
@@ -257,6 +257,26 @@
         if getattr(self, "direct_grads", False):
             return
         self._flat_grad.zero_()
+
+    def loss_on_load_ok(self, logits_nhwc: torch.Tensor) -> bool:
+        eng = getattr(self, "_last_engine", None)
+        return bool(eng is not None and self.training and not getattr(self, "_loss_grad", None) and eng.loss_on_load_ok(logits_nhwc))
+
+    def expect_loss_on_load(self, desc):
+        self._loss_grad = desc
+        self._last_engine.loss_grad = desc
+
+    def finish_loss_on_load(self):
+        desc, self._loss_grad = getattr(self, "_loss_grad", None), None
+        if desc is None:
+            return
+        eng = getattr(self, "_last_engine", None)
+        if eng is not None and eng.loss_grad is desc:
+            eng.loss_grad = None
+        st = torch.cuda.current_stream(desc.keep[0].device).cuda_stream
+        if not desc.consumed and desc.dlogits is not None:
+            desc.fallback(st)
+        desc.tail(st)
 
     def _next_seed(self):
         if getattr(self, "_graph_seed_mode", False):
diff --git a/hpfg_amd/train.py b/hpfg_amd/train.py
--- a/hpfg_amd/train.py
+++ b/hpfg_amd/train.py
@@ -10,7 +10,7 @@
 import torch
 
 from . import _lib as L
-from .utils import (BoxMaskGenerator, build_lr_scheduler, build_optimizer, ema_alpha, linear_rampup, seg_loss, sigmoid_rampup,
+from .utils import (BoxMaskGenerator, build_lr_scheduler, build_optimizer, ema_alpha, linear_rampup, loss_on_load_ok, seg_loss, sigmoid_rampup,
                     update_ema_variables, update_ema_variables_backbone)
 from .utils.loss import _nhwc
 from .utils.optim import FusedSGD
@@ -188,11 +188,18 @@
         if any(p.requires_grad for p in model.parameters()):
             model.direct_grads = True
 
-    def _loss_backward(self, res):
+    def _loss_backward(self, res, on_load=None):
         if getattr(self, "_g1", None) is None or self._g1.device != res.device:
             self._g1 = torch.zeros(res.numel(), dtype=res.dtype, device=res.device)
             self._g1[0] = 1.0
-        res.backward(self._g1)
+        try:
+            res.backward(self._g1)
+        finally:
+            if on_load is not None:
+                on_load.finish_loss_on_load()
+
+    def _on_load(self, model, out, teacher_logits=None):
+        return model if getattr(self, "loss_on_load", False) and loss_on_load_ok(model, out, teacher_logits, self.dp) else None
 
     def _reduce_grads(self, *models):
         if self.dp is not None and (self.dp.world_size > 1 or self.dp.force_sync):
@@ -238,15 +245,17 @@
     def __init__(self, model, args, dp=None):
         super().__init__(args, dp, [model])
         self.sc.host[S_COEF_A:S_COEF_A + 2] = torch.tensor([0.5, 0.5])
+        self.loss_on_load = False
 
     def host_scalars(self, cur_itrs):
         self.sc.host[S_LR1] = self._lr(self.optimizer)
 
     def device_fwd_bwd(self, img, label):
         out = self.model(img)
-        res = seg_loss(out, label, coef=self.sc.view(S_COEF_A, 8), dp=self.dp)
+        ol = self._on_load(self.model, out)
+        res = seg_loss(out, label, coef=self.sc.view(S_COEF_A, 8), dp=self.dp, on_load=ol)
         self.optimizer.zero_grad()
-        self._loss_backward(res)
+        self._loss_backward(res, ol)
         return {"loss": res[0].detach(), "logits": out.detach(), "parts": res.detach()}
 
     def step(self, img, label, cur_itrs):
@@ -279,6 +288,7 @@
     def __init__(self, model, ema_model, args, dp=None):
         super().__init__(model, ema_model, args, dp)
         self.teacher_after = 7
+        self.loss_on_load = True
 
     def device_fwd_bwd(self, label_img, target_label, unlabel_img):
         nl = label_img.shape[0]
@@ -305,11 +315,16 @@
             teacher()
         t_out = box[0]
         self._mark(4)
+        ol = self._on_load(self.model, out, t_out)
+        if ol is not None:
+            res = seg_loss(out, target_label, nl, coef=self.sc.view(S_COEF_A, 8), teacher_logits=t_out, dp=self.dp, on_load=ol)
+        L.log_launch("join:teacher", torch.cuda.current_stream(self.dev).cuda_stream)
         self._join(self.side, t_out)
         self._mark(5)
-        res = seg_loss(out, target_label, nl, coef=self.sc.view(S_COEF_A, 8), teacher_logits=t_out, dp=self.dp)
+        if ol is None:
+            res = seg_loss(out, target_label, nl, coef=self.sc.view(S_COEF_A, 8), teacher_logits=t_out, dp=self.dp)
         self.optimizer.zero_grad()
-        self._loss_backward(res)
+        self._loss_backward(res, ol)
         self._mark(6)
         return {"loss": res[0].detach(), "parts": res.detach(), "logits": out.detach(), "t_logits": t_out}
 
diff --git a/hpfg_amd/utils/__init__.py b/hpfg_amd/utils/__init__.py
--- a/hpfg_amd/utils/__init__.py
+++ b/hpfg_amd/utils/__init__.py
@@ -1,4 +1,4 @@
-from .loss import DiceLoss, Med_Sup_Loss, Dense_Loss, seg_loss
+from .loss import DiceLoss, Med_Sup_Loss, Dense_Loss, loss_on_load_ok, seg_loss
 from .optim import FusedAdamW, FusedSGD, build_lr_scheduler, build_optimizer, flatten_parameters
 from .scheduler import CosineWarmupLR_Scheduler, Medical_LR, PolyLR
 from .utils import (AttrDict, BoxMaskGenerator, ema_alpha, get_current_consistency_weight, linear_rampup, loadyaml, mk_path,
diff --git a/hpfg_amd/utils/loss.py b/hpfg_amd/utils/loss.py
--- a/hpfg_amd/utils/loss.py
+++ b/hpfg_amd/utils/loss.py
@@ -24,9 +24,60 @@
     return t.contiguous()
 
 
+def _exchanges(dp) -> bool:
+    if dp is not None and not getattr(dp, "sync_bn", True):
+        return False
+    return dp is not None and (dp.world_size > 1 or dp.force_sync)
+
+
+def loss_on_load_ok(net, logits: torch.Tensor, teacher_logits: Optional[torch.Tensor] = None, dp=None) -> bool:
+    ok = getattr(net, "loss_on_load_ok", None)
+    if ok is None or _exchanges(dp) or L.load().hpfg_get_option(L.OPT_LOSS_ON_LOAD) == 0:
+        return False
+    if logits.dtype != torch.float32 or not logits.permute(0, 2, 3, 1).is_contiguous():
+        return False
+    t = teacher_logits
+    if t is not None and (t.dtype != torch.float32 or not t.permute(0, 2, 3, 1).is_contiguous()):
+        return False
+    return bool(ok(logits.permute(0, 2, 3, 1)))
+
+
+class LossOnLoad:
+
+    def __init__(self, args, args_cons, keep):
+        self.args, self.args_cons, self.keep = args, args_cons, keep
+        self.dlogits: Optional[torch.Tensor] = None
+        self.grad_scale: Optional[torch.Tensor] = None
+        self.consumed = self.tail_done = False
+
+    def fill(self, fa: "L.FusedBwdArgs"):
+        a, g, s = self.args, fa.lg, fa.d.a0
+        s.z, s.mode, s.C, s.Hs, s.Ws, s.pstride = a.logits, L.ACT_LOSSG, a.C, a.H, a.W, a.C
+        g.t_logits, g.labels0, g.labels1, g.sums, g.coef = a.t_logits, a.labels0, a.labels1, a.sums, a.coef
+        g.grad_scale, g.dlogits = L.ptr(self.grad_scale), L.ptr(self.dlogits)
+        g.n_lab, g.t_unlab_only, g.world = a.n_lab, a.t_unlab_only, a.world
+
+    def fallback(self, stream: int):
+        self.args.dlogits = L.ptr(self.dlogits)
+        L.log_launch("loss_bwd", stream)
+        L.check(L.load().hpfg_seg_loss_bwd(C.byref(self.args), L.ptr(self.grad_scale), stream), "seg_loss_bwd")
+        self.consumed = True
+
+    def tail(self, stream: int):
+        if self.tail_done:
+            return
+        lib = L.load()
+        if self.args_cons is not None:
+            L.log_launch("loss_partials:cons", stream)
+            L.check(lib.hpfg_seg_loss_partials_part(C.byref(self.args_cons), 1, stream), "seg_loss_partials_part")
+        L.log_launch("loss_finalize", stream)
+        L.check(lib.hpfg_seg_loss_finalize(C.byref(self.args), stream), "seg_loss_finalize")
+        self.tail_done = True
+
+
 class _SegLossFn(torch.autograd.Function):
     @staticmethod
-    def forward(ctx, logits, coef, labels0, labels1, t_logits, n_lab, is_prob, dp, t_is_prob=False, cons_mask=None):
+    def forward(ctx, logits, coef, labels0, labels1, t_logits, n_lab, is_prob, dp, t_is_prob=False, cons_mask=None, on_load=None):
         lib = L.load()
         if not logits.is_cuda:
             raise RuntimeError("hpfg_amd losses run on the HIP library only (no CPU fallback)")
@@ -62,15 +113,38 @@
                 raise ValueError("cons_mask needs a consistency target and one weight per unlabelled pixel")
             a.cons_mask = L.ptr(cm)
         st = torch.cuda.current_stream(dev).cuda_stream
+        ctx.on_load = None
+        if on_load is not None:
+            if is_prob or t_is_prob or cons_mask is not None or _exchanges(dp) or x.data_ptr() != logits.data_ptr() or (
+                    t is not None and t.data_ptr() != t_logits.data_ptr()) or not on_load.loss_on_load_ok(x):
+                raise RuntimeError("seg_loss(on_load=...): not eligible for the on-load route (ask loss_on_load_ok first)")
+            a_cons = None
+            if t is not None:
+                a.t_logits = None
+            L.log_launch("loss_partials:student", st)
+            L.check(lib.hpfg_seg_loss_partials_part(C.byref(a), 0, st), "seg_loss_partials_part")
+            if t is not None:
+                a.t_logits = L.ptr(t)
+                partials2 = torch.empty(nblk * nsum, dtype=torch.float32, device=dev)
+                a_cons = L.LossArgs.from_buffer_copy(a)
+                a_cons.labels0, a_cons.labels1, a_cons.partials = None, None, L.ptr(partials2)
+                partials = (partials, partials2)
+            ctx.on_load = LossOnLoad(a, a_cons, (x, t, labels0, labels1, coef, sums, cm, partials, out))
+            on_load.expect_loss_on_load(ctx.on_load)
+            ctx.args, ctx.keep = a, (x, t, labels0, labels1, coef, sums, cm)
+            ctx.shape = (N, H, W, Cc)
+            return out
         if dp is not None and getattr(dp, "p2p", False) and (dp.world_size > 1 or dp.force_sync):
             slot, epoch = dp.next_loss_slot()
             dp.bump(epoch, st)
             px = dp.peer_desc(slot, epoch)
             L.check(lib.hpfg_seg_loss_partials_x(C.byref(a), C.byref(px), st), "seg_loss_partials_x")
         else:
+            L.log_launch("loss_partials", st)
             L.check(lib.hpfg_seg_loss_partials(C.byref(a), st), "seg_loss_partials")
             if dp is not None and (dp.world_size > 1 or dp.force_sync):
                 dp.allreduce_sum(sums)
+        L.log_launch("loss_finalize", st)
         L.check(lib.hpfg_seg_loss_finalize(C.byref(a), st), "seg_loss_finalize")
         ctx.args, ctx.keep = a, (x, t, labels0, labels1, coef, sums, cm)
         ctx.shape = (N, H, W, Cc)
@@ -85,20 +159,24 @@
         dl = torch.empty(N, H, W, Cc, dtype=torch.float32, device=x.device)
         a.dlogits = L.ptr(dl)
         gs = gout[0:1].contiguous()
-        L.check(lib.hpfg_seg_loss_bwd(C.byref(a), L.ptr(gs), torch.cuda.current_stream(x.device).cuda_stream), "seg_loss_bwd")
-        return dl.permute(0, 3, 1, 2), None, None, None, None, None, None, None, None, None
+        if ctx.on_load is not None and not ctx.on_load.consumed:
+            ctx.on_load.dlogits, ctx.on_load.grad_scale = dl, gs
+        else:
+            L.log_launch("loss_bwd", torch.cuda.current_stream(x.device).cuda_stream)
+            L.check(lib.hpfg_seg_loss_bwd(C.byref(a), L.ptr(gs), torch.cuda.current_stream(x.device).cuda_stream), "seg_loss_bwd")
+        return dl.permute(0, 3, 1, 2), None, None, None, None, None, None, None, None, None, None
 
 
 def seg_loss(logits: torch.Tensor, labels: Optional[torch.Tensor], n_lab: Optional[int] = None, *,
              coef: torch.Tensor, pseudo: Optional[torch.Tensor] = None, teacher_logits: Optional[torch.Tensor] = None,
              is_prob: bool = False, dp=None, teacher_prob: Optional[torch.Tensor] = None,
-             cons_mask: Optional[torch.Tensor] = None) -> torch.Tensor:
+             cons_mask: Optional[torch.Tensor] = None, on_load=None) -> torch.Tensor:
     N = logits.shape[0]
     n_lab = N if n_lab is None else int(n_lab)
     if teacher_prob is not None:
         assert teacher_logits is None
-        return _SegLossFn.apply(logits, coef, _labels_u8(labels), _labels_u8(pseudo), teacher_prob, n_lab, is_prob, dp, True, cons_mask)
-    return _SegLossFn.apply(logits, coef, _labels_u8(labels), _labels_u8(pseudo), teacher_logits, n_lab, is_prob, dp, False, cons_mask)
+        return _SegLossFn.apply(logits, coef, _labels_u8(labels), _labels_u8(pseudo), teacher_prob, n_lab, is_prob, dp, True, cons_mask, None)
+    return _SegLossFn.apply(logits, coef, _labels_u8(labels), _labels_u8(pseudo), teacher_logits, n_lab, is_prob, dp, False, cons_mask, on_load)
 
 
 def _coef(dev, vals: Sequence[float]) -> torch.Tensor:
diff --git a/include/hpfg_hip.h b/include/hpfg_hip.h
--- a/include/hpfg_hip.h
+++ b/include/hpfg_hip.h
@@ -7,7 +7,7 @@
 extern "C" {
 #endif
 
-#define HPFG_VERSION 142
+#define HPFG_VERSION 143
 enum { HPFG_MATH_F32 = 0, HPFG_MATH_BF16X3 = 1 };
 
 enum { HPFG_BN_MEAN = 0, HPFG_BN_RSTD = 1, HPFG_BN_SCALE = 2, HPFG_BN_SHIFT = 3,
@@ -22,7 +22,8 @@
   HPFG_ACT_UP2X = 5,
   HPFG_ACT_DZ = 6,
   HPFG_ACT_SPLIT16 = 7,
-  HPFG_ACT_UPBWD = 8
+  HPFG_ACT_UPBWD = 8,
+  HPFG_ACT_LOSSG = 9
 };
 
 typedef struct HpfgAct {
@@ -86,11 +87,26 @@
   int32_t defer_reduce;
 } HpfgWgradArgs;
 
+typedef struct HpfgLossGrad {
+  const float* t_logits;
+  const uint8_t* labels0;
+  const uint8_t* labels1;
+  const float* sums;
+  const float* coef;
+  const float* grad_scale;
+  float* dlogits;
+  int32_t n_lab;
+  int32_t t_unlab_only;
+  int32_t world;
+  int32_t reserved3;
+} HpfgLossGrad;
+
 typedef struct HpfgFusedBwdArgs {
   HpfgConvArgs d;
   HpfgAct xa0, xa1;
   float* slab;
   int32_t Cin, CinPad, Cout, CoutPad;
+  HpfgLossGrad lg;
 } HpfgFusedBwdArgs;
 
 typedef struct HpfgSlabDesc {
@@ -113,7 +129,8 @@
 
 int hpfg_version(void);
 const char* hpfg_last_error(void);
-enum { HPFG_OPT_CONV_THIN = 0, HPFG_OPT_FIRST_MFMA = 1, HPFG_OPT_FIRST_WGRAD = 2, HPFG_OPT_NARROW_DEEP = 3, HPFG_OPT_UPDATE_PACK = 4, HPFG_OPT_COUNT = 5 };
+enum { HPFG_OPT_CONV_THIN = 0, HPFG_OPT_FIRST_MFMA = 1, HPFG_OPT_FIRST_WGRAD = 2, HPFG_OPT_NARROW_DEEP = 3, HPFG_OPT_UPDATE_PACK = 4, HPFG_OPT_LOSS_ON_LOAD = 5,
+       HPFG_OPT_COUNT = 6 };
 int hpfg_get_option(int which);
 int hpfg_set_option(int which, int value);
 
@@ -250,6 +267,7 @@
 int hpfg_loss_nsum(int C);
 int hpfg_seg_loss_partials(const HpfgLossArgs* a, void* stream);
 int hpfg_seg_loss_partials_x(const HpfgLossArgs* a, const HpfgPeerX* px, void* stream);
+int hpfg_seg_loss_partials_part(const HpfgLossArgs* a, int part, void* stream);
 int hpfg_seg_loss_finalize(const HpfgLossArgs* a, void* stream);
 int hpfg_seg_loss_bwd(const HpfgLossArgs* a, const float* grad_scale_dev , void* stream);
 int hpfg_argmax_labels(const float* logits, int N, int H, int W, int C, const uint8_t* mix_labels, const float* mix_mask,
```

Result: no change. 8003 images/s, median of 3 (+0.0%).
